# mlrun/mlrun

Measured on AMD Instinct MI355X. Metric: serving-graph req/sec (Llama-3-8B V2ModelServer), higher is better.
Workload: dtype bf16; 1 GPU; model=llama-3-8b, global_batch=32, seq_len=160, prompt_len=128, parallelism=dp1 (2 engine replica(s)/GPU, 2 in flight), hipgraph=True

## Files before the change

mlrun_amd/models/llama.py:

```python

import math
import typing
from dataclasses import dataclass

import torch

from .. import ops
from ..utils import logger


@dataclass
class LlamaConfig:
    name: str = "llama-3-8b"
    hidden_size: int = 4096
    intermediate_size: int = 14336
    num_layers: int = 32
    num_heads: int = 32
    num_kv_heads: int = 8
    head_dim: int = 128
    vocab_size: int = 128256
    rope_theta: float = 500000.0
    rms_eps: float = 1e-5
    max_seq_len: int = 2048

# ... 81 lines not shown
    while f"blocks.{i}.attn_norm.weight" in state:
        prefix = f"blocks.{i}."
        out[f"layers.{i}.attn_norm"] = state[prefix + "attn_norm.weight"]
        out[f"layers.{i}.wqkv"] = state[prefix + "attn.wqkv.weight"]
        out[f"layers.{i}.wo"] = state[prefix + "attn.wo.weight"]
        out[f"layers.{i}.ffn_norm"] = state[prefix + "ffn_norm.weight"]
        out[f"layers.{i}.wgu"] = state[prefix + "mlp.wgu.weight"]
        out[f"layers.{i}.wdown"] = state[prefix + "mlp.wdown.weight"]
        i += 1
    return {k: v.to(torch.bfloat16) for k, v in out.items()}


LORA_PROJECTIONS = ("wqkv", "wo", "wgu", "wdown")


@dataclass
class SamplingParams:
    temperature: float = 0.0
    top_k: int = 0
    top_p: float = 1.0
    min_p: float = 0.0
    seed: int = 0
    logprobs: bool = False

    def validate(self):
        def number(name, value):
            if isinstance(value, bool) or \
                    not isinstance(value, (int, float)) or \
                    value != value:
                raise ValueError(f"{name} must be a number, got {value!r}")

        def integer(name, value):
            if isinstance(value, bool) or not isinstance(value, int):
                raise ValueError(f"{name} must be an integer, got "
                                 f"{value!r}")

        number("temperature", self.temperature)
        if not 0 <= self.temperature < float("inf"):
            raise ValueError(f"temperature must be >= 0 and finite, got "
                             f"{self.temperature}")
        integer("top_k", self.top_k)
        if not 0 <= self.top_k < 2 ** 31:
            raise ValueError(f"top_k must be an integer >= 0, got "
                             f"{self.top_k}")
        number("top_p", self.top_p)
        if not 0 < self.top_p <= 1:
            raise ValueError(f"top_p must be in (0, 1], got {self.top_p}")
        number("min_p", self.min_p)
        if not 0 <= self.min_p < 1:
            raise ValueError(f"min_p must be in [0, 1), got {self.min_p}")
        integer("seed", self.seed)
        if not 0 <= self.seed < 2 ** 63:
            raise ValueError(f"seed must be an integer in [0, 2^63), got "
                             f"{self.seed}")
        if not isinstance(self.logprobs, bool):
            raise ValueError(f"logprobs must be true or false, got "
                             f"{self.logprobs!r}")
        return self


class LoraTables:

    def __init__(self, weights: LlamaWeights, max_adapters: int,
                 rank: int = 16):
        if rank not in ops.LORA_RANKS:
            raise ValueError(f"lora_rank must be one of {ops.LORA_RANKS}, "
                             f"got {rank}")
        if max_adapters < 1:
            raise ValueError("LoraTables needs max_adapters >= 1")
        self.max_adapters = int(max_adapters)
        self.rank = int(rank)
        self.weights = weights
        self.loaded = set()
        bf16 = dict(dtype=torch.bfloat16, device=weights.device)
        self.layers = []
        for layer in weights.layers:
            tables = {}
            for proj in LORA_PROJECTIONS:
                n, k = layer[proj].shape
                tables[proj] = (
                    torch.zeros(self.max_adapters, self.rank, k, **bf16),
                    torch.zeros(self.max_adapters, n, self.rank, **bf16))
            self.layers.append(tables)

    def _check_slot(self, slot):
        if not 0 <= int(slot) < self.max_adapters:
            raise ValueError(f"adapter slot {slot} outside "
                             f"[0, {self.max_adapters})")
        return int(slot)

    def unload(self, slot: int):
        slot = self._check_slot(slot)
        for tables in self.layers:
            for a_tab, b_tab in tables.values():
                a_tab[slot].zero_()
                b_tab[slot].zero_()
        self.loaded.discard(slot)

    @torch.no_grad()
    def load(self, slot: int, state: dict):
        slot = self._check_slot(slot)
        if "alpha" not in state:
            raise ValueError("adapter state has no 'alpha'")
        alpha = float(state["alpha"])
        pending = []
        seen = set()
        for key in state:
            if not key.startswith("layers."):
                continue
            parts = key.split(".")
            if len(parts) != 4 or not parts[1].isdigit() or \
                    parts[2] not in LORA_PROJECTIONS or \
                    parts[3] not in ("lora_A", "lora_B") or \
                    int(parts[1]) >= len(self.layers):
                raise ValueError(f"unexpected adapter key {key!r}")
            seen.add((int(parts[1]), parts[2]))
        for li, proj in sorted(seen):
            key_a = f"layers.{li}.{proj}.lora_A"
            key_b = f"layers.{li}.{proj}.lora_B"
            for key in (key_a, key_b):
                if key not in state:
                    raise ValueError(f"adapter state lacks {key!r}")
            mat_a, mat_b = state[key_a], state[key_b]
            n, k = self.weights.layers[li][proj].shape
            if mat_a.dim() != 2 or mat_a.shape[1] != k:
                raise ValueError(f"{key_a}: expected [r, {k}], got "
                                 f"{tuple(mat_a.shape)}")
            r = mat_a.shape[0]
            if not 1 <= r <= self.rank:
                raise ValueError(f"{key_a}: rank {r} outside "
                                 f"[1, lora_rank={self.rank}]")
            if tuple(mat_b.shape) != (n, r):
                raise ValueError(f"{key_b}: expected [{n}, {r}], got "
                                 f"{tuple(mat_b.shape)}")
            pending.append((li, proj, r, mat_a, mat_b))
        self.unload(slot)
        for li, proj, r, mat_a, mat_b in pending:
            a_tab, b_tab = self.layers[li][proj]
            a_tab[slot, :r].copy_(mat_a)
            scaled = mat_b.to(device=b_tab.device, dtype=torch.float32) \
                * (alpha / r)
            b_tab[slot, :, :r].copy_(scaled)
        self.loaded.add(slot)


class LlamaDecodeEngine:

    def __init__(self, cfg: LlamaConfig, batch_size: int, device=None,
                 tp_group=None, tp_rank=0, tp_size=1, use_graph=True,
                 seed=1234, weights: "LlamaWeights" = None,
                 weight_dtype: str = "bf16", kv_dtype: str = "bf16",
                 temperature: float = 0.0, top_k: int = 0,
                 max_adapters: int = 0, lora_rank: int = 16,
                 lora: "LoraTables" = None, sampling: str = "engine"):
        if sampling not in ("engine", "request"):
            raise ValueError(f"unknown sampling mode {sampling!r} "
                             "(expected 'engine' or 'request')")
        if sampling == "request" and tp_size > 1:
            raise ValueError(
                f'sampling="request" conflicts with tp_size={tp_size}: '
                "per-request sampling runs on a single GPU")
        if sampling == "request" and batch_size > ops.SAMPLE_MAX_ROWS:
            raise ValueError(
                f'sampling="request" needs batch_size <= '
                f"{ops.SAMPLE_MAX_ROWS}, got {batch_size}")
        if (max_adapters > 0 or lora is not None) and tp_size > 1:
            raise ValueError(
                f"max_adapters={max_adapters} conflicts with tp_size="
                f"{tp_size}: LoRA adapters are not sharded")
        if (max_adapters > 0 or lora is not None) and \
                batch_size > ops.LORA_MAX_ROWS:
            raise ValueError(
                f"max_adapters > 0 needs batch_size <= "
                f"{ops.LORA_MAX_ROWS}, got {batch_size}")
        self.cfg = cfg
        self.B = batch_size
        self.device = torch.device(
            device or ("cuda:0" if torch.cuda.is_available() else "cpu"))
        self.on_gpu = self.device.type == "cuda"
        self.tp_group = tp_group
        self.tp_rank = tp_rank
        self.tp_size = tp_size
        self.use_graph = use_graph and self.on_gpu
        self.temperature = float(temperature)
        self.top_k = int(top_k)
        self.per_slot_temp = self.temperature < 0
        self.buf_temp = torch.full((batch_size, 1), 1e-4,
                                   dtype=torch.float32,
                                   device=self.device) \
            if self.per_slot_temp else None
        self.weights = weights if weights is not None else \
            LlamaWeights(cfg, self.device, tp_rank, tp_size, seed)
        w = self.weights
        d, h = cfg.head_dim, cfg.hidden_size
        B, smax = batch_size, cfg.max_seq_len
        bf16 = dict(dtype=torch.bfloat16, device=self.device)

        self.kv_dtype = kv_dtype
        if kv_dtype == "fp8":
            u8 = dict(dtype=torch.uint8, device=self.device)
            self.k_cache = torch.zeros(cfg.num_layers, B, w.hkv, smax, d,
                                       **u8)
            self.v_cache = torch.zeros(cfg.num_layers, B, w.hkv, smax, d,
                                       **u8)
            f32 = dict(dtype=torch.float32, device=self.device)
            self.k_scale = torch.ones(cfg.num_layers, B, w.hkv, smax,
                                      **f32)
            self.v_scale = torch.ones(cfg.num_layers, B, w.hkv, smax,
                                      **f32)
        else:
            self.k_cache = torch.zeros(cfg.num_layers, B, w.hkv, smax, d,
                                       **bf16)
            self.v_cache = torch.zeros(cfg.num_layers, B, w.hkv, smax, d,
                                       **bf16)
            self.k_scale = self.v_scale = None
        self.cache_lens = torch.zeros(B, dtype=torch.int32,
                                      device=self.device)
        self.buf_positions = torch.zeros(B, dtype=torch.int32,
                                         device=self.device)
        self.cos_sin = ops.build_rope_cos_sin(smax, d, cfg.rope_theta,
                                              self.device)

        qkv_n = (w.hq + 2 * w.hkv) * d
        gemm_shapes = [(qkv_n, h), (h, w.hq * d), (2 * w.inter, h),
                       (h, w.inter), (cfg.vocab_size, h)]
        scratch = max(ops.pick_gemm_plan(B, n, k)[0] * n
                      for n, k in gemm_shapes)
        self.buf_tokens = torch.zeros(B, dtype=torch.int64,
                                      device=self.device)
        self.buf_hidden = torch.zeros(B, h, **bf16)
        self.buf_residual = torch.zeros(B, h, **bf16)
        self.buf_qkv = torch.zeros(B, qkv_n, **bf16)
        self.buf_attn_out = torch.zeros(B, w.hq * d, **bf16)
        self.buf_proj = torch.zeros(B, h, **bf16)
        self.buf_gu = torch.zeros(B, 2 * w.inter, **bf16)
        self.buf_act = torch.zeros(B, w.inter, **bf16)
        self.buf_down = torch.zeros(B, h, **bf16)
        self.buf_logits = torch.zeros(B, cfg.vocab_size, **bf16)
        self.buf_c32 = torch.empty(B * scratch, dtype=torch.float32,
                                   device=self.device)
        self.scale = 1.0 / math.sqrt(d)
        self._capture_stream_ctx = None
        self.weight_dtype = weight_dtype
        self._fp8_packs = {}
        if weight_dtype == "fp8w" and self.on_gpu and tp_size == 1:
            max_k = max(h, w.inter, w.hq * d)
            self.buf_a8 = torch.empty(B * max_k, dtype=torch.uint8,
                                      device=self.device)
            self.buf_a_scale = torch.empty(B, dtype=torch.float32,
                                           device=self.device)
            self.buf_h8 = torch.empty(B, h, dtype=torch.uint8,
                                      device=self.device)
            self.buf_h8_scale = torch.empty(B, dtype=torch.float32,
                                            device=self.device)
            self.rebuild_fp8_packs()
        import os as _os
        _ns = _os.environ.get("MLRUN_ATTN_NSPLIT")
        self.attn_nsplit = int(_ns) if _ns else \
            ops.pick_attn_nsplit(B, w.hkv)
        self.buf_attn_ws = torch.empty(
            B * w.hq * self.attn_nsplit * (d + 2), dtype=torch.float32,
            device=self.device) if self.on_gpu else None
        self._graph = None
        self._ksplits = {}
        if lora is None and max_adapters > 0:
            lora = LoraTables(w, max_adapters, lora_rank)
        self.lora = lora
        self.max_adapters = lora.max_adapters if lora is not None else 0
        if lora is not None:
            self.buf_adapter = torch.full((B,), -1, dtype=torch.int32,
                                          device=self.device)
            self.buf_lora_t = torch.zeros(B, lora.rank,
                                          dtype=torch.float32,
                                          device=self.device)
        self.sampling = sampling
        if sampling == "request":
            dev = self.device
            self.buf_temp_r = torch.zeros(B, dtype=torch.float32, device=dev)
            self.buf_top_k = torch.zeros(B, dtype=torch.int32, device=dev)
            self.buf_top_p = torch.ones(B, dtype=torch.float32, device=dev)
            self.buf_min_p = torch.zeros(B, dtype=torch.float32, device=dev)
            self.buf_seed = torch.zeros(B, dtype=torch.int64, device=dev)
            self.buf_logprob = torch.zeros(B, dtype=torch.float32,
                                           device=dev)
            self.buf_kept = torch.zeros(B, dtype=torch.int32, device=dev)
        self.spec_stats = {"steps": 0, "drafted": 0, "accepted": 0}

    def set_sampling(self, slot: int, temperature: float = 0.0,
                     top_k: int = 0, top_p: float = 1.0, min_p: float = 0.0,
                     seed: int = 0):
        self.set_sampling_slots([slot], [SamplingParams(
            temperature, top_k, top_p, min_p, seed)])

    def set_sampling_slots(self, slots, params):
        if self.sampling != "request":
            raise ValueError('set_sampling needs an engine built with '
                             'sampling="request"')
        slots = [int(slot) for slot in slots]
        params = [SamplingParams() if item is None else item
                  for item in params]
        if len(slots) != len(params):
            raise ValueError(f"{len(params)} parameter sets for "
                             f"{len(slots)} slots")
        for slot in slots:
            if not 0 <= slot < self.B:
                raise ValueError(f"slot {slot} outside [0, {self.B})")
        for item in params:
            item.validate()
        if not slots:
            return
        index = torch.tensor(slots, dtype=torch.long).to(self.device)
        for buf, name in ((self.buf_temp_r, "temperature"),
                          (self.buf_top_k, "top_k"),
                          (self.buf_top_p, "top_p"),
                          (self.buf_min_p, "min_p"),
                          (self.buf_seed, "seed")):
            values = [getattr(item, name) for item in params]
            if name == "temperature":
                values = [max(value, 1e-4) if value > 0 else value
                          for value in values]
            values = torch.tensor(values, dtype=buf.dtype)
            buf[index] = values.to(self.device)

    def _packed_prefill_serves(self) -> bool:
        w = self.weights
        return self.kv_dtype == "bf16" and self.cfg.head_dim == 128 \
            and w.hq % w.hkv == 0 and w.hq // w.hkv <= 8

    def _sample_slots(self, logits, slots):
        logits = logits.contiguous()
        n = logits.shape[0]
        tokens = torch.empty(n, dtype=torch.int64, device=self.device)
        logprob = torch.empty(n, dtype=torch.float32, device=self.device)
        kept = torch.empty(n, dtype=torch.int32, device=self.device)
        ops.sample_tokens(
            logits, self.cache_lens[slots].contiguous(),
            self.buf_temp_r[slots].contiguous(),
            self.buf_top_k[slots].contiguous(),
            self.buf_top_p[slots].contiguous(),
            self.buf_min_p[slots].contiguous(),
            self.buf_seed[slots].contiguous(), tokens, logprob, kept)
        self.buf_tokens[slots] = tokens
        self.buf_logprob[slots] = logprob
        self.buf_kept[slots] = kept
        return tokens

    def _plan(self, w_):
        key = (w_.shape[0], w_.shape[1])
        if key not in self._ksplits:
            self._ksplits[key] = ops.pick_gemm_plan(self.B, *key)
        return self._ksplits[key]

    def _gemm(self, a, w_, out, a8=None, a_scale=None):
        pack = self._fp8_packs.get(id(w_))
        if pack is not None:
            M, K = a.shape
            if a8 is None:
                a8 = self.buf_a8.narrow(0, 0, M * K).view(M, K)
                ops.quant_fp8_rows(a, a8, self.buf_a_scale)
                a_scale = self.buf_a_scale
            ksplit, _ = self._plan(w_)
            return ops.skinny_gemm_fp8(a8, a_scale, pack[0],
                                       pack[1], out=out,
                                       c_f32=self.buf_c32, ksplit=ksplit)
        ksplit, variant = self._plan(w_)
        return ops.skinny_gemm(a, w_, out=out, c_f32=self.buf_c32,
                               ksplit=ksplit, variant=variant)

    def _gemm_slabs(self, a, w_):
        from mlrun_amd import _hip_ops

        ksplit, variant = self._plan(w_)
        if ksplit <= 1:
            return 0
        _hip_ops.skinny_gemm_slabs(self.buf_c32, a, w_, ksplit, variant)
        return ksplit

    def _maybe_allreduce(self, t):
        if self.tp_size > 1:
            from ..parallel.tp import all_reduce_tensor

            all_reduce_tensor(t, group=self.tp_group)
        return t

    def load_adapter(self, slot: int, state: dict):
        if self.lora is None:
            raise ValueError("engine built with max_adapters=0 holds no "
                             "adapter tables")
        self.lora.load(slot, state)

    def unload_adapter(self, slot: int):
        if self.lora is None:
            raise ValueError("engine built with max_adapters=0 holds no "
                             "adapter tables")
        self.lora.unload(slot)

    def _lora_decode(self, li, proj, x, y):
        a_tab, b_tab = self.lora.layers[li][proj]
        ops.lora_shrink(x, a_tab, self.buf_adapter, out=self.buf_lora_t)
        ops.lora_expand(y, self.buf_lora_t, b_tab, self.buf_adapter)

    def _adapter_plan(self, adapters, slots, counts):
        if adapters is None:
            if self.lora is not None:
                self.buf_adapter[slots] = -1
            return None
        ids = [int(a) for a in adapters]
        if self.lora is None:
            if any(a >= 0 for a in ids):
                raise ValueError("adapters= needs an engine built with "
                                 "max_adapters > 0")
            return None
        if len(ids) != len(counts):
            raise ValueError(f"adapters has {len(ids)} ids for "
                             f"{len(counts)} prompts")
        for a in ids:
            if not -1 <= a < self.max_adapters:
                raise ValueError(f"adapter id {a} outside "
                                 f"[-1, {self.max_adapters})")
        self.buf_adapter[slots] = torch.tensor(
            ids, dtype=torch.int32).to(self.device)
        distinct = sorted({a for a in ids if a >= 0})
        if not distinct:
            return None
        if len(set(ids)) == 1:
            return [(distinct[0], None)]
        row_ids = torch.tensor(
            [a for a, count in zip(ids, counts) for _ in range(count)],
            dtype=torch.int32).to(self.device)
        return [(a, (row_ids == a).unsqueeze(1)) for a in distinct]

    def _lora_prefill(self, plan, li, proj, x, y):
        if plan is None:
            return y
        a_tab, b_tab = self.lora.layers[li][proj]
        xf = x.float()
        for a, mask in plan:
            delta = (xf @ a_tab[a].float().t()) @ b_tab[a].float().t()
            new = (y.float() + delta).to(y.dtype)
            y = new if mask is None else torch.where(mask, new, y)
        return y

    def _decode_step_body(self):
        cfg, w = self.cfg, self.weights
        d = cfg.head_dim
        B = self.B
        torch.index_select(w.embed, 0, self.buf_tokens,
                           out=self.buf_residual)
        fp8 = self.weight_dtype == "fp8w" and self.on_gpu and \
            self.tp_size == 1
        h8 = self.buf_h8 if fp8 else None
        h8s = self.buf_h8_scale if fp8 else None
        ops.rmsnorm(self.buf_residual, w.layers[0]["attn_norm"],
                    eps=cfg.rms_eps, out=self.buf_hidden,
                    out8=h8, out_scale=h8s)
        torch.clamp(self.cache_lens, max=self.cfg.max_seq_len - 1,
                    out=self.buf_positions)
        self.cache_lens.add_(1).clamp_(max=self.cfg.max_seq_len)
        positions = self.buf_positions
        import os as _os

        mode = _os.environ.get("MLRUN_SLAB_MODE", "rope")
        on = self.on_gpu and self.tp_size == 1 and mode != "none"
        use_slabs = on and self.weight_dtype == "bf16" and \
            self.kv_dtype == "bf16"
        use_norm_slabs = on and mode == "all" 
        lora = self.lora is not None
        if lora:
            use_slabs = use_norm_slabs = False
        for li, layer in enumerate(w.layers):
            done = 0
            if use_slabs:
                done = self._gemm_slabs(self.buf_hidden, layer["wqkv"])
                if done:
                    from mlrun_amd import _hip_ops

                    _hip_ops.rope_kv_slab(
                        self.buf_qkv, self.k_cache[li], self.v_cache[li],
                        self.buf_c32, positions, self.cos_sin, w.hq, done)
            if not done:
                self._gemm(self.buf_hidden, layer["wqkv"], self.buf_qkv,
                           a8=h8, a_scale=h8s)
                if lora:
                    self._lora_decode(li, "wqkv", self.buf_hidden,
                                      self.buf_qkv)
                ops.rope_kv_fused(self.buf_qkv, self.k_cache[li],
                                  self.v_cache[li], positions,
                                  self.cos_sin, w.hq,
                                  k_scale=self._kscale(li),
                                  v_scale=self._vscale(li))
            q = self.buf_qkv[:, :w.hq * d].view(B, w.hq, d)
            attn_view = self.buf_attn_out.view(B, w.hq, d)
            ops.attn_decode(q, self.k_cache[li], self.v_cache[li],
                            self.cache_lens, self.scale, out=attn_view,
                            partial_ws=self.buf_attn_ws,
                            nsplit=self.attn_nsplit,
                            k_scale=self._kscale(li),
                            v_scale=self._vscale(li))
            done = 0
            if use_norm_slabs:
                done = self._gemm_slabs(self.buf_attn_out, layer["wo"])
                if done:
                    from mlrun_amd import _hip_ops

                    _hip_ops.fused_add_rmsnorm_slab(
                        self.buf_hidden, self.buf_residual, self.buf_c32,
                        layer["ffn_norm"], done, cfg.rms_eps)
            if not done:
                self._gemm(self.buf_attn_out, layer["wo"], self.buf_proj)
                if lora:
                    self._lora_decode(li, "wo", self.buf_attn_out,
                                      self.buf_proj)
                self._maybe_allreduce(self.buf_proj)
                ops.fused_add_rmsnorm(self.buf_proj, layer["ffn_norm"],
                                      residual=self.buf_residual,
                                      eps=cfg.rms_eps, out=self.buf_hidden,
                                      out8=h8, out_scale=h8s)
            done = 0
            if use_norm_slabs:
                done = self._gemm_slabs(self.buf_hidden, layer["wgu"])
                if done:
                    from mlrun_amd import _hip_ops

                    _hip_ops.swiglu_slab(self.buf_act, self.buf_c32, done)
            if not done:
                self._gemm(self.buf_hidden, layer["wgu"], self.buf_gu,
                           a8=h8, a_scale=h8s)
                if lora:
                    self._lora_decode(li, "wgu", self.buf_hidden,
                                      self.buf_gu)
                ops.swiglu_fused(self.buf_gu, out=self.buf_act)
            next_norm = w.layers[li + 1]["attn_norm"] \
                if li + 1 < cfg.num_layers else w.final_norm
            done = 0
            if use_norm_slabs:
                done = self._gemm_slabs(self.buf_act, layer["wdown"])
                if done:
                    from mlrun_amd import _hip_ops

                    _hip_ops.fused_add_rmsnorm_slab(
                        self.buf_hidden, self.buf_residual, self.buf_c32,
                        next_norm, done, cfg.rms_eps)
            if not done:
                self._gemm(self.buf_act, layer["wdown"], self.buf_down)
                if lora:
                    self._lora_decode(li, "wdown", self.buf_act,
                                      self.buf_down)
                self._maybe_allreduce(self.buf_down)
                ops.fused_add_rmsnorm(self.buf_down, next_norm,
                                      residual=self.buf_residual,
                                      eps=cfg.rms_eps, out=self.buf_hidden,
                                      out8=h8, out_scale=h8s)
        self._gemm(self.buf_hidden, w.lm_head, self.buf_logits,
                   a8=h8, a_scale=h8s)
        if self.sampling == "request":
            ops.sample_tokens(self.buf_logits, self.cache_lens,
                              self.buf_temp_r, self.buf_top_k,
                              self.buf_top_p, self.buf_min_p, self.buf_seed,
                              self.buf_tokens, self.buf_logprob,
                              self.buf_kept)
        else:
            self._select_tokens(self.buf_logits, out=self.buf_tokens)

    def _select_tokens(self, logits: torch.Tensor,
                       out: torch.Tensor = None) -> torch.Tensor:
        if self.per_slot_temp and logits.shape[0] == self.B:
            scores = logits.float() / self.buf_temp
            u = torch.rand_like(scores).clamp_(1e-9, 1.0 - 1e-9)
            gumbel = -torch.log(-torch.log(u))
            if out is None:
                return (scores + gumbel).argmax(dim=-1)
            torch.argmax(scores + gumbel, dim=-1, out=out)
            return out
        if self.temperature <= 0.0:
            if out is None:
                return logits.argmax(dim=-1)
            torch.argmax(logits, dim=-1, out=out)
            return out
        scores = logits.float() / self.temperature
        if self.top_k > 0 and self.top_k < scores.shape[-1]:
            kth = torch.topk(scores, self.top_k, dim=-1
                             ).values[..., -1:]
            scores = torch.where(scores < kth,
                                 torch.full_like(scores, float("-inf")),
                                 scores)
        u = torch.rand_like(scores).clamp_(1e-9, 1.0 - 1e-9)
        gumbel = -torch.log(-torch.log(u))
        if out is None:
            return (scores + gumbel).argmax(dim=-1)
        torch.argmax(scores + gumbel, dim=-1, out=out)
        return out

    _capture_lock = None

    def capture_graph(self):
        if not self.use_graph or self._graph is not None:
            return
        import threading

        cls = type(self)
        if cls._capture_lock is None:
            cls._capture_lock = threading.Lock()
        with cls._capture_lock:
            self._capture_graph_locked()

    def _capture_graph_locked(self):
        if self._graph is not None:
            return
        import torch.distributed as dist

        lens_backup = self.cache_lens.clone()
        tokens_backup = self.buf_tokens.clone()
        sample_backup = [(buf, buf.clone()) for buf in (
            self.buf_logprob, self.buf_kept)] \
            if self.sampling == "request" else []
        if self.tp_size > 1 and dist.is_available() and \
                dist.is_initialized():
            dist.barrier(group=self.tp_group)
        side = torch.cuda.Stream()
        side.wait_stream(torch.cuda.current_stream())
        with torch.cuda.stream(side):
            for _ in range(3):
                self._decode_step_body()
        torch.cuda.current_stream().wait_stream(side)
        self.cache_lens.copy_(lens_backup)
        self.buf_tokens.copy_(tokens_backup)
        for buf, backup in sample_backup:
            buf.copy_(backup)
        graph = torch.cuda.CUDAGraph()
        err_mode = "thread_local" if dist.is_available() and \
            dist.is_initialized() else "global"
        with torch.cuda.graph(graph, capture_error_mode=err_mode):
            self._decode_step_body()
        self.cache_lens.copy_(lens_backup)
        self.buf_tokens.copy_(tokens_backup)
        for buf, backup in sample_backup:
            buf.copy_(backup)
        self._graph = graph
        logger.info("decode hipGraph captured", batch=self.B,
                    layers=self.cfg.num_layers)

    def decode_step(self):
        if self._graph is not None:
            self._graph.replay()
        else:
            self._decode_step_body()

    def rebuild_fp8_packs(self):
        if self.weight_dtype != "fp8w" or not (self.on_gpu and
                                               self.tp_size == 1):
            return
        w = self.weights
        self._fp8_packs = {}
        for layer in w.layers:
            for key in ("wqkv", "wo", "wgu", "wdown"):
                self._fp8_packs[id(layer[key])] = \
                    ops.quantize_fp8_weight(layer[key])
        self._fp8_packs[id(w.lm_head)] = \
            ops.quantize_fp8_weight(w.lm_head)

    def _kscale(self, li):
        return None if self.k_scale is None else self.k_scale[li]

    def _vscale(self, li):
        return None if self.v_scale is None else self.v_scale[li]

    def _check_token_ids(self, tokens: torch.Tensor):
        if tokens.device.type != "cpu" or tokens.numel() == 0:
            return
        low, high = int(tokens.min()), int(tokens.max())
        if low < 0 or high >= self.cfg.vocab_size:
            raise ValueError(
                f"token id outside [0, {self.cfg.vocab_size}) in prompt")

    @torch.no_grad()
    def prefill(self, tokens: torch.Tensor, adapters=None
                ) -> torch.Tensor:
        cfg, w = self.cfg, self.weights
        B, S = tokens.shape
        d = cfg.head_dim
        self._check_token_ids(tokens)
        plan = self._adapter_plan(adapters, slice(0, B), [S] * B)
        tokens = tokens.to(self.device)
        x = w.embed[tokens.reshape(-1)]
        residual = x.contiguous()
        positions = torch.arange(S, dtype=torch.int32, device=self.device
                                 ).repeat(B)
        hidden = ops.rmsnorm(residual, w.layers[0]["attn_norm"],
                             eps=cfg.rms_eps)
        for li, layer in enumerate(w.layers):
            qkv = self._lora_prefill(plan, li, "wqkv", hidden,
                                     hidden @ layer["wqkv"].t())
            q = qkv[:, :w.hq * d].reshape(B * S, w.hq, d).contiguous()
            k = qkv[:, w.hq * d:(w.hq + w.hkv) * d].reshape(
                B * S, w.hkv, d).contiguous()
# ... 255 lines not shown
                             f"(kv_dtype={self.kv_dtype!r})")
        if self.weight_dtype != "bf16":
            raise ValueError("speculative decoding needs bf16 weights "
                             f"(weight_dtype={self.weight_dtype!r})")
        if self.tp_size != 1:
            raise ValueError("speculative decoding needs tp_size == 1")
        if not 1 <= int(k) <= ops.VERIFY_MAX_QL - 1:
            raise ValueError(
                f"speculative k must be in [1, {ops.VERIFY_MAX_QL - 1}], "
                f"got {k}")

    def _verify_gemm(self, a, w_, QL):
        if self.on_gpu:
            return a @ w_.t()
        out = torch.empty(a.shape[0], w_.shape[0], dtype=a.dtype)
        for j in range(QL):
            out[j::QL] = ops.skinny_gemm(a[j::QL].contiguous(), w_)
        return out

    @torch.no_grad()
    def verify_step(self, drafts: torch.Tensor):
        cfg, w = self.cfg, self.weights
        if drafts.dim() != 2 or drafts.shape[0] != self.B:
            raise ValueError(f"drafts must be [{self.B}, k], got "
                             f"{tuple(drafts.shape)}")
        k = drafts.shape[1]
        self._check_speculative(k)
        B, QL, d = self.B, k + 1, cfg.head_dim
        T = B * QL
        drafts = drafts.to(device=self.device, dtype=torch.int64)
        fed = drafts.clamp(0, cfg.vocab_size - 1)
        tokens = torch.cat([self.buf_tokens.view(B, 1), fed], dim=1)
        base = torch.clamp(self.cache_lens, min=0,
                           max=cfg.max_seq_len - QL)
        steps = torch.arange(QL, dtype=torch.int32, device=self.device)
        positions = (base.view(B, 1) + steps).reshape(T)
        tok_slot = torch.arange(B, dtype=torch.int32, device=self.device
                                ).repeat_interleave(QL)
        nsplit, ws = None, None
        if self.on_gpu:
            nsplit = ops.pick_verify_nsplit(B, w.hkv, cfg.max_seq_len)
            need = ops.attn_verify_ws_numel(B, QL, w.hq, nsplit)
            ws = getattr(self, "_verify_ws", None)
            if nsplit > 1 and (ws is None or ws.numel() < need):
                ws = self._verify_ws = torch.empty(
                    need, dtype=torch.float32, device=self.device)
        residual = w.embed[tokens.reshape(T)].contiguous()
        hidden = ops.rmsnorm(residual, w.layers[0]["attn_norm"],
                             eps=cfg.rms_eps)
        for li, layer in enumerate(w.layers):
            qkv = self._verify_gemm(hidden, layer["wqkv"], QL)
            ops.rope_kv_varlen(qkv, self.k_cache[li], self.v_cache[li],
                               positions, tok_slot, self.cos_sin, w.hq)
            q = qkv[:, :w.hq * d].view(B, QL, w.hq, d)
            attn = ops.attn_verify(q, self.k_cache[li], self.v_cache[li],
                                   base, self.scale, nsplit=nsplit,
                                   partial_ws=ws)
            proj = self._verify_gemm(attn, layer["wo"], QL)
            hidden = ops.fused_add_rmsnorm(proj, layer["ffn_norm"],
                                           residual=residual,
                                           eps=cfg.rms_eps)
            gu = self._verify_gemm(hidden, layer["wgu"], QL)
            act = ops.swiglu_fused(gu.contiguous())
            down = self._verify_gemm(act, layer["wdown"], QL)
            next_norm = w.layers[li + 1]["attn_norm"] \
                if li + 1 < cfg.num_layers else w.final_norm
            hidden = ops.fused_add_rmsnorm(down, next_norm,
                                           residual=residual,
                                           eps=cfg.rms_eps)
        logits = getattr(self, "buf_verify_logits", None)
        if logits is None or logits.shape[1] != QL:
            logits = self.buf_verify_logits = torch.empty(
                B, QL, cfg.vocab_size, dtype=torch.bfloat16,
                device=self.device)
        logits.view(T, cfg.vocab_size).copy_(
            self._verify_gemm(hidden, w.lm_head, QL))
        pred = logits.argmax(dim=-1)
        hits = (drafts == pred[:, :k]).to(torch.int64)
        n_accepted = hits.cumprod(dim=1).sum(dim=1)
        self.cache_lens.add_((n_accepted + 1).to(torch.int32)
                             ).clamp_(max=cfg.max_seq_len)
        self.buf_tokens.copy_(
            pred.gather(1, n_accepted.view(B, 1)).view(B))
        return pred, n_accepted

    def _speculative_loop(self, history: torch.Tensor,
                          hist_lens: torch.Tensor, start_lens: torch.Tensor,
                          active: torch.Tensor, max_new_tokens: int,
                          k: int, ngram: int) -> torch.Tensor:
        B, QL = self.B, k + 1
        L = history.shape[1]
        steps = torch.arange(QL, dtype=torch.int64, device=self.device)
        counters = torch.zeros(2, dtype=torch.int64, device=self.device)
        big = torch.full((B,), max_new_tokens, dtype=torch.int32,
                         device=self.device)
        n_steps = 0
        produced_min = 1
        while produced_min < max_new_tokens:
            produced = hist_lens - start_lens
            done = (produced >= max_new_tokens) | ~active
            drafts = ops.ngram_draft(history, hist_lens, k, n=ngram)
            lens_before = self.cache_lens.clone()
            tokens_before = self.buf_tokens.clone()
            pred, n_accepted = self.verify_step(drafts)
            self.cache_lens.copy_(
                torch.where(done, lens_before, self.cache_lens))
            self.buf_tokens.copy_(
                torch.where(done, tokens_before, self.buf_tokens))
            idx = (hist_lens.view(B, 1).long() + steps).clamp_(max=L - 1)
            vals = torch.where(done.view(B, 1), history.gather(1, idx),
                               pred)
            history.scatter_(1, idx, vals)
            live = ~done
            hist_lens.add_((live * (n_accepted + 1)).to(torch.int32))
            counters[0] += live.sum() * k
            counters[1] += (n_accepted * live).sum()
            n_steps += 1
            produced_min = int(torch.where(
                active, hist_lens - start_lens, big).min())
        drafted, accepted = counters.tolist()
        self.spec_stats["steps"] += n_steps
        self.spec_stats["drafted"] += drafted
        self.spec_stats["accepted"] += accepted
        cols = start_lens.view(B, 1).long() + torch.arange(
            max_new_tokens, dtype=torch.int64, device=self.device)
        return history.gather(1, cols.clamp_(max=L - 1))

    @torch.no_grad()
    def generate_speculative(self, tokens: torch.Tensor,
                             max_new_tokens: int = 32, k: int = 3,
                             ngram: int = 2) -> torch.Tensor:
        B, S = tokens.shape
        assert B == self.B, f"engine built for batch {self.B}, got {B}"
        self._check_speculative(k)
        assert S + max_new_tokens + k <= self.cfg.max_seq_len, \
            "speculative decoding needs room for k drafted tokens: " \
            f"{S}+{max_new_tokens}+{k} > {self.cfg.max_seq_len}"
        logits = self.prefill(tokens)
        self.buf_tokens.copy_(self._select_tokens(logits))
        history = torch.zeros(B, self.cfg.max_seq_len, dtype=torch.int64,
                              device=self.device)
        history[:, :S] = tokens.to(self.device)
        history[:, S] = self.buf_tokens
        hist_lens = torch.full((B,), S + 1, dtype=torch.int32,
                               device=self.device)
        start_lens = torch.full((B,), S, dtype=torch.int32,
                                device=self.device)
        active = torch.ones(B, dtype=torch.bool, device=self.device)
        return self._speculative_loop(history, hist_lens, start_lens,
                                      active, max_new_tokens, k, ngram)

    def reset(self):
        self.cache_lens.zero_()


class LlamaServer:

    def __init__(self, context=None, name=None, model_path=None,
                 config=None, batch_size=16, max_new_tokens=32,
                 device=None, use_graph=True, batch_window_ms=0,
                 replicas=1, weight_dtype="bf16", kv_dtype="bf16",
                 scheduling="batch", stop_token: int = None,
                 temperature: float = 0.0, top_k: int = 0,
                 prefill: str = "exact", speculative: int = 0,
                 adapters: dict = None, max_adapters: int = None,
                 lora_rank: int = 16, sampling: str = "engine",
                 top_p: float = 1.0, min_p: float = 0.0, **class_args):
        import queue as queue_mod
        import threading

        from ..serving.v2_serving import V2ModelServer

        self.name = name
        self.context = context
        self.model_path = model_path
        self.ready = False
        self.error = ""
        self.protocol = "v2"
        self.model_spec = None
        self._model_logger = None
        self._params = class_args
        self.cfg_name = config or "llama-3-8b"
        self.batch_size = batch_size
        self.max_new_tokens = max_new_tokens
        self.device = device
        self.use_graph = use_graph
        self.weight_dtype = weight_dtype
        self.kv_dtype = kv_dtype
        self.scheduling = scheduling
        if prefill not in ("exact", "packed"):
            raise ValueError(f"unknown prefill mode {prefill!r} "
                             "(expected 'exact' or 'packed')")
        self.prefill = prefill
        self.stop_token = stop_token
        self.temperature = float(temperature)
        self.top_k = int(top_k)
        self.speculative = int(speculative)
        self.adapters = dict(adapters or {})
        self.adapter_slots = {name: slot for slot, name
                              in enumerate(self.adapters)}
        self.max_adapters = len(self.adapters) if max_adapters is None \
            else int(max_adapters)
        if self.max_adapters < len(self.adapters):
            raise ValueError(
                f"max_adapters={self.max_adapters} is below the "
                f"{len(self.adapters)} adapters configured")
        self.lora_rank = int(lora_rank)
        self._lora_requests = {name: 0 for name in self.adapters}
        self._lora_lock = threading.Lock()
        if sampling not in ("engine", "request"):
            raise ValueError(f"unknown sampling mode {sampling!r} "
                             "(expected 'engine' or 'request')")
        self.sampling = sampling
        self._sampling_defaults = None
        self._sampling_counts = {"requests": 0, "sampled": 0, "greedy": 0}
        if sampling == "request":
            if self.temperature < 0:
                raise ValueError(
                    f"temperature={temperature} conflicts with "
                    'sampling="request": per-slot temperatures are the '
                    "request field there, the default must be >= 0")
            self._sampling_defaults = SamplingParams(
                temperature=temperature, top_k=top_k, top_p=top_p,
                min_p=min_p).validate()
        self._check_speculative_config()
        self.replicas = max(int(replicas), 1)
        self.engines: typing.List[LlamaDecodeEngine] = []
        self.batch_window_ms = batch_window_ms
        self._tasks: "queue_mod.Queue" = queue_mod.Queue()
        self._workers: typing.List[threading.Thread] = []
        self._pending = []
        self._pending_cv = threading.Condition()
        self._batcher = None
        self.engine_calls = 0

    @property
    def engine(self):
        return self.engines[0] if self.engines else None

    def _check_speculative_config(self):
        k = self.speculative
        if k == 0:
            return
        if self.sampling == "request":
            raise ValueError(
                f'speculative={k} conflicts with sampling="request": '
                "speculative decoding is greedy only")
        if self.max_adapters > 0:
            raise ValueError(
                f"speculative={k} conflicts with LoRA adapters "
                f"({sorted(self.adapters)}): the verify pass runs the "
                "base weights only")
        if not 1 <= k <= ops.VERIFY_MAX_QL - 1:
            raise ValueError(
                f"speculative={k} is outside [0, {ops.VERIFY_MAX_QL - 1}]")
        if self.scheduling == "continuous":
            raise ValueError(
                f'speculative={k} conflicts with scheduling="continuous" '
                "(its output ring takes one token per slot per step): "
                'use scheduling="batch"')
        if self.temperature != 0.0:
            raise ValueError(
                f"speculative={k} conflicts with temperature="
                f"{self.temperature}: speculative decoding is greedy only")
        if self.kv_dtype == "fp8":
            raise ValueError(
                f'speculative={k} conflicts with kv_dtype="fp8": the '
                "verify attention kernel reads bf16 caches only")
        if self.weight_dtype == "fp8w":
            raise ValueError(
                f'speculative={k} conflicts with weight_dtype="fp8w": '
                "the verify pass runs on the bf16 weights")

    def post_init(self, mode="sync"):
        stream = getattr(self.context, "stream", None) if self.context \
            else None
        if stream is not None:
            from ..serving.v2_serving import _ModelLogPusher

            self._model_logger = _ModelLogPusher(self, stream)
        if mode == "sync":
            self.load()
            self.ready = True

    def _build_config(self) -> LlamaConfig:
        if self.cfg_name in ("llama-3-8b", "8b"):
            cfg = LlamaConfig.llama3_8b()
        elif self.cfg_name in ("llama-3-70b", "70b"):
            cfg = LlamaConfig.llama3_70b()
        elif self.cfg_name == "tiny":
            cfg = LlamaConfig.tiny()
        elif isinstance(self.cfg_name, LlamaConfig):
            cfg = self.cfg_name
        else:
            raise ValueError(f"unknown llama config {self.cfg_name}")
        for key, value in self._params.items():
            if hasattr(cfg, key):
                setattr(cfg, key, value)
        return cfg

    def load(self):
        import threading

        cfg = self._build_config()
        self._check_speculative_config()
        if self.prefill == "packed" and self.kv_dtype == "fp8":
# ... 628 lines not shown
```

mlrun_amd/ops/__init__.py:

```python

import math
import os

import torch

from ..errors import MLRunGPUError

try:
    from mlrun_amd import _hip_ops

    HAVE_HIP_OPS = True
except ImportError:
    _hip_ops = None
    HAVE_HIP_OPS = False


def _require_hip():
    if not HAVE_HIP_OPS:
        raise MLRunGPUError(
            "mlrun_amd._hip_ops extension is not built — run "
            "`PYTORCH_ROCM_ARCH=gfx950 python setup.py build_ext --inplace` "
            "(GPU ops never fall back to eager execution)")
    return _hip_ops




def fused_add_rmsnorm(x: torch.Tensor, weight: torch.Tensor,
                      residual: torch.Tensor = None, eps: float = 1e-5,
                      out: torch.Tensor = None,
                      out8: torch.Tensor = None,
                      out_scale: torch.Tensor = None) -> torch.Tensor:
    if x.is_cuda:
        ops = _require_hip()
        if out is None:
            out = torch.empty_like(x)
        ops.fused_add_rmsnorm(out, x, weight, residual, eps, out8,
                              out_scale)
        return out
    z = x.float() + (residual.float() if residual is not None else 0.0)
    if residual is not None:
        residual.copy_(z.to(residual.dtype))
    var = z.pow(2).mean(dim=-1, keepdim=True)
    result = (z * torch.rsqrt(var + eps)) * weight.float()
    result = result.to(x.dtype)
    if out is not None:
        out.copy_(result)
        return out
    return result


def rmsnorm(x, weight, eps=1e-5, out=None, out8=None, out_scale=None):
    return fused_add_rmsnorm(x, weight, residual=None, eps=eps, out=out,
                             out8=out8, out_scale=out_scale)




def build_rope_cos_sin(max_pos: int, head_dim: int, theta: float = 500000.0,
                       device="cpu") -> torch.Tensor:
    half = head_dim // 2
    inv_freq = 1.0 / (theta ** (torch.arange(0, half, dtype=torch.float64)
                                / half))
    pos = torch.arange(max_pos, dtype=torch.float64)
    angles = torch.outer(pos, inv_freq)
    table = torch.stack([angles.cos(), angles.sin()], dim=-1).float()
    return table.contiguous().to(device)


def rope_inplace(q: torch.Tensor, positions: torch.Tensor,
                 cos_sin: torch.Tensor):
    if q.is_cuda:
        _require_hip().rope(q, positions, cos_sin)
        return q
    T, heads, dim = q.shape
    half = dim // 2
    table = cos_sin[positions.long()]
    cos = table[..., 0].unsqueeze(1)
    sin = table[..., 1].unsqueeze(1)
    qf = q.float()
    q1 = qf[..., :half]
    q2 = qf[..., half:]
    q[..., :half] = (q1 * cos - q2 * sin).to(q.dtype)
    q[..., half:] = (q2 * cos + q1 * sin).to(q.dtype)
    return q




def swiglu_fused(gu: torch.Tensor, out: torch.Tensor = None) -> torch.Tensor:
    rows, two_i = gu.shape
    inter = two_i // 2
    if gu.is_cuda:
        ops = _require_hip()
        if out is None:
            out = torch.empty(rows, inter, dtype=gu.dtype, device=gu.device)
        ops.swiglu_fused(out, gu)
        return out
    result = (torch.nn.functional.silu(gu[:, :inter].float()) *
              gu[:, inter:].float()).to(gu.dtype)
    if out is not None:
        out.copy_(result)
        return out
    return result


def silu_mul(gate: torch.Tensor, up: torch.Tensor,
             out: torch.Tensor = None) -> torch.Tensor:
    if gate.is_cuda:
        ops = _require_hip()
        if out is None:
            out = torch.empty_like(gate)
        ops.silu_mul(out, gate, up)
        return out
    result = (torch.nn.functional.silu(gate.float()) *
              up.float()).to(gate.dtype)
    if out is not None:
        out.copy_(result)
        return out
    return result




def pick_ksplit(M: int, N: int, K: int, target_blocks: int = 2048) -> int:
    nblocks = (N + 127) // 128
    if nblocks >= target_blocks:
        return 1
    ksplit = (target_blocks + nblocks - 1) // nblocks
    ksplit = min(ksplit, max(K // 256, 1), 16)
    return max(ksplit, 1)


_EMPTY_F32 = None


_GEMM_PLAN_TABLE = {
    (6144, 4096): (4, 4),
    (4096, 4096): (2, 4),
    (28672, 4096): (1, 4),
    (4096, 14336): (4, 4),
    (128256, 4096): (1, 0),
}

_plan_env = os.environ.get("MLRUN_GEMM_PLAN", "")
if _plan_env:
    for _cell in _plan_env.split(";"):
        _shape, _plan = _cell.split("=")
        _n, _k = _shape.split("x")
        _ks, _var = _plan.split(",")
        _GEMM_PLAN_TABLE[(int(_n), int(_k))] = (int(_ks), int(_var))


def pick_gemm_plan(M: int, N: int, K: int) -> tuple:
    if (N, K) in _GEMM_PLAN_TABLE:
        return _GEMM_PLAN_TABLE[(N, K)]
    nblocks_ws = (N + 31) // 32
    if nblocks_ws <= 512 and K >= 2048:
        ksplit = max(1, min(1024 // nblocks_ws, K // 1024, 8))
        return ksplit, 1
    return pick_ksplit(M, N, K), 0


def skinny_gemm(a: torch.Tensor, w: torch.Tensor,
                out: torch.Tensor = None,
                c_f32: torch.Tensor = None,
                ksplit: int = None, variant: int = None) -> torch.Tensor:
    global _EMPTY_F32

    M, K = a.shape
    N = w.shape[0]
    if a.is_cuda:
        ops = _require_hip()
        if ksplit is None and variant is None:
            ksplit, variant = pick_gemm_plan(M, N, K)
        elif ksplit is None:
            ksplit = pick_ksplit(M, N, K)
        elif variant is None:
            variant = 0
        if out is None:
            out = torch.empty(M, N, dtype=torch.bfloat16, device=a.device)
        if ksplit > 1 and c_f32 is None:
            c_f32 = torch.empty(ksplit * M * N, dtype=torch.float32,
                                device=a.device)
        if c_f32 is None:
            if _EMPTY_F32 is None or _EMPTY_F32.device != a.device:
                _EMPTY_F32 = torch.empty(1, dtype=torch.float32,
                                         device=a.device)
            c_f32 = _EMPTY_F32
        ops.skinny_gemm(out, c_f32, a, w, ksplit, variant)
        return out
    result = (a.float() @ w.float().t()).to(a.dtype)
    if out is not None:
        out.copy_(result)
        return out
    return result


FP8_MAX = 448.0


def _fp8_pair_swizzle(q: torch.Tensor) -> torch.Tensor:
    n, k = q.shape
    assert k % 64 == 0, "K must be a multiple of 64 for the fp8 path"
    return q.view(n, k // 64, 2, 4, 8).permute(0, 1, 3, 2, 4) \
        .contiguous().view(n, k)


def _fp8_pair_unswizzle(q: torch.Tensor) -> torch.Tensor:
    n, k = q.shape
    return q.view(n, k // 64, 4, 2, 8).permute(0, 1, 3, 2, 4) \
        .contiguous().view(n, k)


def quantize_fp8_weight(w: torch.Tensor):
    amax = w.float().abs().amax(dim=1).clamp(min=1e-8)
    scale = amax / FP8_MAX
    q = (w.float() / scale[:, None]).to(torch.float8_e4m3fn)
    q8 = _fp8_pair_swizzle(q.view(torch.uint8))
    return q8.contiguous(), scale.to(torch.float32).contiguous()


def quant_fp8_rows(a: torch.Tensor, a8: torch.Tensor = None,
                   a_scale: torch.Tensor = None):
    rows, cols = a.shape[0], a.shape[-1]
    if a.is_cuda:
        ops = _require_hip()
        if a8 is None:
            a8 = torch.empty(a.shape, dtype=torch.uint8, device=a.device)
        if a_scale is None:
            a_scale = torch.empty(rows, dtype=torch.float32,
                                  device=a.device)
        ops.quant_fp8_rows(a8, a_scale, a)
        return a8, a_scale
    amax = a.float().abs().amax(dim=-1).clamp(min=1e-8)
    scale = amax / FP8_MAX
    q = (a.float() / scale[:, None]).to(torch.float8_e4m3fn)
    q = _fp8_pair_swizzle(q.view(torch.uint8))
    if a8 is not None:
        a8.copy_(q)
        a_scale.copy_(scale)
        return a8, a_scale
    return q.contiguous(), scale.to(torch.float32).contiguous()


def skinny_gemm_fp8(a8: torch.Tensor, a_scale: torch.Tensor,
                    w8: torch.Tensor, w_scale: torch.Tensor,
                    out: torch.Tensor = None, c_f32: torch.Tensor = None,
                    ksplit: int = 1) -> torch.Tensor:
    global _EMPTY_F32

    M, K = a8.shape
    N = w8.shape[0]
    if a8.is_cuda:
        ops = _require_hip()
        if out is None:
            out = torch.empty(M, N, dtype=torch.bfloat16,
                              device=a8.device)
        if ksplit > 1 and c_f32 is None:
            c_f32 = torch.empty(ksplit * M * N, dtype=torch.float32,
                                device=a8.device)
        if c_f32 is None:
            if _EMPTY_F32 is None or _EMPTY_F32.device != a8.device:
                _EMPTY_F32 = torch.empty(1, dtype=torch.float32,
                                         device=a8.device)
            c_f32 = _EMPTY_F32
        ops.skinny_gemm_fp8(out, c_f32, a8, a_scale, w8, w_scale, ksplit)
        return out
    a = _fp8_pair_unswizzle(a8).view(torch.float8_e4m3fn).float() * \
        a_scale[:, None].float()
    w = _fp8_pair_unswizzle(w8).view(torch.float8_e4m3fn).float() * \
        w_scale[:, None].float()
    result = (a @ w.t()).to(torch.bfloat16)
    if out is not None:
        out.copy_(result)
        return out
    return result


def rope_kv_fused(qkv: torch.Tensor, k_cache: torch.Tensor,
                  v_cache: torch.Tensor, positions: torch.Tensor,
                  cos_sin: torch.Tensor, hq: int,
                  k_scale: torch.Tensor = None,
                  v_scale: torch.Tensor = None):
    B = qkv.shape[0]
    hkv, d = k_cache.shape[1], k_cache.shape[3]
    if qkv.is_cuda:
        _require_hip().rope_kv_fused(qkv, k_cache, v_cache, positions,
                                     cos_sin, hq, k_scale, v_scale)
        return
    q = qkv[:, :hq * d].view(B, hq, d)
    k = qkv[:, hq * d:(hq + hkv) * d].view(B, hkv, d)
    v = qkv[:, (hq + hkv) * d:(hq + 2 * hkv) * d].view(B, hkv, d)
    rope_inplace(q, positions, cos_sin)
    rope_inplace(k, positions, cos_sin)
    if k_scale is not None:
        for b in range(B):
            pos = int(positions[b])
            k8, ks = quantize_kv_rows(k[b])
            v8, vs = quantize_kv_rows(v[b])
            k_cache[b, :, pos] = k8
            v_cache[b, :, pos] = v8
            k_scale.view(B, hkv, -1)[b, :, pos] = ks
            v_scale.view(B, hkv, -1)[b, :, pos] = vs
        return
    kv_append(k_cache, v_cache, k, v, positions)


def quantize_kv_rows(x: torch.Tensor):
    amax = x.float().abs().amax(dim=-1, keepdim=True)
    scales = torch.where(amax > 0, amax / 448.0,
                         torch.ones_like(amax))
    q8 = (x.float() / scales).to(torch.float8_e4m3fn).view(torch.uint8)
    return q8, scales.squeeze(-1)


def dequantize_kv_rows(q8: torch.Tensor, scales: torch.Tensor,
                       dtype=torch.float32):
    x = q8.view(torch.float8_e4m3fn).float()
    return (x * scales.unsqueeze(-1)).to(dtype)




def pick_attn_nsplit(B: int, Hkv: int, target: int = 2048,
                     seq_len: int = None) -> int:
    base = max(B * Hkv, 1)
    fill = (target + base - 1) // base
    chunk = (seq_len + 127) // 128 if seq_len else 1
    n = max(1, fill, chunk)
    n = 1 << (n - 1).bit_length()
    return min(n, 16)


def attn_decode(q: torch.Tensor, k_cache: torch.Tensor,
                v_cache: torch.Tensor, seq_lens: torch.Tensor,
                scale: float = None,
                out: torch.Tensor = None,
                partial_ws: torch.Tensor = None,
                nsplit: int = None,
                k_scale: torch.Tensor = None,
                v_scale: torch.Tensor = None) -> torch.Tensor:
    B, Hq, D = q.shape
    Hkv = k_cache.shape[1]
    scale = scale if scale is not None else 1.0 / math.sqrt(D)
    if q.is_cuda:
        ops = _require_hip()
        if out is None:
            out = torch.empty_like(q)
        if nsplit is None:
            nsplit = pick_attn_nsplit(B, Hkv)
        if nsplit > 1 and partial_ws is None:
            partial_ws = torch.empty(B * Hq * nsplit * (D + 2),
                                     dtype=torch.float32, device=q.device)
        ops.attn_decode(out, q, k_cache, v_cache, seq_lens, scale,
                        partial_ws, nsplit, k_scale, v_scale)
        return out
    if out is None:
        out = torch.empty_like(q)
    if k_scale is not None:
        k_cache = dequantize_kv_rows(k_cache,
                                     k_scale.view(B, Hkv, -1))
        v_cache = dequantize_kv_rows(v_cache,
                                     v_scale.view(B, Hkv, -1))
    G = Hq // Hkv
    for b in range(B):
        length = int(seq_lens[b])
        for h in range(Hq):
            kvh = h // G
            qv = q[b, h].float()
            keys = k_cache[b, kvh, :length].float()
            vals = v_cache[b, kvh, :length].float()
            scores = torch.softmax(keys @ qv * scale, dim=0)
            out[b, h] = (scores @ vals).to(q.dtype)
    return out




def rope_kv_varlen(qkv: torch.Tensor, k_cache: torch.Tensor,
                   v_cache: torch.Tensor, positions: torch.Tensor,
                   tok_slot: torch.Tensor, cos_sin: torch.Tensor, hq: int):
    T = qkv.shape[0]
    hkv, d = k_cache.shape[1], k_cache.shape[3]
    if qkv.is_cuda:
        _require_hip().rope_kv_varlen(qkv, k_cache, v_cache, positions,
                                      tok_slot, cos_sin, hq)
        return
    q = qkv[:, :hq * d].view(T, hq, d)
    k = qkv[:, hq * d:(hq + hkv) * d].view(T, hkv, d)
    v = qkv[:, (hq + hkv) * d:(hq + 2 * hkv) * d].view(T, hkv, d)
    rope_inplace(q, positions, cos_sin)
    rope_inplace(k, positions, cos_sin)
    for t in range(T):
        slot, pos = int(tok_slot[t]), int(positions[t])
        k_cache[slot, :, pos] = k[t]
        v_cache[slot, :, pos] = v[t]


def attn_prefill(q: torch.Tensor, k_cache: torch.Tensor,
                 v_cache: torch.Tensor, cu_seqlens: torch.Tensor,
                 slots: torch.Tensor, kv_start: torch.Tensor,
                 scale: float = None, out: torch.Tensor = None,
                 max_q_len: int = None) -> torch.Tensor:
    T, Hq, D = q.shape
    Hkv = k_cache.shape[1]
    scale = scale if scale is not None else 1.0 / math.sqrt(D)
    if out is None:
        out = torch.empty(T, Hq * D, dtype=q.dtype, device=q.device)
    if q.is_cuda:
        ops = _require_hip()
        if max_q_len is None:
            cu = cu_seqlens.tolist()
            max_q_len = max((b - a for a, b in zip(cu, cu[1:])), default=0)
        ops.attn_prefill(out, q, k_cache, v_cache, cu_seqlens, slots,
                         kv_start, scale, int(max_q_len))
        return out
    G = Hq // Hkv
    cu = cu_seqlens.tolist()
    out_v = out.view(T, Hq, D)
    for i in range(len(cu) - 1):
        slot, start = int(slots[i]), int(kv_start[i])
        for j in range(cu[i + 1] - cu[i]):
            row = cu[i] + j
            length = start + j + 1
            for h in range(Hq):
                kvh = h // G
                qv = q[row, h].float()
                keys = k_cache[slot, kvh, :length].float()
                vals = v_cache[slot, kvh, :length].float()
                scores = torch.softmax(keys @ qv * scale, dim=0)
                out_v[row, h] = (scores @ vals).to(q.dtype)
    return out



VERIFY_MAX_QL = 8
_VERIFY_WS_ROW = 128 + 4


def pick_verify_nsplit(B: int, Hkv: int, Smax: int,
                       target: int = 512) -> int:
    base = max(B * Hkv, 1)
    n = max(1, target // base)
    n = 1 << (n.bit_length() - 1)
    return max(1, min(n, 16, (Smax + 63) // 64))


def attn_verify_ws_numel(B: int, QL: int, Hq: int, nsplit: int) -> int:
    return B * QL * Hq * nsplit * _VERIFY_WS_ROW


def attn_verify(q: torch.Tensor, k_cache: torch.Tensor,
                v_cache: torch.Tensor, base_lens: torch.Tensor,
                scale: float = None, out: torch.Tensor = None,
                nsplit: int = None,
                partial_ws: torch.Tensor = None) -> torch.Tensor:
    if q.dim() != 4 or k_cache.dim() != 4:
        raise ValueError("attn_verify: q must be [B, QL, Hq, D] and the "
                         "caches [B, Hkv, Smax, D]")
    B, QL, Hq, D = q.shape
    Hkv, Smax = k_cache.shape[1], k_cache.shape[2]
    if D != 128 or k_cache.shape[3] != D:
        raise ValueError(f"attn_verify needs head_dim 128, got {D}")
    if not 1 <= QL <= VERIFY_MAX_QL:
        raise ValueError(
            f"attn_verify needs 1 <= QL <= {VERIFY_MAX_QL}, got {QL}")
    if Hkv < 1 or Hq % Hkv or Hq // Hkv > 8:
        raise ValueError("attn_verify: q heads per kv head must divide "
                         f"and be <= 8 (Hq={Hq}, Hkv={Hkv})")
    if k_cache.dtype != torch.bfloat16 or v_cache.dtype != torch.bfloat16 \
            or q.dtype != torch.bfloat16:
        raise ValueError("attn_verify reads bf16 q and bf16 KV caches only")
    if k_cache.shape[0] != B or base_lens.numel() != B:
        raise ValueError("attn_verify: q, caches and base_lens must agree "
                         "on the batch size")
    scale = scale if scale is not None else 1.0 / math.sqrt(D)
    if out is None:
        out = torch.empty(B * QL, Hq * D, dtype=q.dtype, device=q.device)
    if q.is_cuda:
        ops = _require_hip()
        if nsplit is None:
            nsplit = pick_verify_nsplit(B, Hkv, Smax)
        nsplit = max(int(nsplit), 1)
        if nsplit > 1 and partial_ws is None:
            partial_ws = torch.empty(
                attn_verify_ws_numel(B, QL, Hq, nsplit),
                dtype=torch.float32, device=q.device)
        ops.attn_verify(out, q, k_cache, v_cache, base_lens, scale,
                        partial_ws, nsplit)
        return out
    cu = torch.arange(B + 1, dtype=torch.int32) * QL
    slots = torch.arange(B, dtype=torch.int32)
    return attn_prefill(q.reshape(B * QL, Hq, D), k_cache, v_cache, cu,
                        slots, base_lens, scale, out=out)


def ngram_draft(history: torch.Tensor, hist_lens: torch.Tensor, k: int,
                n: int = 2, out: torch.Tensor = None) -> torch.Tensor:
    if history.dim() != 2 or history.dtype != torch.int64:
        raise ValueError("ngram_draft: history must be [B, L] int64")
    k, n = int(k), int(n)
    if k < 1 or not 1 <= n <= 64:
        raise ValueError("ngram_draft needs k >= 1 and 1 <= n <= 64")
    B, L = history.shape
    if hist_lens.numel() != B:
        raise ValueError("ngram_draft: one hist_lens entry per row")
    if out is None:
        out = torch.empty(B, k, dtype=torch.int64, device=history.device)
# ... 479 lines not shown
```

mlrun_amd/ops/hip/bindings.cpp:

```cpp

#include <torch/extension.h>
#include <c10/hip/HIPStream.h>

#include "kernels.h"

#define CHECK_DEV(x) TORCH_CHECK((x).is_cuda(), #x " must be on GPU")
#define CHECK_CONTIG(x) TORCH_CHECK((x).is_contiguous(), #x " not contiguous")
#define CHECK_BF16(x) \
  TORCH_CHECK((x).scalar_type() == torch::kBFloat16, #x " must be bf16")
#define CHECK_F32(x) \
  TORCH_CHECK((x).scalar_type() == torch::kFloat32, #x " must be f32")

#define CHECK_U8(x) \
  TORCH_CHECK((x).scalar_type() == torch::kUInt8, #x " must be uint8")

#define CHECK_I32(x) \
  TORCH_CHECK((x).scalar_type() == torch::kInt32, #x " must be int32")

static void* stream() {
  return (void*)c10::hip::getCurrentHIPStream().stream();
}

void fused_add_rmsnorm(torch::Tensor out, torch::Tensor x,
                       torch::Tensor weight,
                       c10::optional<torch::Tensor> residual, double eps,
                       c10::optional<torch::Tensor> out8,
                       c10::optional<torch::Tensor> out_scale) {
  CHECK_DEV(out); CHECK_CONTIG(out); CHECK_BF16(out);
  CHECK_DEV(x); CHECK_CONTIG(x); CHECK_BF16(x);
  CHECK_DEV(weight); CHECK_CONTIG(weight); CHECK_BF16(weight);
  int64_t hidden = x.size(-1);
  int64_t rows = x.numel() / hidden;
  TORCH_CHECK(hidden % 8 == 0, "hidden must be a multiple of 8");
  TORCH_CHECK(weight.numel() == hidden, "weight size mismatch");
  void* res_ptr = nullptr;
  if (residual.has_value()) {
    CHECK_DEV(*residual); CHECK_CONTIG(*residual); CHECK_BF16(*residual);
    TORCH_CHECK(residual->numel() == x.numel(), "residual size mismatch");
    res_ptr = residual->data_ptr();
  }
  void* out8_ptr = nullptr;
  void* scale_ptr = nullptr;
  if (out8.has_value()) {
    TORCH_CHECK(out_scale.has_value(), "out8 needs out_scale");
    TORCH_CHECK(out8->numel() == x.numel() &&
                out_scale->numel() >= rows, "fp8 sidecar sizes");
    TORCH_CHECK(hidden % 64 == 0, "fp8 sidecar needs hidden % 64 == 0");
    out8_ptr = out8->data_ptr();
    scale_ptr = out_scale->data_ptr();
  }
  launch_fused_add_rmsnorm(out.data_ptr(), res_ptr, x.data_ptr(),
                           weight.data_ptr(), (int)rows, (int)hidden,
                           (float)eps, out8_ptr, scale_ptr, stream());
}

static long long check_head_view(const torch::Tensor& q) {
  TORCH_CHECK(q.dim() == 3, "expected [T, heads, dim]");
  TORCH_CHECK(q.stride(2) == 1 && q.stride(1) == q.size(2),
              "inner dims must be dense (strides (*, dim, 1))");
  return (long long)q.stride(0);
}

void rope(torch::Tensor q, torch::Tensor positions, torch::Tensor cos_sin) {
  CHECK_DEV(q); CHECK_BF16(q);
  CHECK_DEV(positions); CHECK_CONTIG(positions); CHECK_I32(positions);
  CHECK_DEV(cos_sin); CHECK_CONTIG(cos_sin); CHECK_F32(cos_sin);
  long long row_stride = check_head_view(q);
  int T = q.size(0), heads = q.size(1), dim = q.size(2);
  TORCH_CHECK(dim % 2 == 0 && dim / 2 <= 1024, "bad head dim");
  TORCH_CHECK(positions.numel() == T, "positions size mismatch");
  launch_rope(q.data_ptr(), positions.data_ptr(), cos_sin.data_ptr(), T,
              heads, dim, row_stride, stream());
}

void swiglu_fused(torch::Tensor out, torch::Tensor gu) {
  CHECK_DEV(out); CHECK_CONTIG(out); CHECK_BF16(out);
  CHECK_DEV(gu); CHECK_CONTIG(gu); CHECK_BF16(gu);
  TORCH_CHECK(gu.dim() == 2 && out.dim() == 2, "need 2-D tensors");
  int rows = gu.size(0), inter = gu.size(1) / 2;
  TORCH_CHECK(out.size(0) == rows && out.size(1) == inter, "shape mismatch");
  TORCH_CHECK(inter % 8 == 0, "inter must be a multiple of 8");
  launch_swiglu_fused(out.data_ptr(), gu.data_ptr(), rows, inter, stream());
}

void silu_mul(torch::Tensor out, torch::Tensor gate, torch::Tensor up) {
  CHECK_DEV(out); CHECK_CONTIG(out); CHECK_BF16(out);
  CHECK_DEV(gate); CHECK_CONTIG(gate); CHECK_BF16(gate);
  CHECK_DEV(up); CHECK_CONTIG(up); CHECK_BF16(up);
  TORCH_CHECK(out.numel() == gate.numel() && gate.numel() == up.numel(),
              "size mismatch");
  TORCH_CHECK(out.numel() % 8 == 0, "numel must be a multiple of 8");
  launch_silu_mul(out.data_ptr(), gate.data_ptr(), up.data_ptr(),
                  out.numel(), stream());
}

void skinny_gemm(torch::Tensor out_bf16, torch::Tensor part_f32,
                 torch::Tensor a, torch::Tensor w, int64_t ksplit,
                 int64_t variant) {
  CHECK_DEV(out_bf16); CHECK_CONTIG(out_bf16); CHECK_BF16(out_bf16);
  CHECK_DEV(a); CHECK_CONTIG(a); CHECK_BF16(a);
  CHECK_DEV(w); CHECK_CONTIG(w); CHECK_BF16(w);
  int M = a.size(0), K = a.size(1), N = w.size(0);
  TORCH_CHECK(w.size(1) == K, "K mismatch");
  TORCH_CHECK(M <= 64, "skinny_gemm supports M <= 64");
  TORCH_CHECK(K % 32 == 0, "K must be a multiple of 32");
  TORCH_CHECK(out_bf16.numel() == (int64_t)M * N, "out shape mismatch");
  if (ksplit > 1) {
    CHECK_DEV(part_f32); CHECK_CONTIG(part_f32); CHECK_F32(part_f32);
    TORCH_CHECK(part_f32.numel() >= ksplit * (int64_t)M * N,
                "part_f32 scratch too small");
  }
  launch_skinny_gemm(out_bf16.data_ptr(),
                     ksplit > 1 ? part_f32.data_ptr() : nullptr,
                     a.data_ptr(), w.data_ptr(), M, N, K, (int)ksplit,
                     (int)variant, stream());
}

void skinny_gemm_slabs(torch::Tensor part_f32, torch::Tensor a,
                       torch::Tensor w, int64_t ksplit, int64_t variant) {
  CHECK_DEV(part_f32); CHECK_CONTIG(part_f32); CHECK_F32(part_f32);
  CHECK_DEV(a); CHECK_CONTIG(a); CHECK_BF16(a);
  CHECK_DEV(w); CHECK_CONTIG(w); CHECK_BF16(w);
  int M = a.size(0), K = a.size(1), N = w.size(0);
  TORCH_CHECK(w.size(1) == K && M <= 64 && K % 32 == 0, "bad shapes");
  TORCH_CHECK(part_f32.numel() >= ksplit * (int64_t)M * N,
              "part_f32 scratch too small");
  launch_skinny_gemm_slabs(part_f32.data_ptr(), a.data_ptr(), w.data_ptr(),
                           M, N, K, (int)ksplit, (int)variant, stream());
}

void fused_add_rmsnorm_slab(torch::Tensor out, torch::Tensor residual,
                            torch::Tensor slabs, torch::Tensor weight,
                            int64_t ksplit, double eps) {
  CHECK_DEV(out); CHECK_CONTIG(out); CHECK_BF16(out);
  CHECK_DEV(residual); CHECK_CONTIG(residual); CHECK_BF16(residual);
  CHECK_DEV(slabs); CHECK_CONTIG(slabs); CHECK_F32(slabs);
  CHECK_DEV(weight); CHECK_CONTIG(weight); CHECK_BF16(weight);
  int64_t hidden = out.size(-1);
  int64_t rows = out.numel() / hidden;
  TORCH_CHECK(hidden % 8 == 0, "hidden must be a multiple of 8");
  TORCH_CHECK(slabs.numel() >= ksplit * rows * hidden, "slabs too small");
  launch_fused_add_rmsnorm_slab(out.data_ptr(), residual.data_ptr(),
                                slabs.data_ptr(), weight.data_ptr(),
                                (int)rows, (int)hidden, (float)eps,
                                (int)ksplit, stream());
}

void swiglu_slab(torch::Tensor out, torch::Tensor slabs, int64_t ksplit) {
  CHECK_DEV(out); CHECK_CONTIG(out); CHECK_BF16(out);
  CHECK_DEV(slabs); CHECK_CONTIG(slabs); CHECK_F32(slabs);
  int rows = out.size(0), inter = out.size(1);
  TORCH_CHECK(inter % 4 == 0, "inter must be a multiple of 4");
  TORCH_CHECK(slabs.numel() >= (int64_t)ksplit * rows * 2 * inter,
              "slabs too small");
  launch_swiglu_slab(out.data_ptr(), slabs.data_ptr(), rows, inter,
                     (int)ksplit, stream());
}

void rope_kv_slab(torch::Tensor qkv, torch::Tensor kc, torch::Tensor vc,
                  torch::Tensor slabs, torch::Tensor positions,
                  torch::Tensor cos_sin, int64_t hq, int64_t ksplit) {
  CHECK_DEV(qkv); CHECK_CONTIG(qkv); CHECK_BF16(qkv);
  CHECK_DEV(kc); CHECK_CONTIG(kc); CHECK_BF16(kc);
  CHECK_DEV(slabs); CHECK_CONTIG(slabs); CHECK_F32(slabs);
  CHECK_DEV(positions); CHECK_CONTIG(positions); CHECK_I32(positions);
  CHECK_DEV(cos_sin); CHECK_CONTIG(cos_sin); CHECK_F32(cos_sin);
  int B = kc.size(0), Hkv = kc.size(1), Smax = kc.size(2), D = kc.size(3);
  int qkv_row = qkv.size(1);
  TORCH_CHECK(qkv.size(0) == B && qkv_row >= (hq + 2 * Hkv) * D,
              "qkv buffer too small");
  TORCH_CHECK(slabs.numel() >= (int64_t)ksplit * B * qkv_row,
              "slabs too small");
  launch_rope_kv_slab(qkv.data_ptr(), kc.data_ptr(), vc.data_ptr(),
                      slabs.data_ptr(), positions.data_ptr(),
                      cos_sin.data_ptr(), B, (int)hq, Hkv, Smax, D, qkv_row,
                      (int)ksplit, stream());
}

void rope_kv_fused(torch::Tensor qkv, torch::Tensor kc, torch::Tensor vc,
                   torch::Tensor positions, torch::Tensor cos_sin,
                   int64_t hq,
                   c10::optional<torch::Tensor> k_scale = c10::nullopt,
                   c10::optional<torch::Tensor> v_scale = c10::nullopt) {
  CHECK_DEV(qkv); CHECK_CONTIG(qkv); CHECK_BF16(qkv);
  CHECK_DEV(kc); CHECK_CONTIG(kc);
  CHECK_DEV(vc); CHECK_CONTIG(vc);
  CHECK_DEV(positions); CHECK_CONTIG(positions); CHECK_I32(positions);
  CHECK_DEV(cos_sin); CHECK_CONTIG(cos_sin); CHECK_F32(cos_sin);
  int B = kc.size(0), Hkv = kc.size(1), Smax = kc.size(2), D = kc.size(3);
  TORCH_CHECK(qkv.dim() == 2 && qkv.size(0) == B, "qkv must be [B, rows]");
  TORCH_CHECK(qkv.size(1) >= (hq + 2 * Hkv) * D, "qkv row too small");
  if (k_scale.has_value()) {
    TORCH_CHECK(v_scale.has_value(), "fp8 KV needs both scales");
    CHECK_U8(kc); CHECK_U8(vc);
    CHECK_DEV(*k_scale); CHECK_CONTIG(*k_scale); CHECK_F32(*k_scale);
    CHECK_DEV(*v_scale); CHECK_CONTIG(*v_scale); CHECK_F32(*v_scale);
    TORCH_CHECK(k_scale->numel() >= (int64_t)B * Hkv * Smax &&
                v_scale->numel() >= (int64_t)B * Hkv * Smax,
                "scale tensors too small");
    TORCH_CHECK(D == 128, "fp8 KV requires head_dim 128");
    launch_rope_kv_fused_q8(qkv.data_ptr(), kc.data_ptr(), vc.data_ptr(),
                            k_scale->data_ptr(), v_scale->data_ptr(),
                            positions.data_ptr(), cos_sin.data_ptr(), B,
                            (int)hq, Hkv, Smax, D, qkv.size(1), stream());
    return;
  }
  CHECK_BF16(kc); CHECK_BF16(vc);
  launch_rope_kv_fused(qkv.data_ptr(), kc.data_ptr(), vc.data_ptr(),
                       positions.data_ptr(), cos_sin.data_ptr(), B, (int)hq,
                       Hkv, Smax, D, qkv.size(1), stream());
}

void skinny_gemm_fp8(torch::Tensor out_bf16, torch::Tensor part_f32,
                     torch::Tensor a8, torch::Tensor a_scale,
                     torch::Tensor w8, torch::Tensor w_scale,
                     int64_t ksplit) {
  CHECK_DEV(out_bf16); CHECK_CONTIG(out_bf16); CHECK_BF16(out_bf16);
  CHECK_DEV(a8); CHECK_CONTIG(a8); CHECK_U8(a8);
  CHECK_DEV(w8); CHECK_CONTIG(w8); CHECK_U8(w8);
  CHECK_DEV(a_scale); CHECK_F32(a_scale);
  CHECK_DEV(w_scale); CHECK_F32(w_scale);
  int M = a8.size(0), K = a8.size(1), N = w8.size(0);
  TORCH_CHECK(w8.size(1) == K && M <= 64 && K % 64 == 0,
              "bad shapes (fp8 path needs K % 64 == 0)");
  TORCH_CHECK(a_scale.numel() >= M && w_scale.numel() >= N,
              "scale sizes");
  if (ksplit > 1) {
    CHECK_DEV(part_f32); CHECK_CONTIG(part_f32); CHECK_F32(part_f32);
    TORCH_CHECK(part_f32.numel() >= ksplit * (int64_t)M * N,
                "part_f32 scratch too small");
  }
  launch_skinny_gemm_fp8(out_bf16.data_ptr(),
                         ksplit > 1 ? part_f32.data_ptr() : nullptr,
                         a8.data_ptr(), a_scale.data_ptr(), w8.data_ptr(),
                         w_scale.data_ptr(), M, N, K, (int)ksplit,
                         stream());
}

void quant_fp8_rows(torch::Tensor a8, torch::Tensor a_scale,
                    torch::Tensor a) {
  CHECK_DEV(a8); CHECK_CONTIG(a8); CHECK_U8(a8);
  CHECK_DEV(a_scale); CHECK_F32(a_scale);
  CHECK_DEV(a); CHECK_CONTIG(a); CHECK_BF16(a);
  int64_t cols = a.size(-1);
  int64_t rows = a.numel() / cols;
  TORCH_CHECK(cols % 8 == 0, "cols must be a multiple of 8");
  TORCH_CHECK(a8.numel() == a.numel() && a_scale.numel() >= rows,
              "size mismatch");
  launch_quant_fp8_rows(a8.data_ptr(), a_scale.data_ptr(), a.data_ptr(),
                        (int)rows, (int)cols, stream());
}

void cast_f32_bf16(torch::Tensor out, torch::Tensor in) {
  CHECK_DEV(out); CHECK_CONTIG(out); CHECK_BF16(out);
  CHECK_DEV(in); CHECK_CONTIG(in); CHECK_F32(in);
  TORCH_CHECK(out.numel() == in.numel(), "size mismatch");
  launch_cast_f32_bf16(out.data_ptr(), in.data_ptr(), in.numel(), stream());
}

void attn_decode(torch::Tensor o, torch::Tensor q, torch::Tensor kc,
                 torch::Tensor vc, torch::Tensor seq_lens, double scale,
                 c10::optional<torch::Tensor> partial_ws, int64_t nsplit,
                 c10::optional<torch::Tensor> k_scale = c10::nullopt,
                 c10::optional<torch::Tensor> v_scale = c10::nullopt) {
  CHECK_DEV(o); CHECK_CONTIG(o); CHECK_BF16(o);
  CHECK_DEV(q); CHECK_BF16(q);
  CHECK_DEV(kc); CHECK_CONTIG(kc);
  CHECK_DEV(vc); CHECK_CONTIG(vc);
  const bool kvq = k_scale.has_value();
  if (kvq) {
    TORCH_CHECK(v_scale.has_value(), "fp8 KV needs both scales");
    CHECK_U8(kc); CHECK_U8(vc);
    CHECK_DEV(*k_scale); CHECK_CONTIG(*k_scale); CHECK_F32(*k_scale);
    CHECK_DEV(*v_scale); CHECK_CONTIG(*v_scale); CHECK_F32(*v_scale);
  } else {
    CHECK_BF16(kc); CHECK_BF16(vc);
  }
  CHECK_DEV(seq_lens); CHECK_CONTIG(seq_lens); CHECK_I32(seq_lens);
  TORCH_CHECK(q.dim() == 3 && kc.dim() == 4, "q [B,Hq,D], kc [B,Hkv,S,D]");
  long long q_row_stride = check_head_view(q);
  int B = q.size(0), Hq = q.size(1), D = q.size(2);
  int Hkv = kc.size(1), Smax = kc.size(2);
  TORCH_CHECK(D == 128, "attn_decode requires head_dim 128");
  TORCH_CHECK(Hq % Hkv == 0 && Hq / Hkv <= 8,
              "grouped heads per kv head must divide and be <= 8");
  TORCH_CHECK(kc.size(0) == B && kc.size(3) == D, "kc shape mismatch");
  float* ws = nullptr;
  if (nsplit > 1) {
    TORCH_CHECK(partial_ws.has_value(), "nsplit>1 needs partial_ws");
    CHECK_DEV(*partial_ws); CHECK_CONTIG(*partial_ws);
    CHECK_F32(*partial_ws);
    TORCH_CHECK(partial_ws->numel() >=
                (int64_t)B * Hq * nsplit * (D + 2),
                "partial_ws too small");
    ws = (float*)partial_ws->data_ptr();
  }
  if (kvq)
    TORCH_CHECK(k_scale->numel() >= (int64_t)B * Hkv * Smax &&
                v_scale->numel() >= (int64_t)B * Hkv * Smax,
                "scale tensors too small");
  launch_attn_decode(o.data_ptr(), q.data_ptr(), kc.data_ptr(),
                     vc.data_ptr(),
                     kvq ? k_scale->data_ptr() : nullptr,
                     kvq ? v_scale->data_ptr() : nullptr,
                     seq_lens.data_ptr(), B, Hq, Hkv, Smax,
                     (float)scale, q_row_stride, ws, (int)nsplit, stream());
}

void kv_append(torch::Tensor kc, torch::Tensor vc, torch::Tensor knew,
               torch::Tensor vnew, torch::Tensor positions) {
  CHECK_DEV(kc); CHECK_CONTIG(kc); CHECK_BF16(kc);
  CHECK_DEV(knew); CHECK_BF16(knew);
  CHECK_DEV(positions); CHECK_CONTIG(positions); CHECK_I32(positions);
  long long src_stride = check_head_view(knew);
  TORCH_CHECK(check_head_view(vnew) == src_stride,
              "knew/vnew strides must match");
  int B = kc.size(0), Hkv = kc.size(1), Smax = kc.size(2), D = kc.size(3);
  TORCH_CHECK(D % 8 == 0, "head_dim must be a multiple of 8");
  launch_kv_append(kc.data_ptr(), vc.data_ptr(), knew.data_ptr(),
                   vnew.data_ptr(), positions.data_ptr(), B, Hkv, Smax, D,
                   src_stride, stream());
}

void rope_kv_varlen(torch::Tensor qkv, torch::Tensor kc, torch::Tensor vc,
                    torch::Tensor positions, torch::Tensor tok_slot,
                    torch::Tensor cos_sin, int64_t hq) {
  CHECK_DEV(qkv); CHECK_CONTIG(qkv); CHECK_BF16(qkv);
  CHECK_DEV(kc); CHECK_CONTIG(kc); CHECK_BF16(kc);
  CHECK_DEV(vc); CHECK_CONTIG(vc); CHECK_BF16(vc);
  CHECK_DEV(positions); CHECK_CONTIG(positions); CHECK_I32(positions);
  CHECK_DEV(tok_slot); CHECK_CONTIG(tok_slot); CHECK_I32(tok_slot);
  CHECK_DEV(cos_sin); CHECK_CONTIG(cos_sin); CHECK_F32(cos_sin);
  TORCH_CHECK(kc.dim() == 4 && vc.sizes() == kc.sizes(),
              "caches must be [B, Hkv, Smax, D] of equal shape");
  int B = kc.size(0), Hkv = kc.size(1), Smax = kc.size(2), D = kc.size(3);
  TORCH_CHECK(qkv.dim() == 2, "qkv must be [T, rows]");
  int64_t T = qkv.size(0);
  TORCH_CHECK(hq >= 1 && qkv.size(1) >= (hq + 2 * Hkv) * D,
              "qkv row too small");
  TORCH_CHECK(D % 2 == 0 && D / 2 <= 1024, "bad head dim");
  TORCH_CHECK(positions.numel() == T && tok_slot.numel() == T,
              "positions/tok_slot must hold one entry per token");
  TORCH_CHECK(cos_sin.dim() == 3 && cos_sin.size(1) == D / 2 &&
              cos_sin.size(2) == 2, "cos_sin must be [max_pos, D/2, 2]");
  TORCH_CHECK(hq + 2 * Hkv <= 65535, "too many heads");
  if (T == 0) return;
  launch_rope_kv_varlen(qkv.data_ptr(), kc.data_ptr(), vc.data_ptr(),
                        positions.data_ptr(), tok_slot.data_ptr(),
                        cos_sin.data_ptr(), (int)T, B, (int)hq, Hkv, Smax, D,
                        (int)cos_sin.size(0), qkv.size(1), stream());
}

void attn_prefill(torch::Tensor o, torch::Tensor q, torch::Tensor kc,
                  torch::Tensor vc, torch::Tensor cu_seqlens,
                  torch::Tensor slots, torch::Tensor kv_start, double scale,
                  int64_t max_q_len) {
  CHECK_DEV(o); CHECK_CONTIG(o); CHECK_BF16(o);
  CHECK_DEV(q); CHECK_BF16(q);
  CHECK_DEV(kc); CHECK_CONTIG(kc); CHECK_BF16(kc);
  CHECK_DEV(vc); CHECK_CONTIG(vc); CHECK_BF16(vc);
  CHECK_DEV(cu_seqlens); CHECK_CONTIG(cu_seqlens); CHECK_I32(cu_seqlens);
  CHECK_DEV(slots); CHECK_CONTIG(slots); CHECK_I32(slots);
  CHECK_DEV(kv_start); CHECK_CONTIG(kv_start); CHECK_I32(kv_start);
  TORCH_CHECK(kc.dim() == 4 && vc.sizes() == kc.sizes(),
              "caches must be [B, Hkv, Smax, D] of equal shape");
  long long q_row_stride = check_head_view(q);
  int64_t T = q.size(0);
  int Hq = q.size(1), D = q.size(2);
  int B = kc.size(0), Hkv = kc.size(1), Smax = kc.size(2);
  TORCH_CHECK(D == 128 && kc.size(3) == D,
              "attn_prefill requires head_dim 128");
  TORCH_CHECK(Hq % Hkv == 0 && Hq / Hkv <= 8,
              "grouped heads per kv head must divide and be <= 8");
  TORCH_CHECK(o.numel() == T * Hq * D, "out must be [T, Hq*D]");
  TORCH_CHECK(q_row_stride % 8 == 0 &&
              reinterpret_cast<uintptr_t>(q.data_ptr()) % 16 == 0,
              "q rows must be 16-byte aligned");
  int64_t nseq = slots.numel();
  TORCH_CHECK(cu_seqlens.numel() == nseq + 1 && kv_start.numel() == nseq,
              "cu_seqlens [n+1], slots [n], kv_start [n]");
  TORCH_CHECK(nseq <= 65535 && Hq <= 65535, "grid too large");
  TORCH_CHECK(max_q_len >= 0 && max_q_len <= T, "bad max_q_len");
  if (T == 0 || nseq == 0 || max_q_len == 0) return;
  launch_attn_prefill(o.data_ptr(), q.data_ptr(), kc.data_ptr(),
                      vc.data_ptr(), cu_seqlens.data_ptr(),
                      slots.data_ptr(), kv_start.data_ptr(), (int)T,
                      (int)nseq, B, Hq, Hkv, Smax, (float)scale,
                      q_row_stride, (int)max_q_len, stream());
}

void attn_verify(torch::Tensor o, torch::Tensor q, torch::Tensor kc,
                 torch::Tensor vc, torch::Tensor base_lens, double scale,
                 c10::optional<torch::Tensor> partial_ws, int64_t nsplit) {
  CHECK_DEV(o); CHECK_CONTIG(o); CHECK_BF16(o);
  CHECK_DEV(q); CHECK_BF16(q);
  CHECK_DEV(kc); CHECK_CONTIG(kc); CHECK_BF16(kc);
  CHECK_DEV(vc); CHECK_CONTIG(vc); CHECK_BF16(vc);
  CHECK_DEV(base_lens); CHECK_CONTIG(base_lens); CHECK_I32(base_lens);
  TORCH_CHECK(q.dim() == 4, "q must be [B, QL, Hq, D]");
  TORCH_CHECK(kc.dim() == 4 && vc.sizes() == kc.sizes(),
              "caches must be [B, Hkv, Smax, D] of equal shape");
  int64_t B = q.size(0);
  int QL = q.size(1), Hq = q.size(2), D = q.size(3);
  int Hkv = kc.size(1), Smax = kc.size(2);
  TORCH_CHECK(D == 128 && kc.size(3) == D,
              "attn_verify requires head_dim 128");
  TORCH_CHECK(QL >= 1 && QL <= 8, "attn_verify needs 1 <= QL <= 8");
  TORCH_CHECK(Hkv >= 1 && Hq % Hkv == 0 && Hq / Hkv <= 8,
              "grouped heads per kv head must divide and be <= 8");
  TORCH_CHECK(kc.size(0) == B && base_lens.numel() == B,
              "q, caches and base_lens must agree on B");
  TORCH_CHECK(q.stride(3) == 1 && q.stride(2) == D,
              "inner dims must be dense (strides (*, *, dim, 1))");
  long long q_row_stride = QL > 1 ? q.stride(1) : q.stride(0);
  if (B == 1 && QL == 1) q_row_stride = (long long)Hq * D;
  TORCH_CHECK(QL == 1 || B == 1 || q.stride(0) == QL * q.stride(1),
              "q rows must be evenly strided over [B, QL]");
  TORCH_CHECK(q_row_stride >= (long long)Hq * D,
              "q rows must not overlap");
  TORCH_CHECK(q_row_stride % 8 == 0 &&
              reinterpret_cast<uintptr_t>(q.data_ptr()) % 16 == 0,
              "q rows must be 16-byte aligned");
  TORCH_CHECK(o.numel() == B * QL * Hq * D, "out must be [B*QL, Hq*D]");
  TORCH_CHECK(B <= 65535 && Hkv <= 65535, "grid too large");
  TORCH_CHECK(nsplit >= 1 && nsplit <= 1024, "bad nsplit");
  float* ws = nullptr;
  if (nsplit > 1) {
    TORCH_CHECK(partial_ws.has_value(), "nsplit>1 needs partial_ws");
    CHECK_DEV(*partial_ws); CHECK_CONTIG(*partial_ws);
    CHECK_F32(*partial_ws);
    TORCH_CHECK(partial_ws->numel() >=
                B * QL * Hq * nsplit * (int64_t)(D + 4),
                "partial_ws too small");
    TORCH_CHECK(reinterpret_cast<uintptr_t>(partial_ws->data_ptr()) % 16
                == 0, "partial_ws must be 16-byte aligned");
    ws = (float*)partial_ws->data_ptr();
  }
  if (B == 0) return;
  launch_attn_verify(o.data_ptr(), q.data_ptr(), kc.data_ptr(),
                     vc.data_ptr(), base_lens.data_ptr(), (int)B, QL, Hq,
                     Hkv, Smax, (float)scale, q_row_stride, ws,
                     (int)nsplit, stream());
}

void ngram_draft(torch::Tensor drafts, torch::Tensor history,
                 torch::Tensor hist_lens, int64_t n) {
  CHECK_DEV(drafts); CHECK_CONTIG(drafts);
  CHECK_DEV(history); CHECK_CONTIG(history);
  CHECK_DEV(hist_lens); CHECK_CONTIG(hist_lens); CHECK_I32(hist_lens);
  TORCH_CHECK(drafts.scalar_type() == torch::kInt64 &&
              history.scalar_type() == torch::kInt64,
              "drafts and history must be int64");
  TORCH_CHECK(history.dim() == 2 && drafts.dim() == 2,
              "history [B, L], drafts [B, k]");
  int64_t B = history.size(0), L = history.size(1), k = drafts.size(1);
  TORCH_CHECK(drafts.size(0) == B && hist_lens.numel() == B,
              "drafts, history and hist_lens must agree on B");
  TORCH_CHECK(n >= 1 && n <= 64, "ngram_draft needs 1 <= n <= 64");
  TORCH_CHECK(L < (1LL << 30) && k < (1LL << 20), "shape too large");
// ... 78 lines not shown
              top_k.numel() == B && top_p.numel() == B &&
              min_p.numel() == B && seed.numel() == B &&
              out_tokens.numel() == B,
              "sample_tokens: every per-row tensor must hold B entries");
  TORCH_CHECK(reinterpret_cast<uintptr_t>(logits.data_ptr()) % 16 == 0,
              "sample_tokens: logits must be 16-byte aligned");
  void* logprob_ptr = nullptr;
  void* kept_ptr = nullptr;
  if (out_logprob.has_value()) {
    CHECK_DEV(*out_logprob); CHECK_CONTIG(*out_logprob);
    CHECK_F32(*out_logprob);
    TORCH_CHECK(out_logprob->numel() == B,
                "sample_tokens: out_logprob must hold B entries");
    logprob_ptr = out_logprob->data_ptr();
  }
  if (out_kept.has_value()) {
    CHECK_DEV(*out_kept); CHECK_CONTIG(*out_kept); CHECK_I32(*out_kept);
    TORCH_CHECK(out_kept->numel() == B,
                "sample_tokens: out_kept must hold B entries");
    kept_ptr = out_kept->data_ptr();
  }
  if (B == 0) return;
  launch_sample_tokens(logits.data_ptr(), pos.data_ptr(),
                       temperature.data_ptr(), top_k.data_ptr(),
                       top_p.data_ptr(), min_p.data_ptr(), seed.data_ptr(),
                       out_tokens.data_ptr(), logprob_ptr, kept_ptr, (int)B,
                       (int)V, stream());
}

void softmax(torch::Tensor out, torch::Tensor in) {
  CHECK_DEV(out); CHECK_CONTIG(out); CHECK_BF16(out);
  CHECK_DEV(in); CHECK_CONTIG(in); CHECK_BF16(in);
  int64_t cols = in.size(-1);
  int64_t rows = in.numel() / cols;
  launch_softmax(out.data_ptr(), in.data_ptr(), (int)rows, (int)cols,
                 stream());
}

void tree_ensemble(torch::Tensor out, torch::Tensor features,
                   torch::Tensor feature_idx, torch::Tensor threshold,
                   torch::Tensor left, torch::Tensor right,
                   torch::Tensor leaf_value, torch::Tensor tree_offsets,
                   double base_score) {
  CHECK_DEV(out); CHECK_CONTIG(out); CHECK_F32(out);
  CHECK_DEV(features); CHECK_CONTIG(features); CHECK_F32(features);
  CHECK_I32(feature_idx); CHECK_I32(left); CHECK_I32(right);
  CHECK_I32(tree_offsets); CHECK_F32(threshold); CHECK_F32(leaf_value);
  int n_samples = features.size(0), n_features = features.size(1);
  int n_trees = tree_offsets.numel() - 1;
  launch_tree_ensemble(out.data_ptr(), features.data_ptr(),
                       feature_idx.data_ptr(), threshold.data_ptr(),
                       left.data_ptr(), right.data_ptr(),
                       leaf_value.data_ptr(), tree_offsets.data_ptr(),
                       n_trees, n_samples, n_features, (float)base_score,
                       stream());
}

void window_ingest(torch::Tensor ring, torch::Tensor keys,
                   torch::Tensor values, torch::Tensor period_idx) {
  CHECK_DEV(ring); CHECK_CONTIG(ring);
  CHECK_I32(keys); CHECK_F32(values); CHECK_I32(period_idx);
  TORCH_CHECK(ring.dim() == 3 && ring.size(2) == 4,
              "ring must be [keys, periods, 4]");
  if (ring.scalar_type() == torch::kFloat64) {
    launch_window_ingest64(ring.data_ptr(), keys.data_ptr(),
                           values.data_ptr(), period_idx.data_ptr(),
                           keys.numel(), (int)ring.size(1), stream());
    return;
  }
  CHECK_F32(ring);
  launch_window_ingest(ring.data_ptr(), keys.data_ptr(), values.data_ptr(),
                       period_idx.data_ptr(), keys.numel(),
                       (int)ring.size(1), stream());
}

void window_reduce(torch::Tensor out, torch::Tensor ring,
                   int64_t window_periods, int64_t current_period) {
  CHECK_DEV(out); CHECK_CONTIG(out);
  CHECK_DEV(ring); CHECK_CONTIG(ring);
  if (ring.scalar_type() == torch::kFloat64) {
    TORCH_CHECK(out.scalar_type() == torch::kFloat64,
                "out must be f64 for an f64 ring");
    launch_window_reduce64(out.data_ptr(), ring.data_ptr(),
                           (int)ring.size(0), (int)ring.size(1),
                           (int)window_periods, (int)current_period,
                           stream());
    return;
  }
  CHECK_F32(out); CHECK_F32(ring);
  launch_window_reduce(out.data_ptr(), ring.data_ptr(), (int)ring.size(0),
                       (int)ring.size(1), (int)window_periods,
                       (int)current_period, stream());
}

void window_ingest_mm(torch::Tensor ring_mm, torch::Tensor keys,
                      torch::Tensor values, torch::Tensor period_idx) {
  CHECK_DEV(ring_mm); CHECK_CONTIG(ring_mm);
  TORCH_CHECK(ring_mm.scalar_type() == torch::kInt32,
              "ring_mm must be int32 (ordered-f32 bits)");
  CHECK_I32(keys); CHECK_F32(values); CHECK_I32(period_idx);
  TORCH_CHECK(ring_mm.dim() == 3 && ring_mm.size(2) == 2,
              "ring_mm must be [keys, periods, 2]");
  launch_window_ingest_mm(ring_mm.data_ptr(), keys.data_ptr(),
                          values.data_ptr(), period_idx.data_ptr(),
                          keys.numel(), (int)ring_mm.size(1), stream());
}

void window_ingest_fl(torch::Tensor ring_fl, torch::Tensor keys,
                      torch::Tensor values, torch::Tensor timestamps,
                      torch::Tensor period_idx) {
  CHECK_DEV(ring_fl); CHECK_CONTIG(ring_fl);
  TORCH_CHECK(ring_fl.scalar_type() == torch::kInt64,
              "ring_fl must be int64 (packed ts|ordered-f32)");
  CHECK_I32(keys); CHECK_F32(values); CHECK_I32(timestamps);
  CHECK_I32(period_idx);
  TORCH_CHECK(ring_fl.dim() == 3 && ring_fl.size(2) == 2,
              "ring_fl must be [keys, periods, 2]");
  launch_window_ingest_fl(ring_fl.data_ptr(), keys.data_ptr(),
                          values.data_ptr(), timestamps.data_ptr(),
                          period_idx.data_ptr(), keys.numel(),
                          (int)ring_fl.size(1), stream());
}

void window_reduce_mmfl(torch::Tensor out, torch::Tensor ring_mm,
                        torch::Tensor ring_fl, int64_t window_periods,
                        int64_t current_period) {
  CHECK_DEV(out); CHECK_CONTIG(out); CHECK_F32(out);
  CHECK_DEV(ring_mm); CHECK_CONTIG(ring_mm);
  CHECK_DEV(ring_fl); CHECK_CONTIG(ring_fl);
  TORCH_CHECK(out.dim() == 2 && out.size(1) == 4,
              "out must be [keys, 4]");
  launch_window_reduce_mmfl(out.data_ptr(), ring_mm.data_ptr(),
                            ring_fl.data_ptr(), (int)ring_mm.size(0),
                            (int)ring_mm.size(1), (int)window_periods,
                            (int)current_period, stream());
}

PYBIND11_MODULE(TORCH_EXTENSION_NAME, m) {
  m.def("fused_add_rmsnorm", &fused_add_rmsnorm,
        "fused residual add + RMSNorm (bf16)");
  m.def("rope", &rope, "in-place rotary embedding (bf16)");
  m.def("silu_mul", &silu_mul, "silu(gate) * up (bf16)");
  m.def("swiglu_fused", &swiglu_fused,
        "silu(gu[:, :I]) * gu[:, I:] over a fused gate|up buffer");
  m.def("skinny_gemm", &skinny_gemm,
        "decode GEMM C=A@W^T on MFMA (bf16 in/out, split-K f32 slabs)");
  m.def("rope_kv_fused", &rope_kv_fused, py::arg("qkv"), py::arg("kc"),
        py::arg("vc"), py::arg("positions"), py::arg("cos_sin"),
        py::arg("hq"), py::arg("k_scale") = py::none(),
        py::arg("v_scale") = py::none(),
        "fused decode rope(q,k) + KV-cache append");
  m.def("skinny_gemm_slabs", &skinny_gemm_slabs,
        "split-K GEMM emitting f32 slabs only");
  m.def("fused_add_rmsnorm_slab", &fused_add_rmsnorm_slab,
        "slab-sum + residual add + RMSNorm");
  m.def("swiglu_slab", &swiglu_slab, "slab-sum + SwiGLU");
  m.def("rope_kv_slab", &rope_kv_slab,
        "slab-sum + rope(q,k) + KV append");
  m.def("cast_f32_bf16", &cast_f32_bf16, "f32 -> bf16 cast");
  m.def("skinny_gemm_fp8", &skinny_gemm_fp8,
        "fp8-weight decode GEMM (e4m3, per-row scales)");
  m.def("quant_fp8_rows", &quant_fp8_rows,
        "dynamic per-row bf16 -> fp8 e4m3 quantization");
  m.def("attn_decode", &attn_decode, py::arg("o"), py::arg("q"),
        py::arg("kc"), py::arg("vc"), py::arg("seq_lens"),
        py::arg("scale"), py::arg("partial_ws") = py::none(),
        py::arg("nsplit") = 1, py::arg("k_scale") = py::none(),
        py::arg("v_scale") = py::none(),
        "GQA decode attention (bf16 or fp8 KV cache)");
  m.def("kv_append", &kv_append, "append token K/V into cache");
  m.def("rope_kv_varlen", &rope_kv_varlen, py::arg("qkv"), py::arg("kc"),
        py::arg("vc"), py::arg("positions"), py::arg("tok_slot"),
        py::arg("cos_sin"), py::arg("hq"),
        "packed-prefill rope(q,k) + KV append by per-token slot");
  m.def("attn_prefill", &attn_prefill, py::arg("o"), py::arg("q"),
        py::arg("kc"), py::arg("vc"), py::arg("cu_seqlens"),
        py::arg("slots"), py::arg("kv_start"), py::arg("scale"),
        py::arg("max_q_len"),
        "packed causal GQA flash-attention prefill over the KV cache");
  m.def("attn_verify", &attn_verify, py::arg("o"), py::arg("q"),
        py::arg("kc"), py::arg("vc"), py::arg("base_lens"),
        py::arg("scale"), py::arg("partial_ws") = py::none(),
        py::arg("nsplit") = 1,
        "speculative verify attention (QL query rows per sequence)");
  m.def("ngram_draft", &ngram_draft, py::arg("drafts"), py::arg("history"),
        py::arg("hist_lens"), py::arg("n"),
        "device-side prompt-lookup (n-gram) drafter");
  m.def("lora_shrink", &lora_shrink, py::arg("t"), py::arg("x"),
        py::arg("a"), py::arg("idx"),
        "multi-LoRA shrink: t[b] = A[idx[b]] @ x[b] (f32)");
  m.def("lora_expand", &lora_expand, py::arg("y"), py::arg("t"),
        py::arg("bm"), py::arg("idx"),
        "multi-LoRA expand: y[b] += Bm[idx[b]] @ t[b], in place (bf16)");
  m.def("sample_tokens", &sample_tokens, py::arg("logits"), py::arg("pos"),
        py::arg("temperature"), py::arg("top_k"), py::arg("top_p"),
        py::arg("min_p"), py::arg("seed"), py::arg("out_tokens"),
        py::arg("out_logprob") = py::none(),
        py::arg("out_kept") = py::none(),
        "fused seeded sampler: temperature, top_k, top_p, min_p, logprob");
  m.def("softmax", &softmax, "row softmax (bf16)");
  m.def("tree_ensemble", &tree_ensemble, "GBDT ensemble inference (f32)");
  m.def("window_ingest", &window_ingest,
        "feature-store window ring ingest (f32)");
  m.def("window_reduce", &window_reduce,
        "feature-store window ring reduce (f32)");
  m.def("window_ingest_mm", &window_ingest_mm,
        "per-period min/max ingest (ordered-f32 atomics)");
  m.def("window_ingest_fl", &window_ingest_fl,
        "per-period first/last ingest (packed ts|value u64 atomics)");
  m.def("window_reduce_mmfl", &window_reduce_mmfl,
        "window min/max/first/last reduce over period cells");
}
```

mlrun_amd/ops/hip/kernels.h:

```cpp
#pragma once

extern "C++" {

void launch_fused_add_rmsnorm(void* out, void* residual, const void* x,
                              const void* weight, int rows, int hidden,
                              float eps, void* out8, void* out_scale,
                              void* stream);

void launch_rope(void* q, const void* positions, const void* cos_sin, int T,
                 int heads, int dim, long long row_stride, void* stream);

void launch_swiglu_fused(void* out, const void* gu, int rows, int inter,
                         void* stream);

void launch_silu_mul(void* out, const void* gate, const void* up,
                     long long n, void* stream);

void launch_skinny_gemm_slabs(void* part_f32, const void* A, const void* W,
                              int M, int N, int K, int ksplit, int variant,
                              void* stream);

void launch_fused_add_rmsnorm_slab(void* out, void* residual,
                                   const void* slabs, const void* weight,
                                   int rows, int hidden, float eps,
                                   int ksplit, void* stream);

void launch_swiglu_slab(void* out, const void* slabs, int rows, int inter,
                        int ksplit, void* stream);

void launch_rope_kv_slab(void* qkv, void* Kc, void* Vc, const void* slabs,
                         const void* positions, const void* cos_sin, int B,
                         int Hq, int Hkv, int Smax, int D, int qkv_row,
                         int ksplit, void* stream);

void launch_skinny_gemm(void* out_bf16, void* part_f32, const void* A,
                        const void* W, int M, int N, int K, int ksplit,
                        int variant, void* stream);

void launch_rope_kv_fused(void* qkv, void* Kc, void* Vc,
                          const void* positions, const void* cos_sin, int B,
                          int Hq, int Hkv, int Smax, int D,
                          long long row_stride, void* stream);

void launch_rope_kv_fused_q8(void* qkv, void* Kc8, void* Vc8,
                             void* kscale, void* vscale,
                             const void* positions, const void* cos_sin,
                             int B, int Hq, int Hkv, int Smax, int D,
                             long long row_stride, void* stream);

void launch_skinny_gemm_fp8(void* out_bf16, void* part_f32, const void* A8,
                            const void* a_scale, const void* W8,
                            const void* w_scale, int M, int N, int K,
                            int ksplit, void* stream);

void launch_quant_fp8_rows(void* a8, void* a_scale, const void* a, int rows,
                           int cols, void* stream);

void launch_cast_f32_bf16(void* out, const void* in, long long n,
                          void* stream);

void launch_zero_f32(void* p, long long n, void* stream);

void launch_attn_decode(void* O, const void* Q, const void* Kc,
                        const void* Vc, const void* kscale,
                        const void* vscale, const void* seq_lens, int B,
                        int Hq, int Hkv, int Smax, float scale,
                        long long q_row_stride, float* partial_ws,
                        int nsplit, void* stream);

void launch_kv_append(void* Kc, void* Vc, const void* knew, const void* vnew,
                      const void* positions, int B, int Hkv, int Smax, int D,
                      long long src_row_stride, void* stream);

void launch_rope_kv_varlen(void* qkv, void* Kc, void* Vc,
                           const void* positions, const void* tok_slot,
                           const void* cos_sin, int T, int B, int Hq,
                           int Hkv, int Smax, int D, int max_pos,
                           long long row_stride, void* stream);

void launch_attn_prefill(void* O, const void* Q, const void* Kc,
                         const void* Vc, const void* cu_seqlens,
                         const void* slots, const void* kv_start, int T,
                         int nseq, int B, int Hq, int Hkv, int Smax,
                         float scale, long long q_row_stride,
                         int max_q_len, void* stream);

void launch_attn_verify(void* O, const void* Q, const void* Kc,
                        const void* Vc, const void* base_lens, int B,
                        int QL, int Hq, int Hkv, int Smax, float scale,
                        long long q_row_stride, float* partial_ws,
                        int nsplit, void* stream);

void launch_ngram_draft(void* drafts, const void* history,
                        const void* hist_lens, int B, int L, int k, int n,
                        void* stream);

void launch_lora_shrink(void* t, const void* x, const void* A,
                        const void* idx, int B, int NA, int R, int K,
                        void* stream);

void launch_lora_expand(void* y, const void* t, const void* Bm,
                        const void* idx, int B, int NA, int R, int N,
                        void* stream);

void launch_sample_tokens(const void* logits, const void* pos,
                          const void* temperature, const void* top_k,
                          const void* top_p, const void* min_p,
                          const void* seed, void* out_tokens,
                          void* out_logprob, void* out_kept, int B, int V,
                          void* stream);

void launch_softmax(void* out, const void* in, int rows, int cols,
                    void* stream);

void launch_tree_ensemble(void* out, const void* features,
                          const void* feature_idx, const void* threshold,
                          const void* left, const void* right,
                          const void* leaf_value, const void* tree_offsets,
                          int n_trees, int n_samples, int n_features,
                          float base_score, void* stream);

void launch_window_ingest(void* ring, const void* keys, const void* values,
                          const void* period_idx, long long n_events,
                          int n_periods, void* stream);

void launch_window_ingest64(void* ring, const void* keys,
                            const void* values, const void* period_idx,
                            long long n_events, int n_periods,
                            void* stream);
void launch_window_reduce64(void* out, const void* ring, int n_keys,
                            int n_periods, int window_periods,
                            int current_period, void* stream);
void launch_window_ingest_mm(void* ring_mm, const void* keys,
                             const void* values, const void* period_idx,
                             long long n_events, int n_periods,
                             void* stream);
void launch_window_ingest_fl(void* ring_fl, const void* keys,
                             const void* values, const void* timestamps,
                             const void* period_idx, long long n_events,
                             int n_periods, void* stream);
void launch_window_reduce_mmfl(void* out, const void* ring_mm,
                               const void* ring_fl, int n_keys,
                               int n_periods, int window_periods,
                               int current_period, void* stream);
void launch_window_reduce(void* out, const void* ring, int n_keys,
                          int n_periods, int window_periods,
                          int current_period, void* stream);

}
```

mlrun_amd/ops/hip/kernels.hip:

```cpp

#include <hip/hip_fp8.h>
#include <hip/hip_runtime.h>
#include <atomic>
#include <cfloat>
#include <cstdint>
#include <cstring>
#include <mutex>

#include "kernels.h"

typedef __attribute__((ext_vector_type(8))) short short8v;
typedef __attribute__((ext_vector_type(4))) float f32x4v;
typedef __attribute__((ext_vector_type(2))) float f32x2v;

#define DEV __device__ __forceinline__

DEV float bf2f(unsigned short u) {
  union { uint32_t i; float f; } v;
  v.i = uint32_t(u) << 16;
  return v.f;
}

DEV unsigned short f2bf(float f) {
  union { float f; uint32_t i; } v;
// ... 436 lines not shown
template <bool SPLIT, int MT, int DEPTH, int NB = 2>
__global__ __launch_bounds__(256) void skinny_gemm_ws_pipe_kernel(
    void* __restrict__ out, const unsigned short* __restrict__ A,
    const unsigned short* __restrict__ W, int M, int N, int K, int ksplit) {
  const int lane = threadIdx.x & 63;
  const int wave = threadIdx.x >> 6;
  constexpr int NT = 16 * NB;
  const int n0 = blockIdx.x * NT;
  if (n0 >= N) return;
  int cbegin = 0, cend = K;
  if (SPLIT) {
    const int kchunk = (K / ksplit + 31) & ~31;
    cbegin = blockIdx.y * kchunk;
    cend = cbegin + kchunk;
    if (cend > K) cend = K;
  }
  const int clen = cend - cbegin;
  const int per_wave = ((clen / 4) + 31) & ~31;
  int kbegin = cbegin + wave * per_wave;
  int kend = kbegin + per_wave;
  if (kend > cend) kend = cend;

  const int arow = lane & 15;
  const int kb = (lane >> 4) * 8;
  const int brow0 = n0 + (lane & 15);
  const int brow1 = brow0 + 16;

  f32x4v acc0[MT], acc1[MT];
#pragma unroll
  for (int t = 0; t < MT; ++t) {
    acc0[t] = {0.f, 0.f, 0.f, 0.f};
    acc1[t] = {0.f, 0.f, 0.f, 0.f};
  }
  const unsigned short* aptr[MT];
#pragma unroll
  for (int t = 0; t < MT; ++t)
    aptr[t] = A + (size_t)min(arow + 16 * t, M - 1) * K + kb;
  const unsigned short* bptr0 =
      W + (size_t)min(brow0, N - 1) * K + kb;
  const unsigned short* bptr1 =
      W + (size_t)min(NB == 2 ? brow1 : brow0, N - 1) * K + kb;

  short8v a_ring[DEPTH][MT], b0_ring[DEPTH], b1_ring[DEPTH];
  const int nsteps_total = (kend - kbegin) / 32;
  const int ngroups = nsteps_total / DEPTH;
  const int nsteps = ngroups > 0 ? ngroups * DEPTH : 0;
  int kload = kbegin;
  int k = kbegin + nsteps * 32;
  if (nsteps) {
#pragma unroll
    for (int s = 0; s < DEPTH; ++s) {
#pragma unroll
      for (int t = 0; t < MT; ++t)
        a_ring[s][t] =
            *reinterpret_cast<const short8v*>(aptr[t] + kload);
      b0_ring[s] = *reinterpret_cast<const short8v*>(bptr0 + kload);
      if (NB == 2)
        b1_ring[s] = *reinterpret_cast<const short8v*>(bptr1 + kload);
      kload += 32;
    }
    for (int g = DEPTH; g < nsteps; g += DEPTH) {
#pragma unroll
      for (int s = 0; s < DEPTH; ++s) {
#pragma unroll
        for (int t = 0; t < MT; ++t) {
          acc0[t] = __builtin_amdgcn_mfma_f32_16x16x32_bf16(
              a_ring[s][t], b0_ring[s], acc0[t], 0, 0, 0);
          if (NB == 2)
            acc1[t] = __builtin_amdgcn_mfma_f32_16x16x32_bf16(
                a_ring[s][t], b1_ring[s], acc1[t], 0, 0, 0);
        }
#pragma unroll
        for (int t = 0; t < MT; ++t)
          a_ring[s][t] =
              *reinterpret_cast<const short8v*>(aptr[t] + kload);
        b0_ring[s] = *reinterpret_cast<const short8v*>(bptr0 + kload);
        if (NB == 2)
          b1_ring[s] = *reinterpret_cast<const short8v*>(bptr1 + kload);
        kload += 32;
      }
    }
#pragma unroll
    for (int s = 0; s < DEPTH; ++s) {
#pragma unroll
      for (int t = 0; t < MT; ++t) {
        acc0[t] = __builtin_amdgcn_mfma_f32_16x16x32_bf16(
            a_ring[s][t], b0_ring[s], acc0[t], 0, 0, 0);
        if (NB == 2)
          acc1[t] = __builtin_amdgcn_mfma_f32_16x16x32_bf16(
              a_ring[s][t], b1_ring[s], acc1[t], 0, 0, 0);
      }
    }
  }
  for (; k < kend; k += 32) {
    short8v bf0 = *reinterpret_cast<const short8v*>(bptr0 + k);
#pragma unroll
    for (int t = 0; t < MT; ++t) {
      short8v af = *reinterpret_cast<const short8v*>(aptr[t] + k);
      acc0[t] = __builtin_amdgcn_mfma_f32_16x16x32_bf16(af, bf0, acc0[t],
                                                        0, 0, 0);
      if (NB == 2) {
        short8v bf1 = *reinterpret_cast<const short8v*>(bptr1 + k);
        acc1[t] = __builtin_amdgcn_mfma_f32_16x16x32_bf16(af, bf1,
                                                          acc1[t], 0, 0,
                                                          0);
      }
    }
  }

  __shared__ float comb[4][16 * MT][NT];
  const int crow_base = (lane >> 4) * 4;
  const int ccol = lane & 15;
#pragma unroll
  for (int t = 0; t < MT; ++t)
#pragma unroll
    for (int r = 0; r < 4; ++r) {
      comb[wave][16 * t + crow_base + r][ccol] = acc0[t][r];
      if (NB == 2)
        comb[wave][16 * t + crow_base + r][ccol + 16] = acc1[t][r];
    }
  __syncthreads();
  if (wave == 0) {
    constexpr int CPL = 4 * MT * NB;
#pragma unroll
    for (int c = 0; c < CPL; ++c) {
      const int cell = lane * CPL + c;
      const int m = cell / NT;
      const int n = cell % NT;
      if (m >= M || n0 + n >= N) continue;
      float sum = comb[0][m][n] + comb[1][m][n] + comb[2][m][n] +
                  comb[3][m][n];
      if (SPLIT) {
        float* part = (float*)out + (size_t)blockIdx.y * M * N;
        part[(size_t)m * N + n0 + n] = sum;
      } else {
        ((unsigned short*)out)[(size_t)m * N + n0 + n] = f2bf(sum);
      }
    }
  }
}

template <int STAGE_K>
DEV int lds_ring_swz(int row) {
  return STAGE_K == 64 ? ((row >> 1) & 7) : (row & 15);
}

template <int N>
DEV void wait_vmcnt() {
  asm volatile("s_waitcnt vmcnt(%0)" ::"n"(N) : "memory");
}

typedef __attribute__((address_space(3))) void* lds_void_ptr;

template <bool SPLIT, int STAGE_K, int DEPTH>
__global__ __launch_bounds__(256) void skinny_gemm_ws_lds_kernel(
    void* __restrict__ out, const unsigned short* __restrict__ A,
    const unsigned short* __restrict__ W, int M, int N, int K, int ksplit) {
  constexpr int MT = 2, NT = 32;
  constexpr int ROW_B = STAGE_K * 2;
  constexpr int OP_B = 32 * ROW_B;
  constexpr int SLOT_B = 2 * OP_B;
  constexpr int WAVE_B = DEPTH * SLOT_B;
  constexpr int LPR = ROW_B / 16;
  constexpr int RPI = 64 / LPR;
  constexpr int NDMA_OP = 32 / RPI;
  constexpr int NDMA = 2 * NDMA_OP;
  constexpr int SPS = STAGE_K / 32;
  static_assert(WAVE_B >= 4 * 16 * MT * NT, "comb aliases the ring");
  extern __shared__ __attribute__((aligned(1024))) unsigned char lds_ring[];

  const int lane = threadIdx.x & 63;
  const int wave = __builtin_amdgcn_readfirstlane(threadIdx.x >> 6);
  const int n0 = blockIdx.x * NT;
  if (n0 >= N) return;
  int cbegin = 0, cend = K;
  if (SPLIT) {
    const int kchunk = (K / ksplit + 31) & ~31;
    cbegin = blockIdx.y * kchunk;
    cend = cbegin + kchunk;
    if (cend > K) cend = K;
  }
  const int clen = cend - cbegin;
  const int per_wave = ((clen / 4) + 31) & ~31;
  int kbegin = cbegin + wave * per_wave;
  int kend = kbegin + per_wave;
  if (kend > cend) kend = cend;
  const int nst = kend > kbegin ? (kend - kbegin) / STAGE_K : 0;

  f32x4v acc0[MT], acc1[MT];
#pragma unroll
  for (int t = 0; t < MT; ++t) {
    acc0[t] = {0.f, 0.f, 0.f, 0.f};
    acc1[t] = {0.f, 0.f, 0.f, 0.f};
  }

  const unsigned short* wsrc[NDMA_OP];
  const unsigned short* asrc[NDMA_OP];
#pragma unroll
  for (int i = 0; i < NDMA_OP; ++i) {
    const int row = i * RPI + lane / LPR;
    const int chunk = (lane % LPR) ^ lds_ring_swz<STAGE_K>(row);
    wsrc[i] = W + (size_t)min(n0 + row, N - 1) * K + kbegin + chunk * 8;
    asrc[i] = A + (size_t)min(row, M - 1) * K + kbegin + chunk * 8;
  }
  unsigned char* const ring = lds_ring + wave * WAVE_B;
  int rd_off[SPS];
#pragma unroll
  for (int s = 0; s < SPS; ++s) {
    const int row = lane & 15;
    rd_off[s] = row * ROW_B +
                ((((lane >> 4) + 4 * s) ^ lds_ring_swz<STAGE_K>(row)) << 4);
  }

  auto issue = [&](int stage, int slot) {
    unsigned char* dst = ring + slot * SLOT_B;
    const int koff = stage * STAGE_K;
#if defined(__HIP_DEVICE_COMPILE__)
#pragma unroll
    for (int i = 0; i < NDMA_OP; ++i)
      __builtin_amdgcn_global_load_lds(wsrc[i] + koff,
                                       (lds_void_ptr)(dst + i * 1024), 16,
                                       0, 2);
#pragma unroll
    for (int i = 0; i < NDMA_OP; ++i)
      __builtin_amdgcn_global_load_lds(asrc[i] + koff,
                                       (lds_void_ptr)(dst + OP_B + i * 1024),
                                       16, 0, 0);
#else
    (void)dst;
    (void)koff;
#endif
  };
  auto consume = [&](int slot, int refill) {
    const unsigned char* src = ring + slot * SLOT_B;
    short8v bf0[SPS], bf1[SPS], af[SPS][MT];
#pragma unroll
    for (int s = 0; s < SPS; ++s) {
      bf0[s] = *reinterpret_cast<const short8v*>(src + rd_off[s]);
      bf1[s] =
          *reinterpret_cast<const short8v*>(src + rd_off[s] + 16 * ROW_B);
#pragma unroll
      for (int t = 0; t < MT; ++t)
        af[s][t] = *reinterpret_cast<const short8v*>(
            src + OP_B + rd_off[s] + 16 * t * ROW_B);
    }
    asm volatile("s_waitcnt lgkmcnt(0)" ::: "memory");
    __builtin_amdgcn_sched_barrier(0);
    if (refill >= 0) issue(refill, slot);
#pragma unroll
    for (int s = 0; s < SPS; ++s)
#pragma unroll
      for (int t = 0; t < MT; ++t) {
        acc0[t] = __builtin_amdgcn_mfma_f32_16x16x32_bf16(
            af[s][t], bf0[s], acc0[t], 0, 0, 0);
        acc1[t] = __builtin_amdgcn_mfma_f32_16x16x32_bf16(
            af[s][t], bf1[s], acc1[t], 0, 0, 0);
      }
  };

#pragma unroll
  for (int s = 0; s < DEPTH; ++s)
    if (s < nst) issue(s, s);
  int j = 0, slot = 0;
  for (; j + DEPTH < nst; ++j) {
    wait_vmcnt<NDMA*(DEPTH - 1)>();
    consume(slot, j + DEPTH);
    slot = slot + 1 == DEPTH ? 0 : slot + 1;
  }
  static_assert(DEPTH == 2 || DEPTH == 3, "drain is written for 2 and 3");
  if (DEPTH == 3 && nst - j == 3) {
    wait_vmcnt<2 * NDMA>();
    consume(slot, -1);
    slot = slot + 1 == DEPTH ? 0 : slot + 1;
    ++j;
  }
  if (nst - j == 2) {
    wait_vmcnt<NDMA>();
    consume(slot, -1);
    slot = slot + 1 == DEPTH ? 0 : slot + 1;
    ++j;
  }
  if (nst - j == 1) {
    wait_vmcnt<0>();
    consume(slot, -1);
  }

  if (kend > kbegin) {
    const int arow = lane & 15;
    const int kb = (lane >> 4) * 8;
    const unsigned short* aptr0 = A + (size_t)min(arow, M - 1) * K + kb;
    const unsigned short* aptr1 =
        A + (size_t)min(arow + 16, M - 1) * K + kb;
    const unsigned short* bptr0 =
        W + (size_t)min(n0 + arow, N - 1) * K + kb;
    const unsigned short* bptr1 =
        W + (size_t)min(n0 + arow + 16, N - 1) * K + kb;
    for (int k = kbegin + nst * STAGE_K; k < kend; k += 32) {
      short8v bf0 = *reinterpret_cast<const short8v*>(bptr0 + k);
      short8v bf1 = *reinterpret_cast<const short8v*>(bptr1 + k);
      short8v af0 = *reinterpret_cast<const short8v*>(aptr0 + k);
      short8v af1 = *reinterpret_cast<const short8v*>(aptr1 + k);
      acc0[0] = __builtin_amdgcn_mfma_f32_16x16x32_bf16(af0, bf0, acc0[0],
                                                        0, 0, 0);
      acc1[0] = __builtin_amdgcn_mfma_f32_16x16x32_bf16(af0, bf1, acc1[0],
                                                        0, 0, 0);
      acc0[1] = __builtin_amdgcn_mfma_f32_16x16x32_bf16(af1, bf0, acc0[1],
                                                        0, 0, 0);
      acc1[1] = __builtin_amdgcn_mfma_f32_16x16x32_bf16(af1, bf1, acc1[1],
                                                        0, 0, 0);
    }
  }

  asm volatile("s_waitcnt vmcnt(0) lgkmcnt(0)" ::: "memory");
  typedef float comb_t[16 * MT][NT];
  comb_t& mine = *reinterpret_cast<comb_t*>(ring);
  const int crow_base = (lane >> 4) * 4;
  const int ccol = lane & 15;
#pragma unroll
  for (int t = 0; t < MT; ++t)
#pragma unroll
    for (int r = 0; r < 4; ++r) {
      mine[16 * t + crow_base + r][ccol] = acc0[t][r];
      mine[16 * t + crow_base + r][ccol + 16] = acc1[t][r];
    }
  __syncthreads();
  if (wave == 0) {
    const comb_t& c0 = *reinterpret_cast<const comb_t*>(lds_ring);
    const comb_t& c1 = *reinterpret_cast<const comb_t*>(lds_ring + WAVE_B);
    const comb_t& c2 =
        *reinterpret_cast<const comb_t*>(lds_ring + 2 * WAVE_B);
    const comb_t& c3 =
        *reinterpret_cast<const comb_t*>(lds_ring + 3 * WAVE_B);
    constexpr int CPL = 4 * MT * 2;
#pragma unroll
    for (int c = 0; c < CPL; ++c) {
      const int cell = lane * CPL + c;
      const int m = cell / NT;
      const int n = cell % NT;
      if (m >= M || n0 + n >= N) continue;
      float sum = c0[m][n] + c1[m][n] + c2[m][n] + c3[m][n];
      if (SPLIT) {
        float* part = (float*)out + (size_t)blockIdx.y * M * N;
        part[(size_t)m * N + n0 + n] = sum;
      } else {
        ((unsigned short*)out)[(size_t)m * N + n0 + n] = f2bf(sum);
      }
    }
  }
}

__global__ void reduce_cast_kernel(unsigned short* __restrict__ out,
                                   const float* __restrict__ part,
                                   long long mn, int ksplit);

template <bool SPLIT, int MT>
__global__ __launch_bounds__(256) void skinny_gemm_fp8_kernel(
    void* __restrict__ out, const unsigned char* __restrict__ A8,
    const float* __restrict__ a_scale,
    const unsigned char* __restrict__ W8,
    const float* __restrict__ w_scale, int M, int N, int K, int ksplit) {
  const int lane = threadIdx.x & 63;
  const int wave = threadIdx.x >> 6;
  const int n0 = blockIdx.x * 32;
  if (n0 >= N) return;
  int cbegin = 0, cend = K;
  if (SPLIT) {
    const int kchunk = (K / ksplit + 63) & ~63;
    cbegin = blockIdx.y * kchunk;
    cend = cbegin + kchunk;
    if (cend > K) cend = K;
  }
  const int clen = cend - cbegin;
  const int per_wave = ((clen / 4) + 63) & ~63;
  int kbegin = cbegin + wave * per_wave;
  int kend = kbegin + per_wave;
  if (kend > cend) kend = cend;

  const int arow = lane & 15;
  const int kb2 = (lane >> 4) * 16;
  const int brow0 = n0 + (lane & 15);
  const int brow1 = brow0 + 16;

  f32x4v acc0[MT], acc1[MT];
#pragma unroll
  for (int t = 0; t < MT; ++t) {
    acc0[t] = {0.f, 0.f, 0.f, 0.f};
    acc1[t] = {0.f, 0.f, 0.f, 0.f};
  }
  typedef __attribute__((ext_vector_type(2))) long long2v;
  const unsigned char* aptr[MT];
#pragma unroll
  for (int t = 0; t < MT; ++t)
    aptr[t] = A8 + (size_t)min(arow + 16 * t, M - 1) * K + kb2;
  const unsigned char* bptr0 = W8 + (size_t)min(brow0, N - 1) * K + kb2;
  const unsigned char* bptr1 = W8 + (size_t)min(brow1, N - 1) * K + kb2;

  constexpr int UNR = (MT == 1) ? 8 : (MT == 2 ? 4 : 2);
  int k = kbegin;
  const int kend8 = kbegin + ((kend - kbegin) & ~(UNR * 64 - 1));
  for (; k < kend8; k += UNR * 64) {
    long2v af[UNR][MT], bf0[UNR], bf1[UNR];
#pragma unroll
    for (int u = 0; u < UNR; ++u) {
#pragma unroll
      for (int t = 0; t < MT; ++t)
        af[u][t] =
            *reinterpret_cast<const long2v*>(aptr[t] + k + u * 64);
      bf0[u] = *reinterpret_cast<const long2v*>(bptr0 + k + u * 64);
      bf1[u] = *reinterpret_cast<const long2v*>(bptr1 + k + u * 64);
    }
#pragma unroll
    for (int u = 0; u < UNR; ++u) {
#pragma unroll
      for (int t = 0; t < MT; ++t) {
        acc0[t] = __builtin_amdgcn_mfma_f32_16x16x32_fp8_fp8(
            af[u][t][0], bf0[u][0], acc0[t], 0, 0, 0);
        acc1[t] = __builtin_amdgcn_mfma_f32_16x16x32_fp8_fp8(
            af[u][t][0], bf1[u][0], acc1[t], 0, 0, 0);
        acc0[t] = __builtin_amdgcn_mfma_f32_16x16x32_fp8_fp8(
            af[u][t][1], bf0[u][1], acc0[t], 0, 0, 0);
        acc1[t] = __builtin_amdgcn_mfma_f32_16x16x32_fp8_fp8(
            af[u][t][1], bf1[u][1], acc1[t], 0, 0, 0);
      }
    }
  }
  for (; k < kend; k += 64) {
    long2v bf0 = *reinterpret_cast<const long2v*>(bptr0 + k);
    long2v bf1 = *reinterpret_cast<const long2v*>(bptr1 + k);
#pragma unroll
    for (int t = 0; t < MT; ++t) {
      long2v af = *reinterpret_cast<const long2v*>(aptr[t] + k);
      acc0[t] = __builtin_amdgcn_mfma_f32_16x16x32_fp8_fp8(
          af[0], bf0[0], acc0[t], 0, 0, 0);
      acc1[t] = __builtin_amdgcn_mfma_f32_16x16x32_fp8_fp8(
          af[0], bf1[0], acc1[t], 0, 0, 0);
      acc0[t] = __builtin_amdgcn_mfma_f32_16x16x32_fp8_fp8(
          af[1], bf0[1], acc0[t], 0, 0, 0);
      acc1[t] = __builtin_amdgcn_mfma_f32_16x16x32_fp8_fp8(
          af[1], bf1[1], acc1[t], 0, 0, 0);
    }
  }

  __shared__ float comb[4][16 * MT][32];
  const int crow_base = (lane >> 4) * 4;
  const int ccol = lane & 15;
#pragma unroll
  for (int t = 0; t < MT; ++t)
#pragma unroll
    for (int r = 0; r < 4; ++r) {
      comb[wave][16 * t + crow_base + r][ccol] = acc0[t][r];
      comb[wave][16 * t + crow_base + r][ccol + 16] = acc1[t][r];
    }
  __syncthreads();
  if (wave == 0) {
#pragma unroll
    for (int c = 0; c < 8 * MT; ++c) {
      const int cell = lane * 8 * MT + c;
      const int m = cell >> 5;
      const int n = cell & 31;
      if (m >= M || n0 + n >= N) continue;
      float sum = (comb[0][m][n] + comb[1][m][n] + comb[2][m][n] +
                   comb[3][m][n]) * a_scale[m] * w_scale[n0 + n];
      if (SPLIT) {
        float* part = (float*)out + (size_t)blockIdx.y * M * N;
        part[(size_t)m * N + n0 + n] = sum;
      } else {
        ((unsigned short*)out)[(size_t)m * N + n0 + n] = f2bf(sum);
      }
    }
  }
}

void launch_skinny_gemm_fp8(void* out_bf16, void* part_f32, const void* A8,
                            const void* a_scale, const void* W8,
                            const void* w_scale, int M, int N, int K,
                            int ksplit, void* stream) {
  const int nblocks = (N + 31) / 32;
  const dim3 grid(nblocks, ksplit > 1 ? ksplit : 1);
#define FP8_DISPATCH(SPLIT, DEST)                                         \
  do {                                                                    \
    if (M > 32)                                                           \
      hipLaunchKernelGGL((skinny_gemm_fp8_kernel<SPLIT, 4>), grid,        \
                         dim3(256), 0, (hipStream_t)stream, DEST,         \
                         (const unsigned char*)A8, (const float*)a_scale, \
                         (const unsigned char*)W8, (const float*)w_scale, \
// ... 17 lines not shown
    FP8_DISPATCH(true, part_f32);
    long long mn = (long long)M * N;
    long long blocks = (mn / 4 + 255) / 256;
    if (blocks > 2048) blocks = 2048;
    if (blocks < 1) blocks = 1;
    hipLaunchKernelGGL(reduce_cast_kernel, dim3((int)blocks), dim3(256), 0,
                       (hipStream_t)stream, (unsigned short*)out_bf16,
                       (const float*)part_f32, mn, ksplit);
  }
#undef FP8_DISPATCH
}

__global__ void quant_fp8_rows_kernel(unsigned char* __restrict__ a8,
                                      float* __restrict__ a_scale,
                                      const unsigned short* __restrict__ a,
                                      int cols) {
  const int row = blockIdx.x;
  const int tid = threadIdx.x;
  const unsigned short* ar = a + (size_t)row * cols;
  unsigned char* outr = a8 + (size_t)row * cols;
  float amax = 0.f;
  for (int i = tid * 8; i < cols; i += blockDim.x * 8) {
    ushort8 v = *reinterpret_cast<const ushort8*>(ar + i);
#pragma unroll
    for (int j = 0; j < 8; ++j) amax = fmaxf(amax, fabsf(bf2f(v.v[j])));
  }
  __shared__ float red[32];
#pragma unroll
  for (int off = 32; off > 0; off >>= 1)
    amax = fmaxf(amax, __shfl_xor(amax, off, 64));
  if ((tid & 63) == 0) red[tid >> 6] = amax;
  __syncthreads();
  float gmax = 0.f;
  for (int w = 0; w < (blockDim.x >> 6); ++w) gmax = fmaxf(gmax, red[w]);
  const float scale = gmax > 0.f ? gmax / 448.f : 1.f;
  const float inv = 1.f / scale;
  if (tid == 0) a_scale[row] = scale;
  for (int i = tid * 8; i < cols; i += blockDim.x * 8) {
    ushort8 v = *reinterpret_cast<const ushort8*>(ar + i);
    unsigned char q[8];
#pragma unroll
    for (int j = 0; j < 8; ++j) {
      const float scaled = bf2f(v.v[j]) * inv;
      __hip_fp8_e4m3 f8(scaled);
      q[j] = f8.__x;
    }
    const int s = i >> 5;
    const int c = (i >> 3) & 3;
    const int dst = ((s >> 1) << 6) + (c << 4) + ((s & 1) << 3);
    *reinterpret_cast<uint64_t*>(outr + dst) =
        *reinterpret_cast<const uint64_t*>(q);
  }
}

void launch_quant_fp8_rows(void* a8, void* a_scale, const void* a, int rows,
                           int cols, void* stream) {
  int threads = cols >= 2048 ? 256 : 64;
  hipLaunchKernelGGL(quant_fp8_rows_kernel, dim3(rows), dim3(threads), 0,
                     (hipStream_t)stream, (unsigned char*)a8,
                     (float*)a_scale, (const unsigned short*)a, cols);
}

__global__ void reduce_cast_kernel(unsigned short* __restrict__ out,
                                   const float* __restrict__ part,
                                   long long mn, int ksplit) {
  long long i = ((long long)blockIdx.x * blockDim.x + threadIdx.x) * 4;
  long long stride = (long long)gridDim.x * blockDim.x * 4;
  for (; i + 3 < mn; i += stride) {
    f32x4v sum = *reinterpret_cast<const f32x4v*>(part + i);
    for (int s = 1; s < ksplit; ++s) {
      f32x4v v = *reinterpret_cast<const f32x4v*>(part + (size_t)s * mn + i);
#pragma unroll
      for (int j = 0; j < 4; ++j) sum[j] += v[j];
    }
    unsigned short o[4];
#pragma unroll
    for (int j = 0; j < 4; ++j) o[j] = f2bf(sum[j]);
    *reinterpret_cast<uint64_t*>(out + i) =
        *reinterpret_cast<const uint64_t*>(o);
  }
  if (blockIdx.x == 0 && threadIdx.x == 0) {
    for (long long t = (mn & ~3LL); t < mn; ++t) {
      float sum = part[t];
      for (int s = 1; s < ksplit; ++s) sum += part[(size_t)s * mn + t];
      out[t] = f2bf(sum);
    }
  }
}

static int gemm_unr2_env() {
  static int v = [] {
    const char* e = getenv("MLRUN_GEMM_UNR2");
    return e ? atoi(e) : 4;
  }();
  return v;
}

static int gemm_pipe_env() {
  static int v = [] {
    const char* e = getenv("MLRUN_GEMM_PIPE");
    return e ? atoi(e) : 4;
  }();
  return v;
}

template <bool SPLIT>
static bool launch_pipe_mt2(void* out, const void* A, const void* W,
                            int M, int N, int K, int ksplit,
                            const dim3& grid, void* stream) {
  const int depth = gemm_pipe_env();
  if (depth < 2) return false;
  auto kern = depth >= 6 ? (skinny_gemm_ws_pipe_kernel<SPLIT, 2, 6>)
              : depth >= 4 ? (skinny_gemm_ws_pipe_kernel<SPLIT, 2, 4>)
                           : (skinny_gemm_ws_pipe_kernel<SPLIT, 2, 3>);
  hipLaunchKernelGGL(kern, grid, dim3(256), 0, (hipStream_t)stream, out,
                     (const unsigned short*)A, (const unsigned short*)W,
                     M, N, K, ksplit);
  return true;
}

static int gemm_lds_ring_env() {
  static int v = [] {
    const char* e = getenv("MLRUN_GEMM_LDS_RING");
    if (e && !strcmp(e, "64x3")) return 1;
    if (e && !strcmp(e, "128x2")) return 2;
    return 0;
  }();
  return v;
}

typedef void (*lds_ring_kern_t)(void*, const unsigned short*,
                                const unsigned short*, int, int, int, int);

template <int STAGE_K, int DEPTH>
constexpr int lds_ring_bytes() {
  return 4 * DEPTH * 2 * 32 * STAGE_K * 2;
}

static void lds_ring_allow_all() {
  static std::mutex mu;
  static std::atomic<bool> done[16];
  int dev = 0;
  if (hipGetDevice(&dev) != hipSuccess || dev < 0 || dev >= 16) dev = 0;
  if (done[dev].load(std::memory_order_acquire)) return;
  std::lock_guard<std::mutex> lock(mu);
  if (done[dev].load(std::memory_order_relaxed)) return;
  const struct { lds_ring_kern_t kern; int bytes; } all[] = {
      {skinny_gemm_ws_lds_kernel<false, 64, 2>, lds_ring_bytes<64, 2>()},
      {skinny_gemm_ws_lds_kernel<true, 64, 2>, lds_ring_bytes<64, 2>()},
      {skinny_gemm_ws_lds_kernel<false, 64, 3>, lds_ring_bytes<64, 3>()},
      {skinny_gemm_ws_lds_kernel<true, 64, 3>, lds_ring_bytes<64, 3>()},
      {skinny_gemm_ws_lds_kernel<false, 128, 2>, lds_ring_bytes<128, 2>()},
      {skinny_gemm_ws_lds_kernel<true, 128, 2>, lds_ring_bytes<128, 2>()},
  };
  for (const auto& k : all)
    (void)hipFuncSetAttribute(reinterpret_cast<const void*>(k.kern),
                              hipFuncAttributeMaxDynamicSharedMemorySize,
                              k.bytes);
  done[dev].store(true, std::memory_order_release);
}

template <bool SPLIT, int STAGE_K, int DEPTH>
static void launch_lds_ring(void* out, const void* A, const void* W, int M,
                            int N, int K, int ksplit, const dim3& grid,
                            void* stream) {
  lds_ring_kern_t kern = skinny_gemm_ws_lds_kernel<SPLIT, STAGE_K, DEPTH>;
  constexpr int bytes = lds_ring_bytes<STAGE_K, DEPTH>();
  lds_ring_allow_all();
  hipLaunchKernelGGL(kern, grid, dim3(256), bytes, (hipStream_t)stream, out,
                     (const unsigned short*)A, (const unsigned short*)W, M,
                     N, K, ksplit);
}

template <bool SPLIT>
static void launch_lds_mt2(void* out, const void* A, const void* W, int M,
                           int N, int K, int ksplit, const dim3& grid,
                           void* stream) {
  switch (gemm_lds_ring_env()) {
    case 1:
      launch_lds_ring<SPLIT, 64, 3>(out, A, W, M, N, K, ksplit, grid,
                                    stream);
      break;
    case 2:
      launch_lds_ring<SPLIT, 128, 2>(out, A, W, M, N, K, ksplit, grid,
                                     stream);
      break;
    default:
      launch_lds_ring<SPLIT, 64, 2>(out, A, W, M, N, K, ksplit, grid,
                                    stream);
  }
}

void launch_skinny_gemm_slabs(void* part_f32, const void* A, const void* W,
                              int M, int N, int K, int ksplit, int variant,
                              void* stream) {
  const int nblocks = variant == 3 ? (N + 15) / 16
                      : variant >= 1 ? (N + 31) / 32 : (N + 127) / 128;
  const dim3 grid(nblocks, ksplit);
  if (variant == 4 && M > 16 && M <= 32) {
    launch_lds_mt2<true>(part_f32, A, W, M, N, K, ksplit, grid, stream);
  } else if (variant == 3) {
    if (M > 32)
      hipLaunchKernelGGL((skinny_gemm_ws_kernel<true, 4, 4, 1>), grid,
                         dim3(256), 0, (hipStream_t)stream, part_f32,
                         (const unsigned short*)A, (const unsigned short*)W,
                         M, N, K, ksplit);
    else if (M > 16)
      hipLaunchKernelGGL((skinny_gemm_ws_kernel<true, 2, 4, 1>), grid,
                         dim3(256), 0, (hipStream_t)stream, part_f32,
                         (const unsigned short*)A, (const unsigned short*)W,
                         M, N, K, ksplit);
    else
      hipLaunchKernelGGL((skinny_gemm_ws_kernel<true, 1, 4, 1>), grid,
                         dim3(256), 0, (hipStream_t)stream, part_f32,
                         (const unsigned short*)A, (const unsigned short*)W,
                         M, N, K, ksplit);
  } else if (variant >= 1) {
    if (M > 32)
      hipLaunchKernelGGL((skinny_gemm_ws_kernel<true, 4>), grid, dim3(256),
                         0, (hipStream_t)stream, part_f32,
                         (const unsigned short*)A, (const unsigned short*)W,
                         M, N, K, ksplit);
    else if (M > 16) {
      if (!launch_pipe_mt2<true>(part_f32, A, W, M, N, K, ksplit, grid,
                                 stream))
        hipLaunchKernelGGL(gemm_unr2_env() >= 8
                               ? (skinny_gemm_ws_kernel<true, 2, 8>)
                               : (skinny_gemm_ws_kernel<true, 2, 4>),
                           grid, dim3(256),
                           0, (hipStream_t)stream, part_f32,
                           (const unsigned short*)A,
                           (const unsigned short*)W, M, N, K, ksplit);
    }
    else
      hipLaunchKernelGGL((skinny_gemm_ws_kernel<true, 1>), grid, dim3(256),
                         0, (hipStream_t)stream, part_f32,
                         (const unsigned short*)A, (const unsigned short*)W,
                         M, N, K, ksplit);
  } else {
    if (M > 32)
      hipLaunchKernelGGL((skinny_gemm_kernel<true, 4>), grid, dim3(256), 0,
                         (hipStream_t)stream, part_f32,
                         (const unsigned short*)A, (const unsigned short*)W,
                         M, N, K, ksplit);
    else if (M > 16)
      hipLaunchKernelGGL((skinny_gemm_kernel<true, 2>), grid, dim3(256), 0,
                         (hipStream_t)stream, part_f32,
                         (const unsigned short*)A, (const unsigned short*)W,
                         M, N, K, ksplit);
    else
      hipLaunchKernelGGL((skinny_gemm_kernel<true, 1>), grid, dim3(256), 0,
                         (hipStream_t)stream, part_f32,
                         (const unsigned short*)A, (const unsigned short*)W,
                         M, N, K, ksplit);
  }
}

void launch_skinny_gemm(void* out_bf16, void* part_f32, const void* A,
                        const void* W, int M, int N, int K, int ksplit,
                        int variant, void* stream) {
  if (ksplit < 1) ksplit = 1;
  const int nblocks = variant == 3 ? (N + 15) / 16
                      : variant >= 1 ? (N + 31) / 32 : (N + 127) / 128;
  if (ksplit == 1) {
    if (variant == 4 && M > 16 && M <= 32) {
      launch_lds_mt2<false>(out_bf16, A, W, M, N, K, 1, dim3(nblocks),
                            stream);
    } else if (variant == 3) {
      if (M > 32)
        hipLaunchKernelGGL((skinny_gemm_ws_kernel<false, 4, 4, 1>),
                           dim3(nblocks), dim3(256), 0,
                           (hipStream_t)stream, out_bf16,
                           (const unsigned short*)A,
                           (const unsigned short*)W, M, N, K, 1);
      else if (M > 16)
        hipLaunchKernelGGL((skinny_gemm_ws_kernel<false, 2, 4, 1>),
                           dim3(nblocks), dim3(256), 0,
                           (hipStream_t)stream, out_bf16,
                           (const unsigned short*)A,
                           (const unsigned short*)W, M, N, K, 1);
      else
        hipLaunchKernelGGL((skinny_gemm_ws_kernel<false, 1, 4, 1>),
                           dim3(nblocks), dim3(256), 0,
                           (hipStream_t)stream, out_bf16,
                           (const unsigned short*)A,
                           (const unsigned short*)W, M, N, K, 1);
    } else if (variant >= 1) {
      if (M > 32)
        hipLaunchKernelGGL((skinny_gemm_ws_kernel<false, 4>),
                           dim3(nblocks), dim3(256), 0,
                           (hipStream_t)stream, out_bf16,
                           (const unsigned short*)A,
                           (const unsigned short*)W, M, N, K, 1);
      else if (M > 16) {
        if (!launch_pipe_mt2<false>(out_bf16, A, W, M, N, K, 1,
                                    dim3(nblocks), stream))
          hipLaunchKernelGGL(gemm_unr2_env() >= 8
                                 ? (skinny_gemm_ws_kernel<false, 2, 8>)
                                 : (skinny_gemm_ws_kernel<false, 2, 4>),
                             dim3(nblocks), dim3(256), 0,
                             (hipStream_t)stream, out_bf16,
                             (const unsigned short*)A,
                             (const unsigned short*)W, M, N, K, 1);
      }
      else
        hipLaunchKernelGGL((skinny_gemm_ws_kernel<false, 1>),
                           dim3(nblocks), dim3(256), 0,
                           (hipStream_t)stream, out_bf16,
                           (const unsigned short*)A,
                           (const unsigned short*)W, M, N, K, 1);
    } else {
      if (M > 32)
        hipLaunchKernelGGL((skinny_gemm_kernel<false, 4>), dim3(nblocks),
                           dim3(256), 0, (hipStream_t)stream, out_bf16,
                           (const unsigned short*)A,
                           (const unsigned short*)W, M, N, K, 1);
      else if (M > 16)
        hipLaunchKernelGGL((skinny_gemm_kernel<false, 2>), dim3(nblocks),
                           dim3(256), 0, (hipStream_t)stream, out_bf16,
                           (const unsigned short*)A,
                           (const unsigned short*)W, M, N, K, 1);
      else
        hipLaunchKernelGGL((skinny_gemm_kernel<false, 1>), dim3(nblocks),
                           dim3(256), 0, (hipStream_t)stream, out_bf16,
                           (const unsigned short*)A,
                           (const unsigned short*)W, M, N, K, 1);
    }
  } else {
    launch_skinny_gemm_slabs(part_f32, A, W, M, N, K, ksplit, variant,
                             stream);
    long long mn = (long long)M * N;
    long long blocks = (mn / 4 + 255) / 256;
    if (blocks > 2048) blocks = 2048;
    if (blocks < 1) blocks = 1;
    hipLaunchKernelGGL(reduce_cast_kernel, dim3((int)blocks), dim3(256), 0,
                       (hipStream_t)stream, (unsigned short*)out_bf16,
                       (const float*)part_f32, mn, ksplit);
  }
}

__global__ void cast_f32_bf16_kernel(unsigned short* __restrict__ out,
                                     const float* __restrict__ in,
                                     long long n) {
  long long i = ((long long)blockIdx.x * blockDim.x + threadIdx.x) * 4;
  long long stride = (long long)gridDim.x * blockDim.x * 4;
  for (; i + 3 < n; i += stride) {
    f32x4v v = *reinterpret_cast<const f32x4v*>(in + i);
    unsigned short o[4];
#pragma unroll
    for (int j = 0; j < 4; ++j) o[j] = f2bf(v[j]);
    *reinterpret_cast<uint64_t*>(out + i) =
        *reinterpret_cast<const uint64_t*>(o);
  }
  if (blockIdx.x == 0 && threadIdx.x == 0) {
    for (long long t = (n & ~3LL); t < n; ++t) out[t] = f2bf(in[t]);
  }
}

void launch_cast_f32_bf16(void* out, const void* in, long long n,
                          void* stream) {
  long long blocks = (n / 4 + 255) / 256;
  if (blocks > 2048) blocks = 2048;
  if (blocks < 1) blocks = 1;
  hipLaunchKernelGGL(cast_f32_bf16_kernel, dim3((int)blocks), dim3(256), 0,
                     (hipStream_t)stream, (unsigned short*)out,
                     (const float*)in, n);
}

__global__ void zero_f32_kernel(float* __restrict__ p, long long n) {
  long long i = (long long)blockIdx.x * blockDim.x + threadIdx.x;
  long long stride = (long long)gridDim.x * blockDim.x;
  for (; i < n; i += stride) p[i] = 0.f;
}

void launch_zero_f32(void* p, long long n, void* stream) {
  long long blocks = (n + 255) / 256;
  if (blocks > 2048) blocks = 2048;
  hipLaunchKernelGGL(zero_f32_kernel, dim3((int)blocks), dim3(256), 0,
                     (hipStream_t)stream, (float*)p, n);
}


DEV float slab_sum(const float* __restrict__ slabs, size_t idx,
                   size_t slab_stride, int ksplit) {
  float sum = slabs[idx];
  for (int s = 1; s < ksplit; ++s) sum += slabs[idx + s * slab_stride];
  return sum;
}

__global__ void fused_add_rmsnorm_slab_kernel(
    unsigned short* __restrict__ out, unsigned short* __restrict__ residual,
    const float* __restrict__ slabs,
    const unsigned short* __restrict__ weight, int hidden, float eps,
    int ksplit) {
  const int row = blockIdx.x;
  const int tid = threadIdx.x;
  const int nthreads = blockDim.x;
  const size_t rowbase = (size_t)row * hidden;
  const size_t slab_stride = (size_t)gridDim.x * hidden;
  unsigned short* rr = residual + rowbase;
  unsigned short* outr = out + rowbase;

  float sumsq = 0.f;
  for (int i = tid * 4; i < hidden; i += nthreads * 4) {
    float z[4];
#pragma unroll
    for (int j = 0; j < 4; ++j)
      z[j] = slab_sum(slabs, rowbase + i + j, slab_stride, ksplit);
    unsigned short rv[4];
    *reinterpret_cast<uint64_t*>(rv) =
        *reinterpret_cast<const uint64_t*>(rr + i);
#pragma unroll
    for (int j = 0; j < 4; ++j) {
      z[j] += bf2f(rv[j]);
      rv[j] = f2bf(z[j]);
      sumsq += z[j] * z[j];
    }
    *reinterpret_cast<uint64_t*>(rr + i) =
        *reinterpret_cast<const uint64_t*>(rv);
  }
  __shared__ float red[32];
#pragma unroll
  for (int off = 32; off > 0; off >>= 1)
    sumsq += __shfl_down(sumsq, off, 64);
  if ((tid & 63) == 0) red[tid >> 6] = sumsq;
  __syncthreads();
  if (tid < (nthreads >> 6)) sumsq = red[tid];
  else sumsq = 0.f;
  if (tid < 64) {
#pragma unroll
    for (int off = 2; off > 0; off >>= 1)
      sumsq += __shfl_down(sumsq, off, 64);
  }
  if (tid == 0) red[0] = sumsq;
  __syncthreads();
  const float inv = rsqrtf(red[0] / hidden + eps);
  for (int i = tid * 8; i < hidden; i += nthreads * 8) {
    ushort8 zv = *reinterpret_cast<const ushort8*>(rr + i);
    ushort8 wv = *reinterpret_cast<const ushort8*>(weight + i);
    ushort8 ov;
#pragma unroll
    for (int j = 0; j < 8; ++j)
      ov.v[j] = f2bf(bf2f(zv.v[j]) * inv * bf2f(wv.v[j]));
    *reinterpret_cast<ushort8*>(outr + i) = ov;
  }
}

void launch_fused_add_rmsnorm_slab(void* out, void* residual,
                                   const void* slabs, const void* weight,
                                   int rows, int hidden, float eps,
                                   int ksplit, void* stream) {
  int threads = hidden >= 2048 ? 256 : 64;
  hipLaunchKernelGGL(fused_add_rmsnorm_slab_kernel, dim3(rows),
                     dim3(threads), 0, (hipStream_t)stream,
                     (unsigned short*)out, (unsigned short*)residual,
                     (const float*)slabs, (const unsigned short*)weight,
                     hidden, eps, ksplit);
}

__global__ void swiglu_slab_kernel(unsigned short* __restrict__ out,
                                   const float* __restrict__ slabs,
                                   int rows, int inter, int ksplit) {
  const size_t slab_stride = (size_t)rows * 2 * inter;
  const long long total = (long long)rows * inter / 4;
  long long i = (long long)blockIdx.x * blockDim.x + threadIdx.x;
  long long stride = (long long)gridDim.x * blockDim.x;
  for (; i < total; i += stride) {
    const long long flat = i * 4;
    const int r = (int)(flat / inter);
    const int c = (int)(flat % inter);
    const size_t base = (size_t)r * 2 * inter + c;
    unsigned short o[4];
#pragma unroll
    for (int j = 0; j < 4; ++j) {
      const float g = slab_sum(slabs, base + j, slab_stride, ksplit);
      const float u = slab_sum(slabs, base + inter + j, slab_stride,
                               ksplit);
      const float s = g / (1.f + __expf(-g));
      o[j] = f2bf(s * u);
    }
    *reinterpret_cast<uint64_t*>(out + (size_t)r * inter + c) =
        *reinterpret_cast<const uint64_t*>(o);
  }
}

void launch_swiglu_slab(void* out, const void* slabs, int rows, int inter,
                        int ksplit, void* stream) {
  long long blocks = ((long long)rows * inter / 4 + 255) / 256;
  if (blocks > 2048) blocks = 2048;
  if (blocks < 1) blocks = 1;
  hipLaunchKernelGGL(swiglu_slab_kernel, dim3((int)blocks), dim3(256), 0,
                     (hipStream_t)stream, (unsigned short*)out,
                     (const float*)slabs, rows, inter, ksplit);
}

__global__ void rope_kv_slab_kernel(
    unsigned short* __restrict__ qkv, unsigned short* __restrict__ Kc,
    unsigned short* __restrict__ Vc, const float* __restrict__ slabs,
    const int* __restrict__ positions, const float* __restrict__ cos_sin,
    int Hq, int Hkv, int Smax, int D, int qkv_row, int ksplit) {
  const int b = blockIdx.x;
  const int y = blockIdx.y;
  const int i = threadIdx.x;
  const int half = D >> 1;
  const int pos = positions[b];
  const size_t slab_stride = (size_t)gridDim.x * qkv_row;
  const size_t base = (size_t)b * qkv_row + (size_t)y * D;
  const float lo_f = slab_sum(slabs, base + i, slab_stride, ksplit);
  const float hi_f = slab_sum(slabs, base + i + half, slab_stride, ksplit);
  if (y < Hq + Hkv) {
    const float c = cos_sin[((size_t)pos * half + i) * 2];
    const float s = cos_sin[((size_t)pos * half + i) * 2 + 1];
    const unsigned short lo = f2bf(lo_f * c - hi_f * s);
    const unsigned short hi = f2bf(hi_f * c + lo_f * s);
    if (y < Hq) {
      unsigned short* qrow = qkv + (size_t)b * qkv_row + (size_t)y * D;
      qrow[i] = lo;
      qrow[i + half] = hi;
    } else {
      const int kvh = y - Hq;
      unsigned short* dst =
          Kc + (((size_t)b * Hkv + kvh) * Smax + pos) * D;
      dst[i] = lo;
      dst[i + half] = hi;
    }
  } else {
    const int kvh = y - Hq - Hkv;
    unsigned short* dst = Vc + (((size_t)b * Hkv + kvh) * Smax + pos) * D;
    dst[i] = f2bf(lo_f);
    dst[i + half] = f2bf(hi_f);
  }
}

void launch_rope_kv_slab(void* qkv, void* Kc, void* Vc, const void* slabs,
                         const void* positions, const void* cos_sin, int B,
                         int Hq, int Hkv, int Smax, int D, int qkv_row,
                         int ksplit, void* stream) {
  hipLaunchKernelGGL(rope_kv_slab_kernel, dim3(B, Hq + 2 * Hkv),
                     dim3(D / 2), 0, (hipStream_t)stream,
                     (unsigned short*)qkv, (unsigned short*)Kc,
                     (unsigned short*)Vc, (const float*)slabs,
                     (const int*)positions, (const float*)cos_sin, Hq, Hkv,
                     Smax, D, qkv_row, ksplit);
}

__global__ void rope_kv_fused_kernel(
    unsigned short* __restrict__ qkv, unsigned short* __restrict__ Kc,
    unsigned short* __restrict__ Vc, const int* __restrict__ positions,
    const float* __restrict__ cos_sin, int Hq, int Hkv, int Smax, int D,
    long long row_stride) {
  const int b = blockIdx.x;
  const int y = blockIdx.y;
  const int i = threadIdx.x;
  const int half = D >> 1;
  const int pos = positions[b];
  unsigned short* row = qkv + (size_t)b * row_stride;
  if (y < Hq + Hkv) {
    unsigned short* head = row + (size_t)y * D;
    const float c = cos_sin[((size_t)pos * half + i) * 2];
    const float s = cos_sin[((size_t)pos * half + i) * 2 + 1];
    const float a = bf2f(head[i]);
    const float bvf = bf2f(head[i + half]);
    const unsigned short lo = f2bf(a * c - bvf * s);
    const unsigned short hi = f2bf(bvf * c + a * s);
    head[i] = lo;
    head[i + half] = hi;
    if (y >= Hq) {
      const int kvh = y - Hq;
      unsigned short* dst = Kc +
          (((size_t)b * Hkv + kvh) * Smax + pos) * D;
      dst[i] = lo;
      dst[i + half] = hi;
    }
  } else {
    const int kvh = y - Hq - Hkv;
    const unsigned short* src = row + (size_t)(Hq + Hkv + kvh) * D;
    unsigned short* dst = Vc + (((size_t)b * Hkv + kvh) * Smax + pos) * D;
    dst[i] = src[i];
    dst[i + half] = src[i + half];
  }
}

__global__ void rope_kv_fused_q8_kernel(
    unsigned short* __restrict__ qkv, unsigned char* __restrict__ Kc8,
    unsigned char* __restrict__ Vc8, float* __restrict__ kscale,
    float* __restrict__ vscale, const int* __restrict__ positions,
    const float* __restrict__ cos_sin, int Hq, int Hkv, int Smax, int D,
    long long row_stride) {
  const int b = blockIdx.x;
  const int y = blockIdx.y;
  const int i = threadIdx.x;
  const int half = D >> 1;
  const int pos = positions[b];
  unsigned short* row = qkv + (size_t)b * row_stride;
  float lo_f = 0.f, hi_f = 0.f;
  if (y < Hq + Hkv) {
    unsigned short* head = row + (size_t)y * D;
    const float c = cos_sin[((size_t)pos * half + i) * 2];
    const float sn = cos_sin[((size_t)pos * half + i) * 2 + 1];
    const float a = bf2f(head[i]);
    const float bvf = bf2f(head[i + half]);
    lo_f = a * c - bvf * sn;
    hi_f = bvf * c + a * sn;
    head[i] = f2bf(lo_f);
    head[i + half] = f2bf(hi_f);
    if (y < Hq) return;
  } else {
    const unsigned short* src = row + (size_t)y * D;
    lo_f = bf2f(src[i]);
    hi_f = bf2f(src[i + half]);
  }
  float amax = fmaxf(fabsf(lo_f), fabsf(hi_f));
#pragma unroll
  for (int off = 32; off > 0; off >>= 1)
    amax = fmaxf(amax, __shfl_xor(amax, off, 64));
  const float qs = (amax > 0.f) ? amax / 448.f : 1.f;
  const float qinv = 1.f / qs;
  const bool is_k = (y < Hq + Hkv);
  const int kvh = is_k ? (y - Hq) : (y - Hq - Hkv);
  const size_t rowi = ((size_t)b * Hkv + kvh) * Smax + pos;
  unsigned char* dst = (is_k ? Kc8 : Vc8) + rowi * D;
  __hip_fp8_e4m3 lo8(lo_f * qinv), hi8(hi_f * qinv);
  dst[i] = lo8.__x;
  dst[i + half] = hi8.__x;
  if (i == 0) (is_k ? kscale : vscale)[rowi] = qs;
}

void launch_rope_kv_fused(void* qkv, void* Kc, void* Vc,
                          const void* positions, const void* cos_sin, int B,
                          int Hq, int Hkv, int Smax, int D,
                          long long row_stride, void* stream) {
  hipLaunchKernelGGL(rope_kv_fused_kernel, dim3(B, Hq + 2 * Hkv),
                     dim3(D / 2), 0, (hipStream_t)stream,
                     (unsigned short*)qkv, (unsigned short*)Kc,
                     (unsigned short*)Vc, (const int*)positions,
                     (const float*)cos_sin, Hq, Hkv, Smax, D, row_stride);
}

void launch_rope_kv_fused_q8(void* qkv, void* Kc8, void* Vc8,
                             void* kscale, void* vscale,
                             const void* positions, const void* cos_sin,
                             int B, int Hq, int Hkv, int Smax, int D,
                             long long row_stride, void* stream) {
  hipLaunchKernelGGL(rope_kv_fused_q8_kernel, dim3(B, Hq + 2 * Hkv),
                     dim3(D / 2), 0, (hipStream_t)stream,
                     (unsigned short*)qkv, (unsigned char*)Kc8,
                     (unsigned char*)Vc8, (float*)kscale, (float*)vscale,
                     (const int*)positions, (const float*)cos_sin, Hq,
                     Hkv, Smax, D, row_stride);
}

#define ATTN_SCHUNK 64
#define ATTN_MAXG 8

struct AttnState {
  float m, l, acc0, acc1;
};

struct uchar16v { unsigned char v[16]; };

#define ATTN_LDS_PAD 8
template <int SCHUNK, bool KVQ>
__device__ __forceinline__ AttnState attn_chunk_loop(
    const void* __restrict__ kbase_, const void* __restrict__ vbase_,
    const float* __restrict__ kscale, const float* __restrict__ vscale,
    const float* qf, float scale, int s_begin, int s_final,
    int wave, int lane, int tid, int nthreads,
    unsigned short (*kbuf)[128 + ATTN_LDS_PAD],
    unsigned short (*vbuf)[128 + ATTN_LDS_PAD],
    float (*scores)[SCHUNK]) {
  constexpr int D = 128;
  AttnState st = {-FLT_MAX, 0.f, 0.f, 0.f};
  const int d0 = lane * 2;
  for (int s0 = s_begin; s0 < s_final; s0 += SCHUNK) {
    const int cnt = min(SCHUNK, s_final - s0);
    if (!KVQ) {
      const unsigned short* kbase = (const unsigned short*)kbase_;
      const unsigned short* vbase = (const unsigned short*)vbase_;
      const int total_vec = cnt * (D / 8);
      for (int i = tid; i < total_vec; i += nthreads) {
        const int row = i >> 4;
        const int col = (i & 15) * 8;
        const size_t off = (size_t)(s0 + row) * D + col;
        *reinterpret_cast<ushort8*>(&kbuf[row][col]) =
            *reinterpret_cast<const ushort8*>(kbase + off);
        *reinterpret_cast<ushort8*>(&vbuf[row][col]) =
            *reinterpret_cast<const ushort8*>(vbase + off);
      }
    } else {
      const unsigned char* k8 = (const unsigned char*)kbase_;
      const unsigned char* v8 = (const unsigned char*)vbase_;
      const int total_vec = cnt * (D / 16);
      for (int i = tid; i < total_vec; i += nthreads) {
        const int row = i >> 3;
        const int col = (i & 7) * 16;
        const size_t off = (size_t)(s0 + row) * D + col;
        const uchar16v kq = *reinterpret_cast<const uchar16v*>(k8 + off);
        const uchar16v vq = *reinterpret_cast<const uchar16v*>(v8 + off);
        const float ks = kscale[s0 + row];
        const float vs = vscale[s0 + row];
#pragma unroll
        for (int j = 0; j < 16; ++j) {
          __hip_fp8_e4m3 kf8, vf8;
          kf8.__x = kq.v[j];
          vf8.__x = vq.v[j];
          kbuf[row][col + j] = f2bf(float(kf8) * ks);
          vbuf[row][col + j] = f2bf(float(vf8) * vs);
        }
      }
    }
    __syncthreads();
    for (int si = lane >> 4; si < cnt; si += 4) {
      const unsigned short* kp = &kbuf[si][(lane & 15) * 8];
      ushort8 kv = *reinterpret_cast<const ushort8*>(kp);
      float dot = 0.f;
#pragma unroll
      for (int j = 0; j < 8; ++j) dot += qf[j] * bf2f(kv.v[j]);
#pragma unroll
      for (int off = 8; off > 0; off >>= 1)
        dot += __shfl_xor(dot, off, 64);
      if ((lane & 15) == 0) scores[wave][si] = dot * scale;
    }
    __syncthreads();
    float cm = -FLT_MAX;
    for (int si = lane; si < cnt; si += 64)
      cm = fmaxf(cm, scores[wave][si]);
#pragma unroll
    for (int off = 32; off > 0; off >>= 1)
      cm = fmaxf(cm, __shfl_xor(cm, off, 64));
    const float m_new = fmaxf(st.m, cm);
    const float rescale = (st.m == -FLT_MAX) ? 0.f : __expf(st.m - m_new);
    st.acc0 *= rescale;
    st.acc1 *= rescale;
    st.l *= rescale;
    for (int si = 0; si < cnt; ++si) {
      const float p = __expf(scores[wave][si] - m_new);
      st.l += p;
      const ushort2v vv =
          *reinterpret_cast<const ushort2v*>(&vbuf[si][d0]);
      st.acc0 += p * bf2f(vv.x);
      st.acc1 += p * bf2f(vv.y);
    }
    st.m = m_new;
    __syncthreads();
  }
  return st;
}

template <int SCHUNK, bool KVQ = false>
__global__ void attn_decode_kernel(
    unsigned short* __restrict__ O, const unsigned short* __restrict__ Q,
    const void* __restrict__ Kc, const void* __restrict__ Vc,
    const float* __restrict__ kscale, const float* __restrict__ vscale,
    const int* __restrict__ seq_lens, int B, int Hq, int Hkv, int Smax,
    float scale, long long q_row_stride) {
  constexpr int D = 128;
  const int b = blockIdx.x / Hkv;
  const int kvh = blockIdx.x % Hkv;
  const int G = Hq / Hkv;
  const int wave = threadIdx.x >> 6;
  const int lane = threadIdx.x & 63;
  const int h = kvh * G + wave;
  const int len = seq_lens[b];

  __shared__ float scores[ATTN_MAXG][SCHUNK];
  __shared__ __align__(16) unsigned short kbuf[SCHUNK][D + ATTN_LDS_PAD];
  __shared__ __align__(16) unsigned short vbuf[SCHUNK][D + ATTN_LDS_PAD];

  const unsigned short* qp = Q + (size_t)b * q_row_stride +
                             (size_t)h * D + (lane & 15) * 8;
  float qf[8];
  {
    ushort8 qv = *reinterpret_cast<const ushort8*>(qp);
#pragma unroll
    for (int j = 0; j < 8; ++j) qf[j] = bf2f(qv.v[j]);
  }

  const size_t kv_row = ((size_t)b * Hkv + kvh) * Smax;
  const AttnState st = attn_chunk_loop<SCHUNK, KVQ>(
      (const char*)Kc + kv_row * D * (KVQ ? 1 : 2),
      (const char*)Vc + kv_row * D * (KVQ ? 1 : 2),
      kscale ? kscale + kv_row : nullptr,
      vscale ? vscale + kv_row : nullptr, qf, scale, 0, len, wave, lane,
      threadIdx.x, G * 64, kbuf, vbuf, scores);

  const float inv = (st.l > 0.f) ? 1.f / st.l : 0.f;
  unsigned short* op = O + ((size_t)b * Hq + h) * D + lane * 2;
  op[0] = f2bf(st.acc0 * inv);
  op[1] = f2bf(st.acc1 * inv);
}

template <int SCHUNK, bool KVQ = false>
__global__ void attn_decode_split_kernel(
    float* __restrict__ partial, const unsigned short* __restrict__ Q,
    const void* __restrict__ Kc, const void* __restrict__ Vc,
    const float* __restrict__ kscale, const float* __restrict__ vscale,
    const int* __restrict__ seq_lens, int B, int Hq, int Hkv, int Smax,
    float scale, long long q_row_stride, int nsplit) {
  constexpr int D = 128;
  const int b = blockIdx.x / Hkv;
  const int kvh = blockIdx.x % Hkv;
  const int split = blockIdx.y;
  const int G = Hq / Hkv;
  const int wave = threadIdx.x >> 6;
  const int lane = threadIdx.x & 63;
  const int h = kvh * G + wave;
  const int len = seq_lens[b];
  const int per = (len + nsplit - 1) / nsplit;
  const int s_begin = split * per;
  const int s_final = min(len, s_begin + per);
  float* prow = partial + (((size_t)b * Hq + h) * nsplit + split) * (D + 2);

  __shared__ float scores[ATTN_MAXG][SCHUNK];
  __shared__ __align__(16) unsigned short kbuf[SCHUNK][D + ATTN_LDS_PAD];
  __shared__ __align__(16) unsigned short vbuf[SCHUNK][D + ATTN_LDS_PAD];

  const unsigned short* qp = Q + (size_t)b * q_row_stride +
                             (size_t)h * D + (lane & 15) * 8;
  float qf[8];
  {
    ushort8 qv = *reinterpret_cast<const ushort8*>(qp);
#pragma unroll
    for (int j = 0; j < 8; ++j) qf[j] = bf2f(qv.v[j]);
  }
  const size_t kv_row = ((size_t)b * Hkv + kvh) * Smax;
  const AttnState st = attn_chunk_loop<SCHUNK, KVQ>(
      (const char*)Kc + kv_row * D * (KVQ ? 1 : 2),
      (const char*)Vc + kv_row * D * (KVQ ? 1 : 2),
      kscale ? kscale + kv_row : nullptr,
      vscale ? vscale + kv_row : nullptr, qf, scale, s_begin, s_final,
      wave, lane, threadIdx.x, G * 64, kbuf, vbuf, scores);

  prow[lane * 2] = st.acc0;
  prow[lane * 2 + 1] = st.acc1;
  if (lane == 0) {
    prow[D] = st.m;
    prow[D + 1] = st.l;
  }
}

__global__ void attn_decode_combine_kernel(
    unsigned short* __restrict__ O, const float* __restrict__ partial,
    int Hq, int nsplit) {
  constexpr int D = 128;
  const int bh = blockIdx.x;
  const int lane = threadIdx.x;
  const float* base = partial + (size_t)bh * nsplit * (D + 2);
  float m_star = -FLT_MAX;
  for (int s = 0; s < nsplit; ++s)
    m_star = fmaxf(m_star, base[s * (D + 2) + D]);
  float l_total = 0.f, a0 = 0.f, a1 = 0.f;
  for (int s = 0; s < nsplit; ++s) {
    const float* prow = base + s * (D + 2);
    const float ms = prow[D];
    if (ms == -FLT_MAX) continue;
    const float wgt = __expf(ms - m_star);
    l_total += wgt * prow[D + 1];
    a0 += wgt * prow[lane * 2];
    a1 += wgt * prow[lane * 2 + 1];
  }
  const float inv = (l_total > 0.f) ? 1.f / l_total : 0.f;
  unsigned short* op = O + (size_t)bh * D + lane * 2;
  op[0] = f2bf(a0 * inv);
  op[1] = f2bf(a1 * inv);
}

static int attn_schunk_env() {
  static int v = [] {
    const char* e = getenv("MLRUN_ATTN_SCHUNK");
    return e ? atoi(e) : 32;
  }();
  return v;
}

void launch_attn_decode(void* O, const void* Q, const void* Kc,
                        const void* Vc, const void* kscale,
                        const void* vscale, const void* seq_lens, int B,
                        int Hq, int Hkv, int Smax, float scale,
                        long long q_row_stride, float* partial_ws,
                        int nsplit, void* stream) {
  const int G = Hq / Hkv;
  const bool c64 = attn_schunk_env() >= 64;
  const bool kvq = kscale != nullptr;
  if (nsplit <= 1 || partial_ws == nullptr) {
    auto* kern = kvq ? (c64 ? attn_decode_kernel<64, true>
                            : attn_decode_kernel<32, true>)
                     : (c64 ? attn_decode_kernel<64, false>
                            : attn_decode_kernel<32, false>);
    hipLaunchKernelGGL(kern, dim3(B * Hkv), dim3(G * 64), 0,
                       (hipStream_t)stream, (unsigned short*)O,
                       (const unsigned short*)Q, Kc, Vc,
                       (const float*)kscale, (const float*)vscale,
                       (const int*)seq_lens, B,
                       Hq, Hkv, Smax, scale, q_row_stride);
    return;
  }
  auto* kern = kvq ? (c64 ? attn_decode_split_kernel<64, true>
                          : attn_decode_split_kernel<32, true>)
                   : (c64 ? attn_decode_split_kernel<64, false>
                          : attn_decode_split_kernel<32, false>);
  hipLaunchKernelGGL(kern, dim3(B * Hkv, nsplit),
                     dim3(G * 64), 0, (hipStream_t)stream, partial_ws,
                     (const unsigned short*)Q, Kc, Vc,
                     (const float*)kscale, (const float*)vscale,
                     (const int*)seq_lens, B, Hq,
                     Hkv, Smax, scale, q_row_stride, nsplit);
  hipLaunchKernelGGL(attn_decode_combine_kernel, dim3(B * Hq), dim3(64), 0,
                     (hipStream_t)stream, (unsigned short*)O, partial_ws,
                     Hq, nsplit);
}

__global__ void kv_append_kernel(unsigned short* __restrict__ Kc,
                                 unsigned short* __restrict__ Vc,
                                 const unsigned short* __restrict__ knew,
                                 const unsigned short* __restrict__ vnew,
                                 const int* __restrict__ positions, int Hkv,
                                 int Smax, int D, long long src_row_stride) {
  const int b = blockIdx.x;
  const int kvh = blockIdx.y;
  const int pos = positions[b];
  const size_t src = (size_t)b * src_row_stride + (size_t)kvh * D;
  const size_t dst = (((size_t)b * Hkv + kvh) * Smax + pos) * D;
  for (int i = threadIdx.x * 8; i < D; i += blockDim.x * 8) {
    *reinterpret_cast<ushort8*>(Kc + dst + i) =
        *reinterpret_cast<const ushort8*>(knew + src + i);
    *reinterpret_cast<ushort8*>(Vc + dst + i) =
        *reinterpret_cast<const ushort8*>(vnew + src + i);
  }
}

void launch_kv_append(void* Kc, void* Vc, const void* knew, const void* vnew,
                      const void* positions, int B, int Hkv, int Smax, int D,
                      long long src_row_stride, void* stream) {
  hipLaunchKernelGGL(kv_append_kernel, dim3(B, Hkv), dim3(D / 8), 0,
                     (hipStream_t)stream, (unsigned short*)Kc,
                     (unsigned short*)Vc, (const unsigned short*)knew,
                     (const unsigned short*)vnew, (const int*)positions, Hkv,
                     Smax, D, src_row_stride);
}

__global__ void rope_kv_varlen_kernel(
    unsigned short* __restrict__ qkv, unsigned short* __restrict__ Kc,
    unsigned short* __restrict__ Vc, const int* __restrict__ positions,
    const int* __restrict__ tok_slot, const float* __restrict__ cos_sin,
    int B, int Hq, int Hkv, int Smax, int D, int max_pos,
    long long row_stride) {
  const int t = blockIdx.x;
  const int y = blockIdx.y;
  const int i = threadIdx.x;
  const int half = D >> 1;
  const int pos = positions[t];
  const int slot = tok_slot[t];
  if (pos < 0 || pos >= max_pos || pos >= Smax ||
      (unsigned)slot >= (unsigned)B)
    return;
  unsigned short* row = qkv + (size_t)t * row_stride;
  if (y < Hq + Hkv) {
    unsigned short* head = row + (size_t)y * D;
    const float c = cos_sin[((size_t)pos * half + i) * 2];
    const float s = cos_sin[((size_t)pos * half + i) * 2 + 1];
    const float a = bf2f(head[i]);
    const float bvf = bf2f(head[i + half]);
    const unsigned short lo = f2bf(a * c - bvf * s);
    const unsigned short hi = f2bf(bvf * c + a * s);
    head[i] = lo;
    head[i + half] = hi;
    if (y >= Hq) {
      const int kvh = y - Hq;
      unsigned short* dst = Kc +
          (((size_t)slot * Hkv + kvh) * Smax + pos) * D;
      dst[i] = lo;
      dst[i + half] = hi;
    }
  } else {
    const int kvh = y - Hq - Hkv;
    const unsigned short* src = row + (size_t)(Hq + Hkv + kvh) * D;
    unsigned short* dst =
        Vc + (((size_t)slot * Hkv + kvh) * Smax + pos) * D;
    dst[i] = src[i];
    dst[i + half] = src[i + half];
  }
}

void launch_rope_kv_varlen(void* qkv, void* Kc, void* Vc,
                           const void* positions, const void* tok_slot,
                           const void* cos_sin, int T, int B, int Hq,
                           int Hkv, int Smax, int D, int max_pos,
                           long long row_stride, void* stream) {
  hipLaunchKernelGGL(rope_kv_varlen_kernel, dim3(T, Hq + 2 * Hkv),
                     dim3(D / 2), 0, (hipStream_t)stream,
                     (unsigned short*)qkv, (unsigned short*)Kc,
                     (unsigned short*)Vc, (const int*)positions,
                     (const int*)tok_slot, (const float*)cos_sin, B, Hq,
                     Hkv, Smax, D, max_pos, row_stride);
}

#define PF_BM 64
#define PF_BN 64
#define PF_ROW (128 + 16)

typedef __attribute__((ext_vector_type(4))) short short4v;

DEV short4v pf_read_tr16(const unsigned short* p) {
  return __builtin_amdgcn_ds_read_tr16_b64_v4i16(
      (__attribute__((address_space(3))) short4v*)p);
}

DEV short pf_f2bf(float f) {
  return __builtin_bit_cast(short, (__bf16)f);
}

__global__ __launch_bounds__(256) void attn_prefill_kernel(
    unsigned short* __restrict__ O, const unsigned short* __restrict__ Q,
    const unsigned short* __restrict__ Kc,
    const unsigned short* __restrict__ Vc,
    const int* __restrict__ cu_seqlens, const int* __restrict__ slots,
    const int* __restrict__ kv_start, int T, int B, int Hq, int Hkv,
    int Smax, float scale_log2e, long long q_row_stride) {
  constexpr int D = 128;
  __shared__ __attribute__((aligned(16)))
      unsigned short lds[2 * PF_BN * PF_ROW];
  unsigned short* kbuf = lds;
  unsigned short* vbuf = lds + PF_BN * PF_ROW;

  const int seq = blockIdx.z;
  const int h = blockIdx.y;
  const int q0 = blockIdx.x * PF_BM;
  const int row0 = cu_seqlens[seq];
  int qlen = cu_seqlens[seq + 1] - row0;
  if (row0 < 0) return;
  qlen = min(qlen, T - row0);
  if (q0 >= qlen) return;
  const int slot = slots[seq];
  const int start = kv_start[seq];
  if ((unsigned)slot >= (unsigned)B || start < 0) return;
  const int q_hi = min(q0 + PF_BM, qlen);
  const int kv_end = min(start + q_hi, Smax);
  const int ntiles = (kv_end + PF_BN - 1) / PF_BN;

  const int tid = threadIdx.x;
  const int wave = tid >> 6;
  const int lane = tid & 63;
  const int lq = lane & 15;
  const int lh = lane >> 4;
  const int wrow0 = q0 + wave * 16;
  const bool wave_active = wrow0 < qlen;
  const int qr = wrow0 + lq;
  const bool row_valid = qr < qlen;
  const int pos = start + qr;
  const int wave_min_pos = start + wrow0;
  const int wave_max_pos = start + min(wrow0 + 15, qlen - 1);

  short8v qf[4];
  {
    const unsigned short* qp =
        Q + (size_t)(row0 + min(qr, qlen - 1)) * q_row_stride +
        (size_t)h * D + lh * 8;
#pragma unroll
    for (int ks = 0; ks < 4; ++ks)
// ... 1161 lines not shown
```

Baseline: 189.4 req/s.

## Add selectable decode fusions: GEMM+SwiGLU epilogue, slab-fold norm, ticketed attention combine

Adds a decode_fuse option (env MLRUN_DECODE_FUSE, default swiglu,norm) that picks per-layer fusions. 'swiglu' replaces the gate/up GEMM plus separate SwiGLU with one skinny GEMM that applies SwiGLU in its epilogue. 'norm' runs the wo and down split-K slab GEMMs followed by a templated slab-fold + residual add + RMSNorm kernel, and is now on by default instead of only under MLRUN_SLAB_MODE=all. An optional 'attn' mode lets the last split block of each head do the combine through atomic tickets, removing the separate combine launch. The aim is fewer kernel launches and less intermediate traffic per layer, at the cost of added atomics and shape-restricted kernel paths.

Result: faster. 198.2 req/s (median of 6 runs) (+4.6%).

```diff
diff --git a/mlrun_amd/models/llama.py b/mlrun_amd/models/llama.py
--- a/mlrun_amd/models/llama.py
+++ b/mlrun_amd/models/llama.py
@@ -257,7 +257,13 @@
                  weight_dtype: str = "bf16", kv_dtype: str = "bf16",
                  temperature: float = 0.0, top_k: int = 0,
                  max_adapters: int = 0, lora_rank: int = 16,
-                 lora: "LoraTables" = None, sampling: str = "engine"):
+                 lora: "LoraTables" = None, sampling: str = "engine",
+                 decode_fuse: str = None):
+        import os as _os
+        if decode_fuse is None:
+            decode_fuse = _os.environ.get("MLRUN_DECODE_FUSE",
+                                          self.DECODE_FUSE_DEFAULT)
+        self.decode_fuse = self._parse_decode_fuse(decode_fuse)
         if sampling not in ("engine", "request"):
             raise ValueError(f"unknown sampling mode {sampling!r} "
                              "(expected 'engine' or 'request')")
@@ -359,12 +365,14 @@
             self.buf_h8_scale = torch.empty(B, dtype=torch.float32,
                                             device=self.device)
             self.rebuild_fp8_packs()
-        import os as _os
         _ns = _os.environ.get("MLRUN_ATTN_NSPLIT")
         self.attn_nsplit = int(_ns) if _ns else \
             ops.pick_attn_nsplit(B, w.hkv)
         self.buf_attn_ws = torch.empty(
             B * w.hq * self.attn_nsplit * (d + 2), dtype=torch.float32,
+            device=self.device) if self.on_gpu else None
+        self.buf_attn_tickets = torch.zeros(
+            B * w.hkv, dtype=torch.int32,
             device=self.device) if self.on_gpu else None
         self._graph = None
         self._ksplits = {}
@@ -390,6 +398,40 @@
                                            device=dev)
             self.buf_kept = torch.zeros(B, dtype=torch.int32, device=dev)
         self.spec_stats = {"steps": 0, "drafted": 0, "accepted": 0}
+        self.active_fusions = self._resolve_fusions()
+
+    DECODE_FUSIONS = ("swiglu", "norm", "attn")
+    DECODE_FUSE_DEFAULT = "swiglu,norm"
+
+    @classmethod
+    def _parse_decode_fuse(cls, text: str) -> frozenset:
+        names = [n.strip() for n in str(text).split(",") if n.strip()]
+        if names == ["none"] or not names:
+            return frozenset()
+        for name in names:
+            if name not in cls.DECODE_FUSIONS:
+                raise ValueError(
+                    f"unknown decode fusion {name!r} (expected a comma "
+                    f"list of {', '.join(cls.DECODE_FUSIONS)}, or 'none')")
+        return frozenset(names)
+
+    def _resolve_fusions(self) -> tuple:
+        w, cfg = self.weights, self.cfg
+        plain = self.on_gpu and self.tp_size == 1 and \
+            self.weight_dtype == "bf16" and self.lora is None
+        if not plain:
+            return ()
+        h, d = cfg.hidden_size, cfg.head_dim
+        can = {
+            "swiglu": ops.skinny_gemm_swiglu_fuses(
+                self.B, w.inter, h, *ops.pick_gemm_plan(
+                    self.B, 2 * w.inter, h)),
+            "norm": ops.pick_gemm_plan(self.B, h, w.hq * d)[0] > 1 or
+            ops.pick_gemm_plan(self.B, h, w.inter)[0] > 1,
+            "attn": self.attn_nsplit > 1,
+        }
+        return tuple(n for n in self.DECODE_FUSIONS
+                     if n in self.decode_fuse and can[n])
 
     def set_sampling(self, slot: int, temperature: float = 0.0,
                      top_k: int = 0, top_p: float = 1.0, min_p: float = 0.0,
@@ -569,10 +611,13 @@
         on = self.on_gpu and self.tp_size == 1 and mode != "none"
         use_slabs = on and self.weight_dtype == "bf16" and \
             self.kv_dtype == "bf16"
-        use_norm_slabs = on and mode == "all" 
         lora = self.lora is not None
         if lora:
-            use_slabs = use_norm_slabs = False
+            use_slabs = False
+        fuse_swiglu = "swiglu" in self.active_fusions
+        fuse_norm = "norm" in self.active_fusions
+        tickets = self.buf_attn_tickets \
+            if "attn" in self.active_fusions else None
         for li, layer in enumerate(w.layers):
             done = 0
             if use_slabs:
@@ -601,16 +646,15 @@
                             partial_ws=self.buf_attn_ws,
                             nsplit=self.attn_nsplit,
                             k_scale=self._kscale(li),
-                            v_scale=self._vscale(li))
+                            v_scale=self._vscale(li), tickets=tickets)
             done = 0
-            if use_norm_slabs:
+            if fuse_norm:
                 done = self._gemm_slabs(self.buf_attn_out, layer["wo"])
                 if done:
-                    from mlrun_amd import _hip_ops
-
-                    _hip_ops.fused_add_rmsnorm_slab(
-                        self.buf_hidden, self.buf_residual, self.buf_c32,
-                        layer["ffn_norm"], done, cfg.rms_eps)
+                    ops.fused_add_rmsnorm_fold(
+                        self.buf_c32, done, layer["ffn_norm"],
+                        self.buf_residual, eps=cfg.rms_eps,
+                        out=self.buf_hidden)
             if not done:
                 self._gemm(self.buf_attn_out, layer["wo"], self.buf_proj)
                 if lora:
@@ -621,14 +665,11 @@
                                       residual=self.buf_residual,
                                       eps=cfg.rms_eps, out=self.buf_hidden,
                                       out8=h8, out_scale=h8s)
-            done = 0
-            if use_norm_slabs:
-                done = self._gemm_slabs(self.buf_hidden, layer["wgu"])
-                if done:
-                    from mlrun_amd import _hip_ops
-
-                    _hip_ops.swiglu_slab(self.buf_act, self.buf_c32, done)
-            if not done:
+            if fuse_swiglu:
+                ops.skinny_gemm_swiglu(self.buf_hidden, layer["wgu"],
+                                       out=self.buf_act,
+                                       ksplit=1, variant=4)
+            else:
                 self._gemm(self.buf_hidden, layer["wgu"], self.buf_gu,
                            a8=h8, a_scale=h8s)
                 if lora:
@@ -638,14 +679,12 @@
             next_norm = w.layers[li + 1]["attn_norm"] \
                 if li + 1 < cfg.num_layers else w.final_norm
             done = 0
-            if use_norm_slabs:
+            if fuse_norm:
                 done = self._gemm_slabs(self.buf_act, layer["wdown"])
                 if done:
-                    from mlrun_amd import _hip_ops
-
-                    _hip_ops.fused_add_rmsnorm_slab(
-                        self.buf_hidden, self.buf_residual, self.buf_c32,
-                        next_norm, done, cfg.rms_eps)
+                    ops.fused_add_rmsnorm_fold(
+                        self.buf_c32, done, next_norm, self.buf_residual,
+                        eps=cfg.rms_eps, out=self.buf_hidden)
             if not done:
                 self._gemm(self.buf_act, layer["wdown"], self.buf_down)
                 if lora:
@@ -1207,6 +1246,9 @@
 
     def reset(self):
         self.cache_lens.zero_()
+        if self.buf_attn_tickets is not None and \
+                "attn" in self.active_fusions:
+            self.buf_attn_tickets.zero_()
 
 
 class LlamaServer:
diff --git a/mlrun_amd/ops/__init__.py b/mlrun_amd/ops/__init__.py
--- a/mlrun_amd/ops/__init__.py
+++ b/mlrun_amd/ops/__init__.py
@@ -48,6 +48,30 @@
         out.copy_(result)
         return out
     return result
+
+
+def fused_add_rmsnorm_fold(slabs: torch.Tensor, ksplit: int,
+                           weight: torch.Tensor, residual: torch.Tensor,
+                           eps: float = 1e-5,
+                           out: torch.Tensor = None) -> torch.Tensor:
+    rows, hidden = residual.shape
+    if ksplit < 2:
+        raise ValueError(f"fused_add_rmsnorm_fold needs ksplit >= 2, "
+                         f"got {ksplit}")
+    if slabs.is_cuda:
+        ops = _require_hip()
+        if out is None:
+            out = torch.empty_like(residual)
+        ops.fused_add_rmsnorm_fold(out, residual, slabs, weight, ksplit,
+                                   eps)
+        return out
+    parts = slabs.reshape(-1)[:ksplit * rows * hidden].view(
+        ksplit, rows, hidden).float()
+    total = parts[0].clone()
+    for s in range(1, ksplit):
+        total += parts[s]
+    return fused_add_rmsnorm(total.to(residual.dtype), weight,
+                             residual=residual, eps=eps, out=out)
 
 
 def rmsnorm(x, weight, eps=1e-5, out=None, out8=None, out_scale=None):
@@ -195,6 +219,37 @@
         out.copy_(result)
         return out
     return result
+
+
+def skinny_gemm_swiglu_fuses(M: int, inter: int, K: int,
+                             ksplit: int = None,
+                             variant: int = None) -> bool:
+    if ksplit is None and variant is None:
+        ksplit, variant = pick_gemm_plan(M, 2 * inter, K)
+    return 16 < M <= 32 and K % 32 == 0 and inter % 8 == 0 and \
+        (ksplit, variant) == (1, 4)
+
+
+def skinny_gemm_swiglu(a: torch.Tensor, wgu: torch.Tensor,
+                       out: torch.Tensor = None,
+                       ksplit: int = None, variant: int = None,
+                       gu: torch.Tensor = None,
+                       c_f32: torch.Tensor = None) -> torch.Tensor:
+    M, K = a.shape
+    inter = wgu.shape[0] // 2
+    if a.is_cuda:
+        ops = _require_hip()
+        if skinny_gemm_swiglu_fuses(M, inter, K, ksplit, variant):
+            if out is None:
+                out = torch.empty(M, inter, dtype=torch.bfloat16,
+                                  device=a.device)
+            ops.skinny_gemm_swiglu(out, a, wgu)
+            return out
+        gu = skinny_gemm(a, wgu, out=gu, c_f32=c_f32, ksplit=ksplit,
+                         variant=variant)
+        return swiglu_fused(gu, out=out)
+    gu = (a.float() @ wgu.float().t()).to(a.dtype)
+    return swiglu_fused(gu, out=out)
 
 
 FP8_MAX = 448.0
@@ -340,7 +395,8 @@
                 partial_ws: torch.Tensor = None,
                 nsplit: int = None,
                 k_scale: torch.Tensor = None,
-                v_scale: torch.Tensor = None) -> torch.Tensor:
+                v_scale: torch.Tensor = None,
+                tickets: torch.Tensor = None) -> torch.Tensor:
     B, Hq, D = q.shape
     Hkv = k_cache.shape[1]
     scale = scale if scale is not None else 1.0 / math.sqrt(D)
@@ -353,8 +409,12 @@
         if nsplit > 1 and partial_ws is None:
             partial_ws = torch.empty(B * Hq * nsplit * (D + 2),
                                      dtype=torch.float32, device=q.device)
-        ops.attn_decode(out, q, k_cache, v_cache, seq_lens, scale,
-                        partial_ws, nsplit, k_scale, v_scale)
+        if tickets is None:
+            ops.attn_decode(out, q, k_cache, v_cache, seq_lens, scale,
+                            partial_ws, nsplit, k_scale, v_scale)
+        else:
+            ops.attn_decode(out, q, k_cache, v_cache, seq_lens, scale,
+                            partial_ws, nsplit, k_scale, v_scale, tickets)
         return out
     if out is None:
         out = torch.empty_like(q)
diff --git a/mlrun_amd/ops/hip/bindings.cpp b/mlrun_amd/ops/hip/bindings.cpp
--- a/mlrun_amd/ops/hip/bindings.cpp
+++ b/mlrun_amd/ops/hip/bindings.cpp
@@ -129,7 +129,7 @@
                            M, N, K, (int)ksplit, (int)variant, stream());
 }
 
-void fused_add_rmsnorm_slab(torch::Tensor out, torch::Tensor residual,
+void fused_add_rmsnorm_fold(torch::Tensor out, torch::Tensor residual,
                             torch::Tensor slabs, torch::Tensor weight,
                             int64_t ksplit, double eps) {
   CHECK_DEV(out); CHECK_CONTIG(out); CHECK_BF16(out);
@@ -139,22 +139,33 @@
   int64_t hidden = out.size(-1);
   int64_t rows = out.numel() / hidden;
   TORCH_CHECK(hidden % 8 == 0, "hidden must be a multiple of 8");
+  TORCH_CHECK(ksplit >= 2, "fused_add_rmsnorm_fold needs ksplit >= 2");
+  TORCH_CHECK(residual.numel() == out.numel(), "residual size mismatch");
+  TORCH_CHECK(weight.numel() == hidden, "weight size mismatch");
   TORCH_CHECK(slabs.numel() >= ksplit * rows * hidden, "slabs too small");
-  launch_fused_add_rmsnorm_slab(out.data_ptr(), residual.data_ptr(),
+  launch_fused_add_rmsnorm_fold(out.data_ptr(), residual.data_ptr(),
                                 slabs.data_ptr(), weight.data_ptr(),
                                 (int)rows, (int)hidden, (float)eps,
                                 (int)ksplit, stream());
 }
 
-void swiglu_slab(torch::Tensor out, torch::Tensor slabs, int64_t ksplit) {
+void skinny_gemm_swiglu(torch::Tensor out, torch::Tensor a,
+                        torch::Tensor wgu) {
   CHECK_DEV(out); CHECK_CONTIG(out); CHECK_BF16(out);
-  CHECK_DEV(slabs); CHECK_CONTIG(slabs); CHECK_F32(slabs);
-  int rows = out.size(0), inter = out.size(1);
-  TORCH_CHECK(inter % 4 == 0, "inter must be a multiple of 4");
-  TORCH_CHECK(slabs.numel() >= (int64_t)ksplit * rows * 2 * inter,
-              "slabs too small");
-  launch_swiglu_slab(out.data_ptr(), slabs.data_ptr(), rows, inter,
-                     (int)ksplit, stream());
+  CHECK_DEV(a); CHECK_CONTIG(a); CHECK_BF16(a);
+  CHECK_DEV(wgu); CHECK_CONTIG(wgu); CHECK_BF16(wgu);
+  TORCH_CHECK(a.dim() == 2 && wgu.dim() == 2, "need 2-D tensors");
+  int M = a.size(0), K = a.size(1);
+  TORCH_CHECK(wgu.size(0) % 2 == 0, "wgu must hold gate then up rows");
+  int inter = wgu.size(0) / 2;
+  TORCH_CHECK(wgu.size(1) == K, "K mismatch");
+  TORCH_CHECK(M > 16 && M <= 32, "skinny_gemm_swiglu needs 16 < M <= 32");
+  TORCH_CHECK(K % 32 == 0, "K must be a multiple of 32");
+  TORCH_CHECK(inter % 8 == 0, "inter must be a multiple of 8");
+  TORCH_CHECK(inter >= 8 && out.numel() == (int64_t)M * inter,
+              "out shape mismatch");
+  launch_skinny_gemm_swiglu(out.data_ptr(), a.data_ptr(), wgu.data_ptr(), M,
+                            inter, K, stream());
 }
 
 void rope_kv_slab(torch::Tensor qkv, torch::Tensor kc, torch::Tensor vc,
@@ -262,7 +273,8 @@
                  torch::Tensor vc, torch::Tensor seq_lens, double scale,
                  c10::optional<torch::Tensor> partial_ws, int64_t nsplit,
                  c10::optional<torch::Tensor> k_scale = c10::nullopt,
-                 c10::optional<torch::Tensor> v_scale = c10::nullopt) {
+                 c10::optional<torch::Tensor> v_scale = c10::nullopt,
+                 c10::optional<torch::Tensor> tickets = c10::nullopt) {
   CHECK_DEV(o); CHECK_CONTIG(o); CHECK_BF16(o);
   CHECK_DEV(q); CHECK_BF16(q);
   CHECK_DEV(kc); CHECK_CONTIG(kc);
@@ -299,12 +311,19 @@
     TORCH_CHECK(k_scale->numel() >= (int64_t)B * Hkv * Smax &&
                 v_scale->numel() >= (int64_t)B * Hkv * Smax,
                 "scale tensors too small");
+  int* tk = nullptr;
+  if (tickets.has_value() && nsplit > 1) {
+    CHECK_DEV(*tickets); CHECK_CONTIG(*tickets); CHECK_I32(*tickets);
+    TORCH_CHECK(tickets->numel() >= (int64_t)B * Hkv, "tickets too small");
+    tk = (int*)tickets->data_ptr();
+  }
   launch_attn_decode(o.data_ptr(), q.data_ptr(), kc.data_ptr(),
                      vc.data_ptr(),
                      kvq ? k_scale->data_ptr() : nullptr,
                      kvq ? v_scale->data_ptr() : nullptr,
                      seq_lens.data_ptr(), B, Hq, Hkv, Smax,
-                     (float)scale, q_row_stride, ws, (int)nsplit, stream());
+                     (float)scale, q_row_stride, ws, (int)nsplit, tk,
+                     stream());
 }
 
 void kv_append(torch::Tensor kc, torch::Tensor vc, torch::Tensor knew,
@@ -689,9 +708,10 @@
         "fused decode rope(q,k) + KV-cache append");
   m.def("skinny_gemm_slabs", &skinny_gemm_slabs,
         "split-K GEMM emitting f32 slabs only");
-  m.def("fused_add_rmsnorm_slab", &fused_add_rmsnorm_slab,
-        "slab-sum + residual add + RMSNorm");
-  m.def("swiglu_slab", &swiglu_slab, "slab-sum + SwiGLU");
+  m.def("fused_add_rmsnorm_fold", &fused_add_rmsnorm_fold,
+        "slab fold + bf16 rounding + residual add + RMSNorm");
+  m.def("skinny_gemm_swiglu", &skinny_gemm_swiglu,
+        "gate|up decode GEMM with SwiGLU in the epilogue");
   m.def("rope_kv_slab", &rope_kv_slab,
         "slab-sum + rope(q,k) + KV append");
   m.def("cast_f32_bf16", &cast_f32_bf16, "f32 -> bf16 cast");
@@ -703,7 +723,7 @@
         py::arg("kc"), py::arg("vc"), py::arg("seq_lens"),
         py::arg("scale"), py::arg("partial_ws") = py::none(),
         py::arg("nsplit") = 1, py::arg("k_scale") = py::none(),
-        py::arg("v_scale") = py::none(),
+        py::arg("v_scale") = py::none(), py::arg("tickets") = py::none(),
         "GQA decode attention (bf16 or fp8 KV cache)");
   m.def("kv_append", &kv_append, "append token K/V into cache");
   m.def("rope_kv_varlen", &rope_kv_varlen, py::arg("qkv"), py::arg("kc"),
diff --git a/mlrun_amd/ops/hip/kernels.h b/mlrun_amd/ops/hip/kernels.h
--- a/mlrun_amd/ops/hip/kernels.h
+++ b/mlrun_amd/ops/hip/kernels.h
@@ -20,13 +20,13 @@
                               int M, int N, int K, int ksplit, int variant,
                               void* stream);
 
-void launch_fused_add_rmsnorm_slab(void* out, void* residual,
+void launch_fused_add_rmsnorm_fold(void* out, void* residual,
                                    const void* slabs, const void* weight,
                                    int rows, int hidden, float eps,
                                    int ksplit, void* stream);
 
-void launch_swiglu_slab(void* out, const void* slabs, int rows, int inter,
-                        int ksplit, void* stream);
+void launch_skinny_gemm_swiglu(void* out, const void* A, const void* W,
+                               int M, int inter, int K, void* stream);
 
 void launch_rope_kv_slab(void* qkv, void* Kc, void* Vc, const void* slabs,
                          const void* positions, const void* cos_sin, int B,
@@ -66,7 +66,7 @@
                         const void* vscale, const void* seq_lens, int B,
                         int Hq, int Hkv, int Smax, float scale,
                         long long q_row_stride, float* partial_ws,
-                        int nsplit, void* stream);
+                        int nsplit, int* tickets, void* stream);
 
 void launch_kv_append(void* Kc, void* Vc, const void* knew, const void* vnew,
                       const void* positions, int B, int Hkv, int Smax, int D,
diff --git a/mlrun_amd/ops/hip/kernels.hip b/mlrun_amd/ops/hip/kernels.hip
--- a/mlrun_amd/ops/hip/kernels.hip
+++ b/mlrun_amd/ops/hip/kernels.hip
@@ -612,10 +612,11 @@
 
 typedef __attribute__((address_space(3))) void* lds_void_ptr;
 
-template <bool SPLIT, int STAGE_K, int DEPTH>
+template <bool SPLIT, int STAGE_K, int DEPTH, bool PAIR = false>
 __global__ __launch_bounds__(256) void skinny_gemm_ws_lds_kernel(
     void* __restrict__ out, const unsigned short* __restrict__ A,
     const unsigned short* __restrict__ W, int M, int N, int K, int ksplit) {
+  static_assert(!(PAIR && SPLIT), "the paired epilogue needs whole sums");
   constexpr int MT = 2, NT = 32;
   constexpr int ROW_B = STAGE_K * 2;
   constexpr int OP_B = 32 * ROW_B;
@@ -631,8 +632,15 @@
 
   const int lane = threadIdx.x & 63;
   const int wave = __builtin_amdgcn_readfirstlane(threadIdx.x >> 6);
-  const int n0 = blockIdx.x * NT;
-  if (n0 >= N) return;
+  const int inter = N >> 1;
+  const int n0 = blockIdx.x * (PAIR ? NT / 2 : NT);
+  if (n0 >= (PAIR ? inter : N)) return;
+  auto wrow = [&](int row) {
+    if (PAIR)
+      return row < 16 ? min(n0 + row, inter - 1)
+                      : inter + min(n0 + row - 16, inter - 1);
+    return min(n0 + row, N - 1);
+  };
   int cbegin = 0, cend = K;
   if (SPLIT) {
     const int kchunk = (K / ksplit + 31) & ~31;
@@ -660,7 +668,7 @@
   for (int i = 0; i < NDMA_OP; ++i) {
     const int row = i * RPI + lane / LPR;
     const int chunk = (lane % LPR) ^ lds_ring_swz<STAGE_K>(row);
-    wsrc[i] = W + (size_t)min(n0 + row, N - 1) * K + kbegin + chunk * 8;
+    wsrc[i] = W + (size_t)wrow(row) * K + kbegin + chunk * 8;
     asrc[i] = A + (size_t)min(row, M - 1) * K + kbegin + chunk * 8;
   }
   unsigned char* const ring = lds_ring + wave * WAVE_B;
@@ -751,10 +759,8 @@
     const unsigned short* aptr0 = A + (size_t)min(arow, M - 1) * K + kb;
     const unsigned short* aptr1 =
         A + (size_t)min(arow + 16, M - 1) * K + kb;
-    const unsigned short* bptr0 =
-        W + (size_t)min(n0 + arow, N - 1) * K + kb;
-    const unsigned short* bptr1 =
-        W + (size_t)min(n0 + arow + 16, N - 1) * K + kb;
+    const unsigned short* bptr0 = W + (size_t)wrow(arow) * K + kb;
+    const unsigned short* bptr1 = W + (size_t)wrow(arow + 16) * K + kb;
     for (int k = kbegin + nst * STAGE_K; k < kend; k += 32) {
       short8v bf0 = *reinterpret_cast<const short8v*>(bptr0 + k);
       short8v bf1 = *reinterpret_cast<const short8v*>(bptr1 + k);
@@ -791,6 +797,26 @@
         *reinterpret_cast<const comb_t*>(lds_ring + 2 * WAVE_B);
     const comb_t& c3 =
         *reinterpret_cast<const comb_t*>(lds_ring + 3 * WAVE_B);
+    if (PAIR) {
+      const int m = lane >> 1;
+      const int nb = (lane & 1) * 8;
+      ushort8 o;
+#pragma unroll
+      for (int c = 0; c < 8; ++c) {
+        const int n = nb + c;
+        const float sum_gate = c0[m][n] + c1[m][n] + c2[m][n] + c3[m][n];
+        const float sum_up = c0[m][n + 16] + c1[m][n + 16] +
+                             c2[m][n + 16] + c3[m][n + 16];
+        const float gf = bf2f(f2bf(sum_gate));
+        const float s = gf / (1.f + __expf(-gf));
+        o.v[c] = f2bf(s * bf2f(f2bf(sum_up)));
+      }
+      unsigned short* orow =
+          (unsigned short*)out + (size_t)m * inter + n0 + nb;
+      if (m < M && n0 + nb < inter)
+        *reinterpret_cast<ushort8*>(orow) = o;
+      return;
+    }
     constexpr int CPL = 4 * MT * 2;
 #pragma unroll
     for (int c = 0; c < CPL; ++c) {
@@ -1114,6 +1140,12 @@
       {skinny_gemm_ws_lds_kernel<true, 64, 3>, lds_ring_bytes<64, 3>()},
       {skinny_gemm_ws_lds_kernel<false, 128, 2>, lds_ring_bytes<128, 2>()},
       {skinny_gemm_ws_lds_kernel<true, 128, 2>, lds_ring_bytes<128, 2>()},
+      {skinny_gemm_ws_lds_kernel<false, 64, 2, true>,
+       lds_ring_bytes<64, 2>()},
+      {skinny_gemm_ws_lds_kernel<false, 64, 3, true>,
+       lds_ring_bytes<64, 3>()},
+      {skinny_gemm_ws_lds_kernel<false, 128, 2, true>,
+       lds_ring_bytes<128, 2>()},
   };
   for (const auto& k : all)
     (void)hipFuncSetAttribute(reinterpret_cast<const void*>(k.kern),
@@ -1150,6 +1182,31 @@
     default:
       launch_lds_ring<SPLIT, 64, 2>(out, A, W, M, N, K, ksplit, grid,
                                     stream);
+  }
+}
+
+template <int STAGE_K, int DEPTH>
+static void launch_lds_ring_pair(void* out, const void* A, const void* W,
+                                 int M, int inter, int K, void* stream) {
+  lds_ring_kern_t kern = skinny_gemm_ws_lds_kernel<false, STAGE_K, DEPTH, true>;
+  constexpr int bytes = lds_ring_bytes<STAGE_K, DEPTH>();
+  lds_ring_allow_all();
+  hipLaunchKernelGGL(kern, dim3((inter + 15) / 16), dim3(256), bytes,
+                     (hipStream_t)stream, out, (const unsigned short*)A,
+                     (const unsigned short*)W, M, 2 * inter, K, 1);
+}
+
+void launch_skinny_gemm_swiglu(void* out, const void* A, const void* W,
+                               int M, int inter, int K, void* stream) {
+  switch (gemm_lds_ring_env()) {
+    case 1:
+      launch_lds_ring_pair<64, 3>(out, A, W, M, inter, K, stream);
+      break;
+    case 2:
+      launch_lds_ring_pair<128, 2>(out, A, W, M, inter, K, stream);
+      break;
+    default:
+      launch_lds_ring_pair<64, 2>(out, A, W, M, inter, K, stream);
   }
 }
 
@@ -1350,7 +1407,8 @@
   return sum;
 }
 
-__global__ void fused_add_rmsnorm_slab_kernel(
+template <int KS>
+__global__ void fused_add_rmsnorm_fold_kernel(
     unsigned short* __restrict__ out, unsigned short* __restrict__ residual,
     const float* __restrict__ slabs,
     const unsigned short* __restrict__ weight, int hidden, float eps,
@@ -1358,28 +1416,64 @@
   const int row = blockIdx.x;
   const int tid = threadIdx.x;
   const int nthreads = blockDim.x;
-  const size_t rowbase = (size_t)row * hidden;
   const size_t slab_stride = (size_t)gridDim.x * hidden;
-  unsigned short* rr = residual + rowbase;
-  unsigned short* outr = out + rowbase;
+  const float* sr = slabs + (size_t)row * hidden;
+  unsigned short* rr = residual + (size_t)row * hidden;
+  unsigned short* outr = out + (size_t)row * hidden;
 
   float sumsq = 0.f;
-  for (int i = tid * 4; i < hidden; i += nthreads * 4) {
-    float z[4];
-#pragma unroll
-    for (int j = 0; j < 4; ++j)
-      z[j] = slab_sum(slabs, rowbase + i + j, slab_stride, ksplit);
-    unsigned short rv[4];
-    *reinterpret_cast<uint64_t*>(rv) =
-        *reinterpret_cast<const uint64_t*>(rr + i);
+  for (int i = tid * 8; i < hidden; i += nthreads * 8) {
+    f32x4v lo, hi;
+    ushort8 rv;
+    if (KS > 0) {
+      f32x4v plo[KS > 0 ? KS : 1], phi[KS > 0 ? KS : 1];
+#pragma unroll
+      for (int s = 0; s < KS; ++s) {
+        const float* p = sr + (size_t)s * slab_stride + i;
+        plo[s] = *reinterpret_cast<const f32x4v*>(p);
+        phi[s] = *reinterpret_cast<const f32x4v*>(p + 4);
+      }
+      rv = *reinterpret_cast<const ushort8*>(rr + i);
+      lo = plo[0];
+      hi = phi[0];
+#pragma unroll
+      for (int s = 1; s < KS; ++s) {
+#pragma unroll
+        for (int j = 0; j < 4; ++j) {
+          lo[j] += plo[s][j];
+          hi[j] += phi[s][j];
+        }
+      }
+    } else {
+      lo = *reinterpret_cast<const f32x4v*>(sr + i);
+      hi = *reinterpret_cast<const f32x4v*>(sr + i + 4);
+      rv = *reinterpret_cast<const ushort8*>(rr + i);
+      for (int s = 1; s < ksplit; ++s) {
+        const float* p = sr + (size_t)s * slab_stride + i;
+        const f32x4v vlo = *reinterpret_cast<const f32x4v*>(p);
+        const f32x4v vhi = *reinterpret_cast<const f32x4v*>(p + 4);
+#pragma unroll
+        for (int j = 0; j < 4; ++j) {
+          lo[j] += vlo[j];
+          hi[j] += vhi[j];
+        }
+      }
+    }
+    float z[8];
 #pragma unroll
     for (int j = 0; j < 4; ++j) {
-      z[j] += bf2f(rv[j]);
-      rv[j] = f2bf(z[j]);
-      sumsq += z[j] * z[j];
-    }
-    *reinterpret_cast<uint64_t*>(rr + i) =
-        *reinterpret_cast<const uint64_t*>(rv);
+      z[j] = bf2f(f2bf(lo[j]));
+      z[j + 4] = bf2f(f2bf(hi[j]));
+    }
+    ushort8 zv;
+#pragma unroll
+    for (int j = 0; j < 8; ++j) {
+      z[j] += bf2f(rv.v[j]);
+      zv.v[j] = f2bf(z[j]);
+    }
+    *reinterpret_cast<ushort8*>(rr + i) = zv;
+#pragma unroll
+    for (int j = 0; j < 8; ++j) sumsq += z[j] * z[j];
   }
   __shared__ float red[32];
 #pragma unroll
@@ -1397,63 +1491,34 @@
   if (tid == 0) red[0] = sumsq;
   __syncthreads();
   const float inv = rsqrtf(red[0] / hidden + eps);
+
   for (int i = tid * 8; i < hidden; i += nthreads * 8) {
     ushort8 zv = *reinterpret_cast<const ushort8*>(rr + i);
     ushort8 wv = *reinterpret_cast<const ushort8*>(weight + i);
     ushort8 ov;
 #pragma unroll
-    for (int j = 0; j < 8; ++j)
-      ov.v[j] = f2bf(bf2f(zv.v[j]) * inv * bf2f(wv.v[j]));
+    for (int j = 0; j < 8; ++j) {
+      const float value = bf2f(zv.v[j]) * inv * bf2f(wv.v[j]);
+      ov.v[j] = f2bf(value);
+    }
     *reinterpret_cast<ushort8*>(outr + i) = ov;
   }
 }
 
-void launch_fused_add_rmsnorm_slab(void* out, void* residual,
+void launch_fused_add_rmsnorm_fold(void* out, void* residual,
                                    const void* slabs, const void* weight,
                                    int rows, int hidden, float eps,
                                    int ksplit, void* stream) {
   int threads = hidden >= 2048 ? 256 : 64;
-  hipLaunchKernelGGL(fused_add_rmsnorm_slab_kernel, dim3(rows),
-                     dim3(threads), 0, (hipStream_t)stream,
-                     (unsigned short*)out, (unsigned short*)residual,
-                     (const float*)slabs, (const unsigned short*)weight,
-                     hidden, eps, ksplit);
-}
-
-__global__ void swiglu_slab_kernel(unsigned short* __restrict__ out,
-                                   const float* __restrict__ slabs,
-                                   int rows, int inter, int ksplit) {
-  const size_t slab_stride = (size_t)rows * 2 * inter;
-  const long long total = (long long)rows * inter / 4;
-  long long i = (long long)blockIdx.x * blockDim.x + threadIdx.x;
-  long long stride = (long long)gridDim.x * blockDim.x;
-  for (; i < total; i += stride) {
-    const long long flat = i * 4;
-    const int r = (int)(flat / inter);
-    const int c = (int)(flat % inter);
-    const size_t base = (size_t)r * 2 * inter + c;
-    unsigned short o[4];
-#pragma unroll
-    for (int j = 0; j < 4; ++j) {
-      const float g = slab_sum(slabs, base + j, slab_stride, ksplit);
-      const float u = slab_sum(slabs, base + inter + j, slab_stride,
-                               ksplit);
-      const float s = g / (1.f + __expf(-g));
-      o[j] = f2bf(s * u);
-    }
-    *reinterpret_cast<uint64_t*>(out + (size_t)r * inter + c) =
-        *reinterpret_cast<const uint64_t*>(o);
-  }
-}
-
-void launch_swiglu_slab(void* out, const void* slabs, int rows, int inter,
-                        int ksplit, void* stream) {
-  long long blocks = ((long long)rows * inter / 4 + 255) / 256;
-  if (blocks > 2048) blocks = 2048;
-  if (blocks < 1) blocks = 1;
-  hipLaunchKernelGGL(swiglu_slab_kernel, dim3((int)blocks), dim3(256), 0,
+  auto kern = ksplit == 2   ? fused_add_rmsnorm_fold_kernel<2>
+              : ksplit == 3 ? fused_add_rmsnorm_fold_kernel<3>
+              : ksplit == 4 ? fused_add_rmsnorm_fold_kernel<4>
+              : ksplit == 8 ? fused_add_rmsnorm_fold_kernel<8>
+                            : fused_add_rmsnorm_fold_kernel<0>;
+  hipLaunchKernelGGL(kern, dim3(rows), dim3(threads), 0,
                      (hipStream_t)stream, (unsigned short*)out,
-                     (const float*)slabs, rows, inter, ksplit);
+                     (unsigned short*)residual, (const float*)slabs,
+                     (const unsigned short*)weight, hidden, eps, ksplit);
 }
 
 __global__ void rope_kv_slab_kernel(
@@ -1752,13 +1817,44 @@
   op[1] = f2bf(st.acc1 * inv);
 }
 
+DEV void attn_combine_head(unsigned short* __restrict__ O,
+                           const float* __restrict__ partial, int bh,
+                           int lane, int nsplit) {
+  constexpr int D = 128;
+  const float* base = partial + (size_t)bh * nsplit * (D + 2);
+  float m_star = -FLT_MAX;
+  for (int s = 0; s < nsplit; ++s)
+    m_star = fmaxf(m_star, base[s * (D + 2) + D]);
+  float l_total = 0.f, a0 = 0.f, a1 = 0.f;
+  for (int s = 0; s < nsplit; ++s) {
+    const float* prow = base + s * (D + 2);
+    const float ms = prow[D];
+    if (ms == -FLT_MAX) continue;
+    const float wgt = __expf(ms - m_star);
+    l_total += wgt * prow[D + 1];
+    a0 += wgt * prow[lane * 2];
+    a1 += wgt * prow[lane * 2 + 1];
+  }
+  const float inv = (l_total > 0.f) ? 1.f / l_total : 0.f;
+  unsigned short* op = O + (size_t)bh * D + lane * 2;
+  op[0] = f2bf(a0 * inv);
+  op[1] = f2bf(a1 * inv);
+}
+
+__global__ void attn_decode_combine_kernel(
+    unsigned short* __restrict__ O, const float* __restrict__ partial,
+    int Hq, int nsplit) {
+  attn_combine_head(O, partial, blockIdx.x, threadIdx.x, nsplit);
+}
+
 template <int SCHUNK, bool KVQ = false>
 __global__ void attn_decode_split_kernel(
     float* __restrict__ partial, const unsigned short* __restrict__ Q,
     const void* __restrict__ Kc, const void* __restrict__ Vc,
     const float* __restrict__ kscale, const float* __restrict__ vscale,
     const int* __restrict__ seq_lens, int B, int Hq, int Hkv, int Smax,
-    float scale, long long q_row_stride, int nsplit) {
+    float scale, long long q_row_stride, int nsplit,
+    unsigned short* __restrict__ O, int* __restrict__ tickets) {
   constexpr int D = 128;
   const int b = blockIdx.x / Hkv;
   const int kvh = blockIdx.x % Hkv;
@@ -1799,32 +1895,29 @@
     prow[D] = st.m;
     prow[D + 1] = st.l;
   }
-}
-
-__global__ void attn_decode_combine_kernel(
-    unsigned short* __restrict__ O, const float* __restrict__ partial,
-    int Hq, int nsplit) {
-  constexpr int D = 128;
-  const int bh = blockIdx.x;
-  const int lane = threadIdx.x;
-  const float* base = partial + (size_t)bh * nsplit * (D + 2);
-  float m_star = -FLT_MAX;
-  for (int s = 0; s < nsplit; ++s)
-    m_star = fmaxf(m_star, base[s * (D + 2) + D]);
-  float l_total = 0.f, a0 = 0.f, a1 = 0.f;
-  for (int s = 0; s < nsplit; ++s) {
-    const float* prow = base + s * (D + 2);
-    const float ms = prow[D];
-    if (ms == -FLT_MAX) continue;
-    const float wgt = __expf(ms - m_star);
-    l_total += wgt * prow[D + 1];
-    a0 += wgt * prow[lane * 2];
-    a1 += wgt * prow[lane * 2 + 1];
-  }
-  const float inv = (l_total > 0.f) ? 1.f / l_total : 0.f;
-  unsigned short* op = O + (size_t)bh * D + lane * 2;
-  op[0] = f2bf(a0 * inv);
-  op[1] = f2bf(a1 * inv);
+  if (tickets == nullptr) return;
+  asm volatile("s_waitcnt vmcnt(0)" ::: "memory");
+  __syncthreads();
+  if (threadIdx.x == 0) {
+    __builtin_amdgcn_fence(__ATOMIC_RELEASE, "agent");
+    asm volatile("s_waitcnt vmcnt(0)" ::: "memory");
+    const int t = __hip_atomic_fetch_add(&tickets[blockIdx.x], 1,
+                                         __ATOMIC_RELAXED,
+                                         __HIP_MEMORY_SCOPE_AGENT);
+    scores[0][0] = __int_as_float(t);
+  }
+  __syncthreads();
+  const int ticket = __float_as_int(scores[0][0]);
+  if (ticket != nsplit - 1) return;
+  if (threadIdx.x == 0) {
+    __builtin_amdgcn_fence(__ATOMIC_ACQUIRE, "agent");
+    asm volatile("s_waitcnt vmcnt(0)" ::: "memory");
+  }
+  __syncthreads();
+  attn_combine_head(O, partial, b * Hq + h, lane, nsplit);
+  if (threadIdx.x == 0)
+    __hip_atomic_store(&tickets[blockIdx.x], 0, __ATOMIC_RELAXED,
+                       __HIP_MEMORY_SCOPE_AGENT);
 }
 
 static int attn_schunk_env() {
@@ -1840,7 +1933,7 @@
                         const void* vscale, const void* seq_lens, int B,
                         int Hq, int Hkv, int Smax, float scale,
                         long long q_row_stride, float* partial_ws,
-                        int nsplit, void* stream) {
+                        int nsplit, int* tickets, void* stream) {
   const int G = Hq / Hkv;
   const bool c64 = attn_schunk_env() >= 64;
   const bool kvq = kscale != nullptr;
@@ -1866,7 +1959,9 @@
                      (const unsigned short*)Q, Kc, Vc,
                      (const float*)kscale, (const float*)vscale,
                      (const int*)seq_lens, B, Hq,
-                     Hkv, Smax, scale, q_row_stride, nsplit);
+                     Hkv, Smax, scale, q_row_stride, nsplit,
+                     (unsigned short*)O, tickets);
+  if (tickets != nullptr) return;
   hipLaunchKernelGGL(attn_decode_combine_kernel, dim3(B * Hq), dim3(64), 0,
                      (hipStream_t)stream, (unsigned short*)O, partial_ws,
                      Hq, nsplit);
```
